# Patryk27/strolle

Measured on NVIDIA H100. Metric: Mrays/s (+ frames/s) at 1080p-per-GPU Cornell, ReSTIR DI+GI + SVGF; H100 vs CPU restatement of the reference, higher is better.
Workload: dtype f32

## Files before the change

### strolle_b200/csrc/engine.cu

```cuda
#include <algorithm>
#include <cmath>
#include <cstdio>
#include <cstring>
#include <deque>
#include <functional>
#include <limits>
#include <string>
#include <unordered_map>
#include <vector>

#include <nccl.h>

#include "../../include/strolle_b200.h"
#include "kernels.h"

#include <dlfcn.h>
namespace {
struct NcclApi {
    void* lib = nullptr;
    ncclResult_t (*GetUniqueId)(ncclUniqueId*) = nullptr;
    ncclResult_t (*CommInitRank)(ncclComm_t*, int, ncclUniqueId, int) = nullptr;
    ncclResult_t (*CommDestroy)(ncclComm_t) = nullptr;
    ncclResult_t (*GroupStart)() = nullptr;
    ncclResult_t (*GroupEnd)() = nullptr;
// ... 268 lines not shown
            nodes[pr.dst] = n;
        }
    }
    void plan_child(RefitPlan* plan, int child, uint32_t ptr, uint32_t slot, int depth) const {
        const Node& c = nodes[child];
        if (c.left >= 0) {
            if ((int)plan->levels.size() <= depth) plan->levels.resize(depth + 1);
            plan->levels[depth].push_back(make_uint2(ptr, slot));
        } else plan->runs.push_back(make_uint4(slot, ptr, c.e - c.b, 0u));
    }
    uint32_t emit(int id, int depth, const std::vector<uint8_t>& alpha, BvhOut* out, RefitPlan* plan) const {
        uint32_t at = (uint32_t)out->buf.size();
        if (depth > out->depth) out->depth = depth;
        const Node& nd = nodes[id];
        if (nd.left >= 0) {
            out->buf.resize(out->buf.size() + 4, make_float4(0, 0, 0, 0));
            uint32_t lp = emit(nd.left, depth + 1, alpha, out, plan);
            uint32_t rp = emit(nd.right, depth + 1, alpha, out, plan);
            if (plan) { plan_child(plan, nd.left, lp, at, depth + 1); plan_child(plan, nd.right, rp, at + 2, depth + 1); }
            const Box& lb = nodes[nd.left].box; const Box& rb = nodes[nd.right].box;
            out->buf[at] = make_float4(lb.lo.x, lb.lo.y, lb.lo.z, bits2f(0u));
            out->buf[at + 1] = make_float4(lb.hi.x, lb.hi.y, lb.hi.z, bits2f(rp));
            out->buf[at + 2] = make_float4(rb.lo.x, rb.lo.y, rb.lo.z, 0.0f);
            out->buf[at + 3] = make_float4(rb.hi.x, rb.hi.y, rb.hi.z, 0.0f);
        } else {
            uint32_t n = nd.e - nd.b;
            for (uint32_t i = 0; i < n; i++) {
                const Prim& p = prims[nd.b + i];
                uint32_t flags = (i + 1 < n ? 1u : 0u) | ((alpha[p.mat] ? 1u : 0u) << 1);
                out->buf.push_back(make_float4(bits2f(flags), bits2f(p.tri), bits2f(p.mat), bits2f(1u)));
            }
        }
        return at;
    }
};

struct DevMem {
    void* p = nullptr; size_t cap = 0;
    int ensure(size_t bytes) {
        if (bytes <= cap) return ST_OK;
        if (p) cudaFree(p);
        p = nullptr; cap = 0;
        size_t want = std::max<size_t>(bytes, 256);
        CK(cudaMalloc(&p, want));
        CK(cudaMemset(p, 0, want));
        CK(cudaDeviceSynchronize());
        cap = want;
        return ST_OK;
    }
    void release() { if (p) cudaFree(p); p = nullptr; cap = 0; }
};

static const char* kPassNames[P_COUNT] = {
    "prim_gbuffer", "di_sampling", "di_temporal_resampling", "di_spatial_resampling_pick", "di_spatial_resampling_trace", "di_spatial_resampling_sample",
    "di_resolving", "gi_reprojection", "gi_sampling_a", "gi_sampling_b", "gi_temporal_resampling", "gi_spatial_resampling_pick",
    "gi_spatial_resampling_trace", "gi_spatial_resampling_sample", "gi_preview_resampling", "gi_resolving", "frame_reprojection",
    "frame_denoising_reproject", "frame_denoising_estimate_variance", "frame_denoising_wavelet", "frame_composition", "ref_tracing",
    "ref_shading", "bvh_heatmap", "atmosphere", "trace_stream", "halo_exchange"};

static uint32_t dispatch_seed(uint32_t base, uint32_t frame, uint32_t k) {
    uint32_t s = base ^ (frame * 64u + k);
    s = s * 747796405u + 2891336453u;
    uint32_t w = ((s >> ((s >> 28) + 4u)) ^ s) * 277803737u;
    return (w >> 22) ^ w;
}

struct CameraSlot {
    bool alive = false;
    st_camera desc;
    st_camera prev_desc;
    uint32_t frame = 0;
    CameraDev dev;
    std::vector<std::pair<std::string, float4**>> named;
    std::vector<std::pair<std::string, size_t>> sizes;
    DevMem arena;
    DevMem svgf_pairs; float4* pair[2] = {nullptr, nullptr};
    DevMem rgba8; int rgba8_slot = 0;
    DevMem taa; float4* taa_hist[2] = {nullptr, nullptr};
    cudaEvent_t ev_ready[2] = {nullptr, nullptr}, ev_copied[2] = {nullptr, nullptr};
    cudaStream_t side[2] = {nullptr, nullptr}; cudaEvent_t ev_produced = nullptr, ev_pushed[2] = {nullptr, nullptr}; bool pushed_pending[2] = {false, false};
    struct PeerLink { bool ready = false; bool ipc = false; std::vector<char*> arena, rgba8; std::vector<uint32_t*> flags; DevMem sync; uint32_t seq = 0, fseq = 0; } peer;
};

struct Step { int pass; std::function<void(cudaStream_t)> run; int sub = -1; };

}

using namespace st;

struct st_engine {
    int device = 0;
    cudaStream_t stream = nullptr; bool own_stream = true;
    cudaStream_t copy_stream = nullptr;
    std::unordered_map<st_handle, std::vector<st_mesh_triangle>> meshes;
    std::vector<st_material> materials; std::vector<st_handle> material_handles; bool materials_dirty = false;
    struct MatTex { st_handle tex[4]; uint32_t mask; };
    std::vector<MatTex> material_textures;
    struct ImageRect { st_handle handle; uint32_t x, y, w, h; };
    std::vector<ImageRect> images; uint32_t shelf_x = 0, shelf_y = 0, shelf_h = 0; bool images_dirty = false;
    DevMem d_atlas, d_srgb, d_tri_instance, d_instance_xforms;
    bool motion_dirty = true;
    bool moved_last_tick = false;
    struct Inst {
        st_handle handle, mesh, material; Affine3 xf, xf_inv, prev_xf; bool dirty;
        st_handle baked_mesh = ~(st_handle)0, baked_material = ~(st_handle)0; bool host_stale = false; Affine3 dev_xf, dev_xf_inv;
    };
    std::vector<Inst> instances; bool instances_dirty = false;
    struct Range { st_handle handle; size_t b, e; };
    std::vector<Range> tri_ranges; SlotAllocator tri_alloc;
    std::vector<float4> h_triangles; std::vector<Prim> prims; bool triangles_dirty = false;
    BvhBuild bvh; BvhOut bvh_out; bool bvh_dirty = false;
    std::vector<GpuMaterial> h_materials;
    static const st_handle kSun = ~(st_handle)0;
    std::vector<GpuLight> h_lights; std::vector<std::pair<st_handle, uint32_t>> light_slots;
    std::vector<st_handle> lights_created, lights_updated; std::vector<std::pair<st_handle, uint32_t>> lights_remapped; std::vector<uint32_t> lights_killed;
    uint32_t next_light = 1; bool lights_dirty = true;
    float sun_azimuth = 0.0f, sun_altitude = 0.35f; bool sun_dirty = true;
    GpuWorld world;
    uint32_t frame = 1, seed_base = 0xC0FFEEu;
    DevMem d_triangles, d_bvh, d_materials, d_matpacked, d_unpacklut, d_lights, d_noise, d_tlut, d_slut, d_skylut, d_scratch, d_raycount;
    bool count_rays = false;
    bool svgf_fast = true;
    bool shading_fast = ST_SHADING_FAST_DEFAULT != 0;
    bool fused_passes = ST_FUSED_PASSES_DEFAULT != 0;
    bool async_output = false;
    bool halo_nccl = false;
    int wavelet_paired = ST_WAVELET_PAIRED_DEFAULT;
    int strip_dma = ST_STRIP_DMA_DEFAULT;
    bool strip_fused = true;
    bool last_frame_fused = false;
    int wavelet_tiled = ST_WAVELET_TILED_DEFAULT;
    int wavelet_cfg = ST_WAVELET_CFG_DEFAULT;
    DevMem d_tile_errors; uint64_t wavelet_tiled_launches = 0;
    bool fuse_reproject = ST_FUSE_REPROJECT_DEFAULT != 0;
    bool bvh_reuse = true;
    bool variance_tiled = ST_VARIANCE_TILED_DEFAULT != 0; uint64_t variance_tiled_launches = 0;
    bool normal_maps = false, any_normal_map = false, nmap_frame = false; uint64_t normal_map_launches = 0;
    int bvh_refit = 0; uint32_t refit_run = 0; uint64_t bvh_refits = 0; bool structure_changed = false;
    RefitPlan plan; bool plan_ready = false; std::vector<uint32_t> plan_levels; std::vector<uint8_t> plan_alpha; DevMem d_plan, d_bake;
    std::unordered_map<st_handle, DevMem> d_meshes;
    void* staging[2] = {nullptr, nullptr}; size_t staging_cap[2] = {0, 0}; cudaEvent_t staging_ev[2] = {nullptr, nullptr}; int staging_slot = 0;
    int light_grid = 0, lgrid_built = 0; bool lgrid_frame = false; LightGridDev lgrid{}; DevMem d_lgrid; uint64_t light_grid_builds = 0;
    bool texture_filter = false, texf_built = false, any_color_texture = false, texf_frame = false; TexFilterDev texf{};
    DevMem d_texf_pool, d_texf_table, d_texf_jobs; std::vector<uint2> h_texf_table; std::vector<MipJob> h_texf_jobs; size_t texf_pool_texels = 0;
    uint64_t texture_mip_builds = 0;
    bool temporal_aa = false, taa_frame = false; uint64_t taa_resolves = 0;
    bool luts_static_ready = false, sky_ready = false; float sky_for_altitude = 0.0f;
    std::vector<CameraSlot*> cameras;
    bool timing = false;
    float pass_ms[P_COUNT] = {}; uint32_t pass_launches[P_COUNT] = {};
    float wavelet_ms[5] = {}; uint32_t wavelet_launches[5] = {};
    struct Timed { int pass; cudaEvent_t a, b; int sub; };
    std::vector<Timed> pending; std::vector<cudaEvent_t> event_pool;
    cudaEvent_t mark_a = nullptr, mark_b = nullptr;
    ncclComm_t comm = nullptr; int rank = 0, n_ranks = 1;
    uint64_t halo_bytes_last_frame = 0;

    SceneDev scene() const {
        SceneDev s;
        s.triangles = (const float4*)d_triangles.p; s.bvh = (const float4*)d_bvh.p; s.bvh_len = (uint32_t)bvh_out.buf.size(); s.materials = (const GpuMaterial*)d_materials.p;
        s.lights = (const GpuLight*)d_lights.p; s.blue_noise = (const uchar4*)d_noise.p;
        s.transmittance_lut = (const float4*)d_tlut.p; s.scattering_lut = (const float4*)d_slut.p; s.sky_lut = (const float4*)d_skylut.p;
        s.world = world;
        s.tri_instance = (const uint32_t*)d_tri_instance.p; s.instance_xforms = (const float4*)d_instance_xforms.p;
        s.atlas = (const uchar4*)d_atlas.p; s.srgb_lut = (const float*)d_srgb.p;
        s.material_packed = (const uint32_t*)d_matpacked.p; s.unpack_lut = (const float*)d_unpacklut.p;
        s.ray_counter = count_rays ? (unsigned long long*)d_raycount.p : nullptr;
// ... 400 lines not shown
    for (auto& s : cs->sizes) total += (s.second * 16 + 255) / 256 * 256;
    cs->arena.release();
    int rc = cs->arena.ensure(total); if (rc) return rc;
    CK(cudaMemsetAsync(cs->arena.p, 0, total, e->stream));
    const size_t pair_bytes = (2 * n * 16 + 255) / 256 * 256;
    cs->svgf_pairs.release();
    if ((rc = cs->svgf_pairs.ensure(2 * pair_bytes))) return rc;
    CK(cudaMemsetAsync(cs->svgf_pairs.p, 0, 2 * pair_bytes, e->stream));
    cs->pair[0] = (float4*)cs->svgf_pairs.p; cs->pair[1] = (float4*)((char*)cs->svgf_pairs.p + pair_bytes);
    size_t off = 0;
    for (size_t i = 0; i < cs->named.size(); i++) { *cs->named[i].second = (float4*)((char*)cs->arena.p + off); off += (cs->sizes[i].second * 16 + 255) / 256 * 256; }
    d.w = (int)cs->desc.width; d.h = (int)cs->desc.height; d.y0 = 0; d.y1 = d.h;
    d.own_y0 = 0; d.own_y1 = d.h; d.mirror_up = 0; d.mirror_dn = 0; d.need_rows = nullptr; d.gi_mirror_reach = 128; d.di_mirror_reach = 128;
    cs->taa.release(); cs->taa_hist[0] = cs->taa_hist[1] = nullptr;
    return ST_OK;
}

struct StripExt { int gbuffer = 0, variance = 0, wavelet[5] = {0, 0, 0, 0, 0}; int preview_mirror[2] = {0, 0}; bool still = false;  };
static CameraDev grown(const CameraDev& c, int rows) { CameraDev g = c; g.y0 = std::max(0, c.y0 - rows); g.y1 = std::min(c.h, c.y1 + rows); return g; }
static void build_schedule(st_engine* e, CameraSlot* cs, std::vector<Step>* steps, const StripExt* ext = nullptr) {
    GpuCamera jc, jp; float4 jit;
    const bool taa = taa_cameras(e, cs, &jc, &jp, &jit);
    const CameraDev cam = [&] { CameraDev c = cs->dev; if (taa) { c.curr = jc; c.prev = jp; } return c; }();
    const StripExt no_ext; const StripExt& x = ext ? *ext : no_ext;
    const CameraDev camG = grown(cam, x.gbuffer), camV = grown(cam, x.variance);
    const int pm0 = x.preview_mirror[0], pm1 = x.preview_mirror[1];
    const SceneDev sc = e->scene();
    const uint32_t f = cs->frame;
    const int cur = (f % 2u) == 1u ? 1 : 0;
    const st_camera& d = cs->desc;
    const bool fs = e->shading_fast;
    const bool nm = e->nmap_frame;
    const bool lgon = e->lgrid_frame;
    const LightGridDev lgd = e->lgrid;
    const bool tfon = e->texf_frame;
    const TexFilterDev tfd = e->texf;
    auto seed = [&](uint32_t k) { return dispatch_seed(e->seed_base, f, k); };
    auto add = [&](int pass, std::function<void(cudaStream_t)> fn) { steps->push_back(Step{pass, std::move(fn)}); };
    const float4* di_final = (d.denoise && (d.mode == ST_MODE_IMAGE || d.mode == ST_MODE_DI_DIFFUSE)) ? cam.di_diff_curr_colors : cam.di_diff_samples;
    const float4* gi_final = (d.denoise && (d.mode == ST_MODE_IMAGE || d.mode == ST_MODE_GI_DIFFUSE)) ? cam.gi_diff_curr_colors : cam.gi_diff_samples;
    if (d.mode == ST_MODE_BVH_HEATMAP) {
        add(P_BVH_HEATMAP, [=](cudaStream_t s) { launch_bvh_heatmap(cam, sc, s); });
        add(P_COMPOSITION, [=](cudaStream_t s) { launch_composition(cam, sc, cur, 5u, di_final, gi_final, s); });
        return;
    }
    if (d.mode == ST_MODE_REFERENCE) {
        for (uint32_t depth = 0; depth <= (uint32_t)d.ref_depth; depth++) {
            uint32_t sd = seed(P_REF_SHADING_SEED + depth);
            add(P_REF_TRACING, [=](cudaStream_t s) { if (nm) e->normal_map_launches++; launch_ref_tracing(cam, sc, depth, nm, s); });
            add(P_REF_SHADING, [=](cudaStream_t s) { launch_ref_shading(cam, sc, sd, depth, lgon ? &lgd : nullptr, tfon ? &tfd : nullptr, s); });
        }
        add(P_REF_SHADING, [=](cudaStream_t s) { launch_ref_shading(cam, sc, 0u, 255u, nullptr, nullptr, s); });
        add(P_COMPOSITION, [=](cudaStream_t s) { launch_composition(cam, sc, cur, 6u, di_final, gi_final, s); });
        return;
    }
    const bool needs_di = d.mode == ST_MODE_IMAGE || d.mode == ST_MODE_DI_DIFFUSE || d.mode == ST_MODE_DI_SPECULAR;
    const bool needs_gi = d.mode == ST_MODE_IMAGE || d.mode == ST_MODE_GI_DIFFUSE || d.mode == ST_MODE_GI_SPECULAR;
    const int k4_in_k0 = (e->fused_passes && (ext == nullptr || ext->still) && !e->instances.empty()) ? 1 : 0;
    add(P_PRIM_GBUFFER, [=](cudaStream_t s) { if (nm) e->normal_map_launches++; launch_prim_gbuffer(camG, sc, cur, k4_in_k0, nm, tfon ? &tfd : nullptr, s); });
    const bool fp = e->fused_passes;
    if (!e->instances.empty()) {
        if (!k4_in_k0) add(P_FRAME_REPROJECTION, [=](cudaStream_t s) { launch_frame_reprojection(cam, sc, cur, s); });
        if (needs_di) {
            uint32_t s1 = seed(P_DI_SAMPLING), s2 = seed(P_DI_TEMPORAL), s3 = seed(P_DI_SPATIAL_PICK), s5 = seed(P_DI_SPATIAL_SAMPLE);
            if (fp) {
                add(P_DI_TEMPORAL, [=](cudaStream_t s) { (fs ? stf::launch_di_sample_temporal : st::launch_di_sample_temporal)(cam, sc, cur, s1, s2, f, lgon ? &lgd : nullptr, s); });
                add(P_DI_SPATIAL_PICK, [=](cudaStream_t s) { (fs ? stf::launch_di_spatial_fused : st::launch_di_spatial_fused)(cam, sc, cur, s3, s5, f, s); });
            } else {
                add(P_DI_SAMPLING, [=](cudaStream_t s) { (fs ? stf::launch_di_sampling : st::launch_di_sampling)(cam, sc, cur, s1, f, lgon ? &lgd : nullptr, s); });
                add(P_DI_TEMPORAL, [=](cudaStream_t s) { (fs ? stf::launch_di_temporal : st::launch_di_temporal)(cam, sc, cur, s2, s); });
                add(P_DI_SPATIAL_PICK, [=](cudaStream_t s) { (fs ? stf::launch_di_spatial_pick : st::launch_di_spatial_pick)(cam, sc, cur, s3, f, s); });
                add(P_DI_SPATIAL_TRACE, [=](cudaStream_t s) { (fs ? stf::launch_spatial_trace : st::launch_spatial_trace)(cam, sc, cam.di_diff_samples, cam.di_diff_curr_colors, cam.di_diff_stash, s); });
                add(P_DI_SPATIAL_SAMPLE, [=](cudaStream_t s) { (fs ? stf::launch_di_spatial_sample : st::launch_di_spatial_sample)(cam, sc, s5, f, s); });
            }
            add(P_DI_RESOLVING, [=](cudaStream_t s) { (fs ? stf::launch_di_resolving : st::launch_di_resolving)(cam, sc, cur, s); });
        }
        if (needs_gi) {
            uint32_t sa = seed(P_GI_SAMPLING_A), sb = seed(P_GI_SAMPLING_B), st_ = seed(P_GI_TEMPORAL), sp = seed(P_GI_SPATIAL_PICK), ss = seed(P_GI_SPATIAL_SAMPLE), sv = seed(P_GI_PREVIEW);
            uint32_t source;
            const bool tracing = f % 6u < 4u;
            const int inline_rp = (fp && tracing) ? 1 : 0;
            if (!inline_rp) add(P_GI_REPROJECTION, [=](cudaStream_t s) { (fs ? stf::launch_gi_reprojection : st::launch_gi_reprojection)(cam, sc, cur, s); });
            auto sampling = [&]() {
                if (fp) { add(P_GI_SAMPLING_B, [=](cudaStream_t s) { if (nm) e->normal_map_launches++; (fs ? stf::launch_gi_sampling_fused : st::launch_gi_sampling_fused)(cam, sc, cur, sa, sb, f, nm, lgon ? &lgd : nullptr, tfon ? &tfd : nullptr, s); }); return; }
                add(P_GI_SAMPLING_A, [=](cudaStream_t s) { if (nm) e->normal_map_launches++; (fs ? stf::launch_gi_sampling_a : st::launch_gi_sampling_a)(cam, sc, cur, sa, f, nm, tfon ? &tfd : nullptr, s); });
                add(P_GI_SAMPLING_B, [=](cudaStream_t s) { (fs ? stf::launch_gi_sampling_b : st::launch_gi_sampling_b)(cam, sc, cur, sb, f, lgon ? &lgd : nullptr, s); });
            };
            if (tracing) {
                if (f % 2u == 0u) sampling();
                add(P_GI_TEMPORAL, [=](cudaStream_t s) { (fs ? stf::launch_gi_temporal : st::launch_gi_temporal)(cam, sc, cur, st_, f, inline_rp, s); });
                if (f % 2u == 1u) {
                    if (fp) add(P_GI_SPATIAL_PICK, [=](cudaStream_t s) { (fs ? stf::launch_gi_spatial_fused : st::launch_gi_spatial_fused)(cam, sc, cur, sp, ss, f, s); });
                    else {
                        add(P_GI_SPATIAL_PICK, [=](cudaStream_t s) { (fs ? stf::launch_gi_spatial_pick : st::launch_gi_spatial_pick)(cam, sc, cur, sp, f, s); });
                        add(P_GI_SPATIAL_TRACE, [=](cudaStream_t s) { (fs ? stf::launch_spatial_trace : st::launch_spatial_trace)(cam, sc, cam.gi_d0, cam.gi_d1, cam.gi_d2, s); });
                        add(P_GI_SPATIAL_SAMPLE, [=](cudaStream_t s) { (fs ? stf::launch_gi_spatial_sample : st::launch_gi_spatial_sample)(cam, sc, ss, f, s); });
                    }
                    source = 1;
                } else source = 0;
            } else {
                sampling();
                add(P_GI_TEMPORAL, [=](cudaStream_t s) { (fs ? stf::launch_gi_temporal : st::launch_gi_temporal)(cam, sc, cur, st_, f, 0, s); });
                source = 0;
            }
            const float4* src0 = source == 0 ? cam.gi_reservoirs[1] : cam.gi_reservoirs[2];
            add(P_GI_PREVIEW, [=](cudaStream_t s) { (fs ? stf::launch_gi_preview : st::launch_gi_preview)(cam, sc, cur, sv, 0u, src0, cam.gi_reservoirs[3], pm0, s); });
            if (fp) add(P_GI_PREVIEW, [=](cudaStream_t s) { (fs ? stf::launch_gi_preview_resolve : st::launch_gi_preview_resolve)(cam, sc, cur, sv, cam.gi_reservoirs[3], src0, s); });
            else {
                add(P_GI_PREVIEW, [=](cudaStream_t s) { (fs ? stf::launch_gi_preview : st::launch_gi_preview)(cam, sc, cur, sv, 1u, cam.gi_reservoirs[3], cam.gi_reservoirs[0], pm1, s); });
                add(P_GI_RESOLVING, [=](cudaStream_t s) { (fs ? stf::launch_gi_resolving : st::launch_gi_resolving)(cam, sc, cur, src0, s); });
            }
        }
    }
    if (d.denoise) {
        if (e->fuse_reproject) {
            add(P_DENOISE_REPROJECT, [=](cudaStream_t s) { launch_denoise_reproject_pair(cam, sc, cur, s); });
        } else {
            add(P_DENOISE_REPROJECT, [=](cudaStream_t s) { launch_denoise_reproject(cam, sc, cur, cam.di_diff_prev_colors, cam.di_diff_moments[cur ^ 1], cam.di_diff_samples, cam.di_diff_curr_colors, cam.di_diff_moments[cur], s); });
            add(P_DENOISE_REPROJECT, [=](cudaStream_t s) { launch_denoise_reproject(cam, sc, cur, cam.gi_diff_prev_colors, cam.gi_diff_moments[cur ^ 1], cam.gi_diff_samples, cam.gi_diff_curr_colors, cam.gi_diff_moments[cur], s); });
        }
        const bool fast = e->svgf_fast;
        const bool var_tiled = e->variance_tiled; uint32_t* verr = (uint32_t*)e->d_tile_errors.p;
        add(P_DENOISE_VARIANCE, [=](cudaStream_t s) {
            if (var_tiled && launch_denoise_variance_tiled(camV, sc, cur, fast, verr, s)) { e->variance_tiled_launches++; return; }
            launch_denoise_variance(camV, sc, cur, fast, s);
        });
        float4* di_io[5][2] = {{cam.di_diff_stash, cam.di_diff_prev_colors}, {cam.di_diff_prev_colors, cam.di_diff_stash}, {cam.di_diff_stash, cam.di_diff_curr_colors},
                               {cam.di_diff_curr_colors, cam.di_diff_stash}, {cam.di_diff_stash, cam.di_diff_curr_colors}};
        float4* gi_io[5][2] = {{cam.gi_diff_stash, cam.gi_diff_prev_colors}, {cam.gi_diff_prev_colors, cam.gi_diff_stash}, {cam.gi_diff_stash, cam.gi_diff_curr_colors},
                               {cam.gi_diff_curr_colors, cam.gi_diff_stash}, {cam.gi_diff_stash, cam.gi_diff_curr_colors}};
        const bool whole_or_fused = ext != nullptr || (cam.y0 == 0 && cam.y1 == cam.h);
        const int first_paired_read = (fast && whole_or_fused && cs->pair[0]) ? (e->wavelet_paired == 2 ? 3 : e->wavelet_paired == 1 ? 4 : 5) : 5;
        for (uint32_t nth = 0; nth < 5; nth++) {
            float4 *a = di_io[nth][0], *b = di_io[nth][1], *c = gi_io[nth][0], *g = gi_io[nth][1];
            const bool reads_pair = (int)nth >= first_paired_read, writes_pair = (int)nth + 1 >= first_paired_read && nth < 4;
            const float4* pin = reads_pair ? cs->pair[nth & 1] : nullptr; float4* pout = writes_pair ? cs->pair[(nth + 1) & 1] : nullptr;
            const bool tiled = !reads_pair && ((e->wavelet_tiled >> nth) & 1) != 0; const int cfg = (e->wavelet_cfg >> (4 * nth)) & 15;
            uint32_t* terr = (uint32_t*)e->d_tile_errors.p;
            const CameraDev camW = grown(cam, x.wavelet[nth]);
            add(P_DENOISE_WAVELET, [=](cudaStream_t s) {
                if (tiled && launch_denoise_wavelet_tiled(camW, sc, f, 1u << nth, (float)(1 + nth), a, b, c, g, pout, fast, cfg, terr, s)) { e->wavelet_tiled_launches++; return; }
                launch_denoise_wavelet(camW, sc, cur, f, 1u << nth, (float)(1 + nth), a, b, c, g, pin, pout, fast, s);
            });
            steps->back().sub = (int)nth;
        }
    }
    uint32_t mode = (uint32_t)d.mode;
    if (taa) {
        const float4* hin = cs->taa_hist[cur ^ 1]; float4* hout = cs->taa_hist[cur];
        add(P_COMPOSITION, [=](cudaStream_t s) { e->taa_resolves++; launch_taa_resolve(cam, sc, cur, mode, di_final, gi_final, hin, hout, jit, s); });
        return;
    }
    add(P_COMPOSITION, [=](cudaStream_t s) { launch_composition(cam, sc, cur, mode, di_final, gi_final, s); });
}


struct HaloItem { std::string name; int reach; };
struct HaloExchange { int before_step; std::vector<HaloItem> items; };
static const int kSpatialReach = 128;
static const int kPreview2Reach = 64;
static const int kVarianceReach = 3;
static const int kWaveletReach[5] = {1, 2, 4, 9, 19};

static void plan_frame(const int* schedule, int n, uint32_t frame, int temporal_reach, std::vector<HaloExchange>* plan) {
    const char* cur = (frame % 2u == 1u) ? "b" : "a";
    const char* prv = (frame % 2u == 1u) ? "a" : "b";
    bool have_gbuffer = false; int nth_preview = 0, nth_wavelet = 0;
    const char* wavelet_inputs[5] = {"stash", "prev_colors", "stash", "curr_colors", "stash"};
    bool has_preview = false, has_gi_spatial = false;
    for (int i = 0; i < n; i++) { if (schedule[i] == P_GI_PREVIEW) has_preview = true; if (schedule[i] == P_GI_SPATIAL_PICK) has_gi_spatial = true; }
    std::string gi_source = has_gi_spatial ? "gi_reservoirs_2" : "gi_reservoirs_1";
    for (int i = 0; i < n; i++) {
        int p = schedule[i];
        HaloExchange ex; ex.before_step = i;
        auto add = [&](const std::string& name, int reach) { ex.items.push_back({name, reach}); };
        if (i == 0 && temporal_reach > 0) {
            add(std::string("prim_surface_map_") + prv, temporal_reach); add(std::string("prim_gbuffer_d0_") + prv, temporal_reach); add(std::string("prim_gbuffer_d1_") + prv, temporal_reach);
            add("di_reservoirs_0", temporal_reach); add("gi_reservoirs_0", temporal_reach); add("di_diff_prev_colors", temporal_reach); add("gi_diff_prev_colors", temporal_reach);
            add(std::string("di_diff_moments_") + prv, temporal_reach); add(std::string("gi_diff_moments_") + prv, temporal_reach);
        }
        if (p == P_DI_SPATIAL_PICK || p == P_GI_SPATIAL_PICK) {
            if (!have_gbuffer) { add(std::string("prim_gbuffer_d0_") + cur, kSpatialReach); add(std::string("prim_gbuffer_d1_") + cur, kSpatialReach); add("surface_nd", kSpatialReach); have_gbuffer = true; }
            add(p == P_DI_SPATIAL_PICK ? "di_reservoirs_1" : "gi_reservoirs_1", kSpatialReach);
        } else if (p == P_GI_PREVIEW) {
            if (nth_preview == 0) {
// ... 564 lines not shown
            e->refit_run = 0;
            e->plan_ready = e->bvh_refit > 0 && !too_deep;
            if (e->plan_ready) { e->plan_alpha = alpha; if ((rc = upload_plan(e))) return rc; }
        }
        e->moved_last_tick = e->motion_dirty;
    }
    if (e->motion_dirty) {
        e->motion_dirty = false;
        std::vector<uint32_t> tri_inst(e->h_triangles.size() / 9, 0u);
        std::vector<float4> xf = instance_xforms();
        for (size_t k = 0; k < e->instances.size(); k++)
            for (const auto& r : e->tri_ranges) if (r.handle == e->instances[k].handle) for (size_t t = r.b; t < r.e; t++) tri_inst[t] = (uint32_t)k;
        if ((rc = upload(e, e->d_tri_instance, tri_inst.data(), tri_inst.size() * 4))) return rc;
        if ((rc = upload(e, e->d_instance_xforms, xf.data(), xf.size() * 16))) return rc;
        CK(cudaStreamSynchronize(e->stream));
    }
    if (e->triangles_dirty) { e->triangles_dirty = false; if ((rc = upload(e, e->d_triangles, e->h_triangles.data(), e->h_triangles.size() * 16))) return rc; }
    e->world.light_count = e->next_light; e->world.sun_azimuth = e->sun_azimuth; e->world.sun_altitude = e->sun_altitude;
    if (e->sun_dirty) {
        e->sun_dirty = false;
        if ((rc = e->d_scratch.ensure(64))) return rc;
        launch_atm_sun_color((float4*)e->d_scratch.p, e->world, e->stream);
        float4 sun[2];
        CK(cudaMemcpyAsync(sun, e->d_scratch.p, 32, cudaMemcpyDeviceToHost, e->stream));
        CK(cudaStreamSynchronize(e->stream));
        light_overwrite(e, 0, st_engine::kSun, make_sun(sun[0], sun[1]));
    }
    const bool lights_uploaded = e->lights_dirty;
    if (e->lights_dirty) {
        for (uint32_t id : e->lights_killed) e->h_lights[id].d3.x = bits2f(0xcafebabeu);
        for (auto& r : e->lights_remapped) e->h_lights[r.second].d3.x = bits2f(*e->light_slot(r.first) + 1u);
        if ((rc = upload(e, e->d_lights, e->h_lights.data(), e->h_lights.size() * sizeof(GpuLight)))) return rc;
        CK(cudaStreamSynchronize(e->stream));
        bool again = !e->lights_created.empty() || !e->lights_updated.empty() || !e->lights_killed.empty() || !e->lights_remapped.empty();
        for (st_handle h : e->lights_created) { GpuLight& l = e->h_lights[*e->light_slot(h)]; l.prev_d0 = l.d0; l.prev_d1 = l.d1; l.prev_d2 = l.d2; }
        for (st_handle h : e->lights_updated) { GpuLight& l = e->h_lights[*e->light_slot(h)]; l.prev_d0 = l.d0; l.prev_d1 = l.d1; l.prev_d2 = l.d2; }
        for (uint32_t id : e->lights_killed) e->h_lights[id].d3.x = 0.0f;
        for (auto& r : e->lights_remapped) e->h_lights[r.second].d3.x = 0.0f;
        e->lights_created.clear(); e->lights_updated.clear(); e->lights_remapped.clear(); e->lights_killed.clear();
        e->lights_dirty = again;
    }
    if (e->light_grid == 0) e->lgrid_built = 0;
    else if (lights_uploaded || e->lgrid_built != e->light_grid) { if ((rc = build_light_grid(e))) return rc; }
    e->lgrid_frame = e->light_grid > 0;
    for (CameraSlot* c : e->cameras) if (c->alive) c->frame = e->frame;
    e->nmap_frame = e->normal_maps && e->any_normal_map;
    if (!e->texture_filter) {
        if (e->texf_built || e->d_texf_pool.p) { e->d_texf_pool.release(); e->d_texf_table.release(); e->d_texf_jobs.release(); e->texf = TexFilterDev{}; }
        e->texf_built = false;
    } else if (textures_changed || !e->texf_built) { if ((rc = build_texture_mips(e))) return rc; }
    e->texf_frame = e->texture_filter && e->any_color_texture;
    if (e->temporal_aa != e->taa_frame) for (CameraSlot* c : e->cameras) { c->taa.release(); c->taa_hist[0] = c->taa_hist[1] = nullptr; }
    e->taa_frame = e->temporal_aa;
    e->frame += 1;
    if (too_deep) return fail(ST_ERR_LIMIT, "BVH deeper than the 24-entry traversal stack (strolle-gpu/src/lib.rs:72-76): the scene is not drawn until it changes");
    return ST_OK;
}

int st_frame_schedule(st_engine* e, st_camera_handle h, int* pass_ids, int cap, int* count) {
    CameraSlot* cs = e ? get_camera(e, h) : nullptr;
    if (!cs || !count) return fail(ST_ERR_NOT_FOUND, "unknown camera");
    std::vector<Step> steps; build_schedule(e, cs, &steps);
    *count = (int)steps.size();
    for (int i = 0; i < cap && i < *count; i++) pass_ids[i] = steps[i].pass;
    return ST_OK;
}
static int ensure_taa_history(st_engine* e, CameraSlot* cs) {
    GpuCamera a, b; float4 j;
    if (cs->taa.p || !taa_cameras(e, cs, &a, &b, &j)) return ST_OK;
    const size_t bytes = ((size_t)cs->desc.width * cs->desc.height * 16 + 255) / 256 * 256;
    int rc = cs->taa.ensure(2 * bytes); if (rc) return rc;
    cs->taa_hist[0] = (float4*)cs->taa.p; cs->taa_hist[1] = (float4*)((char*)cs->taa.p + bytes);
    return ST_OK;
}
int st_render_range(st_engine* e, st_camera_handle h, int first, int last) {
    CameraSlot* cs = e ? get_camera(e, h) : nullptr;
    if (!cs) return fail(ST_ERR_NOT_FOUND, "unknown camera");
    if (cs->frame == 0) return fail(ST_ERR_INVALID, "st_tick must precede st_render_camera");
    CK(cudaSetDevice(e->device));
    int rc = ensure_luts(e); if (rc) return rc;
    if ((rc = ensure_taa_history(e, cs))) return rc;
    std::vector<Step> steps; build_schedule(e, cs, &steps);
    if (last < 0 || last >= (int)steps.size()) last = (int)steps.size() - 1;
    for (int i = std::max(first, 0); i <= last; i++) e->run_timed(steps[i].pass, steps[i].run, steps[i].sub);
    CK(cudaGetLastError());
    return ST_OK;
}
int st_render_camera(st_engine* e, st_camera_handle h, void* host_out, int format) {
    int rc = st_render_range(e, h, 0, -1); if (rc) return rc;
    if (host_out) return st_copy_output(e, h, host_out, format);
    return ST_OK;
}
static int copy_rows_out(st_engine* e, CameraSlot* cs, void* host_out, int format, int y0, int y1) {
    const size_t W = cs->desc.width, n = W * cs->desc.height;
    const size_t first = (size_t)y0 * W, count = (size_t)(y1 - y0) * W;
    if (format == ST_FORMAT_RGBA32F) CK(cudaMemcpyAsync((char*)host_out + first * 16, cs->dev.output + first, count * 16, cudaMemcpyDeviceToHost, e->stream));
    else if (format == ST_FORMAT_RGBA8_SRGB) {
        int rc2 = cs->rgba8.ensure(2 * n * 4); if (rc2) return rc2;
        cs->rgba8_slot ^= 1;
        SceneDev sc = e->scene(); uchar4* dst8 = (uchar4*)cs->rgba8.p + (cs->rgba8_slot ? n : 0); CameraDev cd = cs->dev; cd.y0 = y0; cd.y1 = y1;
        const int k = cs->rgba8_slot;
        if (e->async_output) {
            if (!e->copy_stream) CK(cudaStreamCreateWithFlags(&e->copy_stream, cudaStreamNonBlocking));
            if (!cs->ev_ready[k]) { CK(cudaEventCreateWithFlags(&cs->ev_ready[k], cudaEventDisableTiming)); CK(cudaEventCreateWithFlags(&cs->ev_copied[k], cudaEventDisableTiming)); }
            else CK(cudaStreamWaitEvent(e->stream, cs->ev_copied[k], 0));
        }
        e->run_timed(P_COMPOSITION, [=](cudaStream_t s) { launch_output_rgba8(cd, sc, dst8, s); });
        if (e->async_output) {
            CK(cudaEventRecord(cs->ev_ready[k], e->stream));
            CK(cudaStreamWaitEvent(e->copy_stream, cs->ev_ready[k], 0));
            CK(cudaMemcpyAsync((char*)host_out + first * 4, dst8 + first, count * 4, cudaMemcpyDeviceToHost, e->copy_stream));
            CK(cudaEventRecord(cs->ev_copied[k], e->copy_stream));
        } else CK(cudaMemcpyAsync((char*)host_out + first * 4, dst8 + first, count * 4, cudaMemcpyDeviceToHost, e->stream));
    } else return fail(ST_ERR_INVALID, "unsupported output format");
    return ST_OK;
}
int st_copy_output(st_engine* e, st_camera_handle h, void* host_out, int format) {
    CameraSlot* cs = e ? get_camera(e, h) : nullptr;
    if (!cs || !host_out) return fail(ST_ERR_NOT_FOUND, "unknown camera");
    CK(cudaSetDevice(e->device));
    int rc = copy_rows_out(e, cs, host_out, format, 0, (int)cs->desc.height); if (rc) return rc;
    if (!e->async_output) CK(cudaStreamSynchronize(e->stream));
    return ST_OK;
}
int st_synchronize(st_engine* e) {
    if (!e) return fail(ST_ERR_INVALID, "null engine");
    CK(cudaSetDevice(e->device)); CK(cudaStreamSynchronize(e->stream));
    if (e->copy_stream) CK(cudaStreamSynchronize(e->copy_stream));
    for (CameraSlot* c : e->cameras) for (int k = 0; k < 2; k++) if (c->side[k]) CK(cudaStreamSynchronize(c->side[k]));
    return ST_OK;
}

int st_read_buffer(st_engine* e, st_camera_handle h, const char* name, float* dst, size_t cap, size_t* count) {
    CameraSlot* cs = e ? get_camera(e, h) : nullptr;
    if (!cs || !name || !count) return fail(ST_ERR_NOT_FOUND, "unknown camera");
    CK(cudaSetDevice(e->device));
    if (!std::strcmp(name, "curr_camera") || !std::strcmp(name, "prev_camera")) {
        GpuCamera jc, jp; float4 jit;
        const bool taa = taa_cameras(e, cs, &jc, &jp, &jit);
        const GpuCamera& c = !std::strcmp(name, "curr_camera") ? (taa ? jc : cs->dev.curr) : (taa ? jp : cs->dev.prev);
        *count = 40; if (dst) std::memcpy(dst, &c, 4 * std::min<size_t>(cap, 40)); return ST_OK;
    }
    if (!std::strcmp(name, "taa_history_a") || !std::strcmp(name, "taa_history_b")) {
        const float4* p = cs->taa_hist[name[12] == 'a' ? 0 : 1];
        if (!p) return fail(ST_ERR_NOT_FOUND, "no temporal history: ST_OPT_TEMPORAL_AA is off or the camera has not resolved a frame since");
        *count = (size_t)cs->desc.width * cs->desc.height * 4;
        if (dst) { CK(cudaStreamSynchronize(e->stream)); CK(cudaMemcpy(dst, p, 4 * std::min(cap, *count), cudaMemcpyDeviceToHost)); }
        return ST_OK;
    }
    for (size_t i = 0; i < cs->named.size(); i++) if (cs->named[i].first == name) {
        *count = cs->sizes[i].second * 4;
        if (dst) { CK(cudaStreamSynchronize(e->stream)); CK(cudaMemcpy(dst, *cs->named[i].second, 4 * std::min(cap, *count), cudaMemcpyDeviceToHost)); }
        return ST_OK;
    }
    return fail(ST_ERR_NOT_FOUND, std::string("unknown buffer ") + name);
}
int st_buffer_device_ptr(st_engine* e, st_camera_handle h, const char* name, void** ptr, size_t* bytes) {
    CameraSlot* cs = e ? get_camera(e, h) : nullptr;
    if (!cs || !name || !ptr || !bytes) return fail(ST_ERR_NOT_FOUND, "unknown camera");
    for (size_t i = 0; i < cs->named.size(); i++) if (cs->named[i].first == name) { *ptr = *cs->named[i].second; *bytes = cs->sizes[i].second * 16; return ST_OK; }
    if ((!std::strcmp(name, "taa_history_a") || !std::strcmp(name, "taa_history_b")) && cs->taa_hist[0]) {
        *ptr = cs->taa_hist[name[12] == 'a' ? 0 : 1]; *bytes = (size_t)cs->desc.width * cs->desc.height * 16; return ST_OK;
    }
    return fail(ST_ERR_NOT_FOUND, std::string("unknown buffer ") + name);
}
int st_read_scene(st_engine* e, const char* name, float* dst, size_t cap, size_t* count) {
    if (!e || !name || !count) return fail(ST_ERR_INVALID, "null argument");
// ... 598 lines not shown
```

### strolle_b200/csrc/kernels.cu

```cuda
#include <algorithm>
#include <cstdio>
#include <cuda_fp16.h>
#include <cuda.h>
#include <map>
#include <mutex>
#include <tuple>
#include <vector>
#include "st_device.cuh"
#include "kernels.h"

#if defined(ST_FAST) && ST_FAST
#define ST_EXACT_ONLY 0
#else
#define ST_EXACT_ONLY 1
#endif

namespace ST_NS {

#define TILE_W 16
#define TILE_H 8

struct Px { u32 x, y; bool in; };
ST_DEV u32 row_tile(const CameraDev& cam) {
    if (cam.mirror_dn == 0) return blockIdx.y;
    const u32 lead = (u32)(ST_REACH_SPATIAL / TILE_H);
    return gridDim.y > lead ? (blockIdx.y + gridDim.y - lead) % gridDim.y : blockIdx.y;
}
ST_DEV Px pixel_full(const CameraDev& cam) {
    Px p; p.x = blockIdx.x * TILE_W + (threadIdx.x % TILE_W); p.y = (u32)cam.y0 + row_tile(cam) * TILE_H + (threadIdx.x / TILE_W);
    p.in = p.x < (u32)cam.w && p.y < (u32)cam.y1;
    return p;
}
ST_DEV int half_grid_w(int w) { return 8 * (((w + 7) / 8) / 2); }
ST_DEV Px pixel_half(const CameraDev& cam) {
    Px p; p.x = blockIdx.x * TILE_W + (threadIdx.x % TILE_W); p.y = (u32)cam.y0 + row_tile(cam) * TILE_H + (threadIdx.x / TILE_W);
    p.in = p.x < (u32)half_grid_w(cam.w) && p.y < (u32)cam.y1;
    return p;
}
ST_DEV size_t pix(const CameraDev& cam, u32 x, u32 y) { return (size_t)y * (size_t)cam.w + x; }
ST_DEV size_t screen_idx(const CameraDev& cam, u32 x, u32 y) { return (size_t)(y * to_u32_sat(cam.curr.screen.x) + x); }
ST_DEV bool in_tex(const CameraDev& cam, u32 x, u32 y) { return x < (u32)cam.w && y < (u32)cam.h; }
ST_DEV float4 tex_or_zero(const float4* __restrict__ t, const CameraDev& cam, u32 x, u32 y) { return in_tex(cam, x, y) ? t[pix(cam, x, y)] : f4zero(); }
ST_DEV void tex_store(float4* __restrict__ t, const CameraDev& cam, u32 x, u32 y, float4 v) { if (in_tex(cam, x, y)) t[pix(cam, x, y)] = v; }
ST_DEV Hit load_hit(const GpuCamera& c, const float4* __restrict__ d0, const float4* __restrict__ d1, const CameraDev& cam, u32 x, u32 y) {
    return hit_make(cam_ray(c, x, y), gbuf_unpack(tex_or_zero(d0, cam, x, y), tex_or_zero(d1, cam, x, y)));
}
ST_DEV Hit load_hit_lut(const SceneDev& sc, const GpuCamera& c, const float4* __restrict__ d0, const float4* __restrict__ d1, const CameraDev& cam, u32 x, u32 y) {
    return hit_make(cam_ray(c, x, y), gbuf_unpack(sc, tex_or_zero(d0, cam, x, y), tex_or_zero(d1, cam, x, y)));
}
#define ST_TRACE_STACK()                                          \
    __shared__ u32 s_stack[ST_BVH_STACK * ST_BLOCK];              \
    TraceStack stk; stk.base = s_stack + threadIdx.x;

#define KPARAMS const __grid_constant__ CameraDev cam, const __grid_constant__ SceneDev sc

#define ST_LB_N(N) __launch_bounds__(ST_BLOCK, N)
#if !defined(ST_MINB_ALL)
#define ST_MINB_GI_PREVIEW 8
#define ST_MINB_GI_TEMPORAL 8
#define ST_MINB_GI_SAMPLING_B 8
#define ST_MINB_GI_SPATIAL_PICK 8
#define ST_MINB_DI_TEMPORAL 12
#endif
#define ST_LB_PICK(per_kernel) ST_LB_CHOOSE(ST_MINB_ALL_OR_0, per_kernel)
#if defined(ST_MINB_ALL)
#define ST_MINB_ALL_OR_0 ST_MINB_ALL
#else
#define ST_MINB_ALL_OR_0 0
#endif
template <int ALL, int ONE> struct LbMin { static constexpr int value = ALL > 0 ? ALL : ONE; };
#define ST_LB_CHOOSE(all, one) __launch_bounds__(ST_BLOCK, (LbMin<all, one>::value > 0 ? LbMin<all, one>::value : 1))
#ifndef ST_MINB_PRIM_GBUFFER
#define ST_MINB_PRIM_GBUFFER 0
#endif
#define ST_LB_PRIM_GBUFFER ST_LB_PICK(ST_MINB_PRIM_GBUFFER)
#ifndef ST_MINB_DI_SAMPLING
#define ST_MINB_DI_SAMPLING 0
#endif
#define ST_LB_DI_SAMPLING ST_LB_PICK(ST_MINB_DI_SAMPLING)
#ifndef ST_MINB_DI_TEMPORAL
#define ST_MINB_DI_TEMPORAL 0
#endif
#define ST_LB_DI_TEMPORAL ST_LB_PICK(ST_MINB_DI_TEMPORAL)
#ifndef ST_MINB_DI_SPATIAL_PICK
#define ST_MINB_DI_SPATIAL_PICK 0
#endif
#define ST_LB_DI_SPATIAL_PICK ST_LB_PICK(ST_MINB_DI_SPATIAL_PICK)
#ifndef ST_MINB_SPATIAL_TRACE
#define ST_MINB_SPATIAL_TRACE 0
#endif
#define ST_LB_SPATIAL_TRACE ST_LB_PICK(ST_MINB_SPATIAL_TRACE)
#ifndef ST_MINB_DI_RESOLVING
#define ST_MINB_DI_RESOLVING 0
#endif
#define ST_LB_DI_RESOLVING ST_LB_PICK(ST_MINB_DI_RESOLVING)
#ifndef ST_MINB_GI_SAMPLING_A
#define ST_MINB_GI_SAMPLING_A 0
#endif
#define ST_LB_GI_SAMPLING_A ST_LB_PICK(ST_MINB_GI_SAMPLING_A)
#ifndef ST_MINB_GI_SAMPLING_B
#define ST_MINB_GI_SAMPLING_B 0
#endif
#define ST_LB_GI_SAMPLING_B ST_LB_PICK(ST_MINB_GI_SAMPLING_B)
#ifndef ST_MINB_GI_TEMPORAL
#define ST_MINB_GI_TEMPORAL 0
#endif
#define ST_LB_GI_TEMPORAL ST_LB_PICK(ST_MINB_GI_TEMPORAL)
#ifndef ST_MINB_GI_SPATIAL_PICK
#define ST_MINB_GI_SPATIAL_PICK 0
#endif
#define ST_LB_GI_SPATIAL_PICK ST_LB_PICK(ST_MINB_GI_SPATIAL_PICK)
#ifndef ST_MINB_GI_SPATIAL_SAMPLE
#define ST_MINB_GI_SPATIAL_SAMPLE 0
#endif
#define ST_LB_GI_SPATIAL_SAMPLE ST_LB_PICK(ST_MINB_GI_SPATIAL_SAMPLE)
#ifndef ST_MINB_GI_PREVIEW
#define ST_MINB_GI_PREVIEW 0
#endif
#define ST_LB_GI_PREVIEW ST_LB_PICK(ST_MINB_GI_PREVIEW)
#ifndef ST_MINB_GI_RESOLVING
#define ST_MINB_GI_RESOLVING 0
#endif
#define ST_LB_GI_RESOLVING ST_LB_PICK(ST_MINB_GI_RESOLVING)

#if ST_EXACT_ONLY
ST_DEV float4 frame_reprojection_px(const CameraDev& cam, int cur, Px p, float4 surface_texel, float4 vel);
template <bool NMAP, bool TEXF>
__global__ void ST_LB_PRIM_GBUFFER k_prim_gbuffer(KPARAMS, int cur, int with_reprojection, const __grid_constant__ TexFilterDev tf) {
    ST_TRACE_STACK();
    Px p = pixel_full(cam);
    if (!p.in) return;
    Ray ray = cam_ray(cam.curr, p.x, p.y);
    TriHit th = trace_closest(ray, sc, stk);
    if ((int)p.y < cam.own_y0 || (int)p.y >= cam.own_y1) uncount_ray(sc);
    float4 g0 = f4zero(), g1 = f4zero(), surf = f4zero(), vel = f4zero(), tid = f4(bitsf(0xffffffffu), 0.f, 0.f, 0.f), nd = f4zero();
    if (trihit_some(th)) {
        const GpuMaterial m = sc.materials[th.material_id];
        if (NMAP) th.normal = nmap_normal(sc, th, m.normal_map_texture);
        GBuf g;
        float2 mr;
        if (TEXF) {
            TexFoot ft; ft.tri = th.triangle_id; ft.dir = ray.d; ft.w = texf_cone_width(cam.curr, p.x, p.y, th.t, true);
            const float4 t = texf_sample(sc, tf, th.material_id, 2u, m.metallic_roughness_texture, f4(1.0f, m.roughness, m.metallic, 1.0f), th.uv, ft);
            mr = f2(t.z, t.y);
            g.base_color = texf_sample(sc, tf, th.material_id, 0u, m.base_color_texture, m.base_color, th.uv, ft);
            g.emissive = xyz(texf_sample(sc, tf, th.material_id, 1u, m.emissive_texture, m.emissive, th.uv, ft));
        } else {
            mr = mat_metallic_roughness(sc, m, th.uv);
            g.base_color = mat_base_color(sc, m, th.uv); g.emissive = mat_emissive(sc, m, th.uv);
        }
        g.normal = th.normal; g.metallic = mr.x;
        g.roughness = mr.y; g.reflectance = m.reflectance; g.depth = dist(ray.o, th.point);
        gbuf_pack_pre(g, all_zero(m.base_color_texture) ? __ldg(sc.material_packed + th.material_id) : gbuf_pack_color(g.base_color), &g0, &g1);
        float2 n = oct_encode(th.normal);
        surf = f4(n.x, n.y, g.depth, m.roughness);
        nd = f4(oct_decode(n), g.depth);
        const float4* xf = sc.instance_xforms + 6u * (size_t)__ldg(sc.tri_instance + th.triangle_id);
        float4 c0 = ldg4(xf), c1 = ldg4(xf + 1), c2 = ldg4(xf + 2), q0 = ldg4(xf + 3), q1 = ldg4(xf + 4), q2 = ldg4(xf + 5);
        float3 local = ((xyz(c0) * th.point.x + xyz(c1) * th.point.y) + xyz(c2) * th.point.z) + f3(c0.w, c1.w, c2.w);
        float3 prev_point = ((xyz(q0) * local.x + xyz(q1) * local.y) + xyz(q2) * local.z) + f3(q0.w, q1.w, q2.w);
        float2 v = cam_world_to_screen(cam.curr, th.point) - cam_world_to_screen(cam.prev, prev_point);
        if (len2(v) >= 0.001f) vel = f4(v.x, v.y, 0.f, 0.f);
        tid.x = bitsf(th.triangle_id);
        if (cam.need_rows != nullptr && vel.y != 0.0f && (int)p.y >= cam.own_y0 && (int)p.y < cam.own_y1) {
            float py = (float)p.y - vel.y;
            int lo = max(0, min(cam.h - 1, to_i32_sat(floorf(py)))), hi = max(0, min(cam.h - 1, to_i32_sat(ceilf(py))));
            if (lo < cam.own_y0) atomicMin(cam.need_rows, lo);
            if (hi >= cam.own_y1) atomicMax(cam.need_rows + 1, hi);
        }
    }
    size_t i = pix(cam, p.x, p.y);
    cam.prim_gbuffer_d0[cur][i] = g0; cam.prim_gbuffer_d1[cur][i] = g1; cam.prim_surface_map[cur][i] = surf;
    cam.velocity_map[i] = vel; cam.prim_triangle_ids[i] = tid; cam.surface_nd[i] = nd;
    if (with_reprojection && (int)p.y >= cam.own_y0 && (int)p.y < cam.own_y1) cam.reprojection_map[i] = frame_reprojection_px(cam, cur, p, surf, vel);
}

ST_DEV float4 frame_reprojection_px(const CameraDev& cam, int cur, Px p, float4 surface_texel, float4 vel) {
    const float4* sp_ = cam.prim_surface_map[cur ^ 1];
    Reproj rp; rp.px = 0.f; rp.py = 0.f; rp.confidence = 0.f; rp.validity = 0u;
    Surf surface = surf_decode(surface_texel);
    if (surface.depth == 0.0f) return reproj_encode(rp);
    float2 prev = f2((float)p.x, (float)p.y) - f2(vel.x, vel.y);
    float2 pr = f2(roundf(prev.x), roundf(prev.y));
    if (cam_contains_f(cam.prev, pr)) {
        Surf ps = surf_decode(tex_or_zero(sp_, cam, to_u32_sat(pr.x), to_u32_sat(pr.y)));
        float conf = surf_similarity(ps, surface);
        if (conf > 0.0f) { rp.px = prev.x; rp.py = prev.y; rp.confidence = conf; rp.validity = 0u; }
    }
    if (reproj_some(rp)) {
        int x0 = to_i32_sat(floorf(rp.px)), x1 = to_i32_sat(ceilf(rp.px)), y0 = to_i32_sat(floorf(rp.py)), y1 = to_i32_sat(ceilf(rp.py));
        int xs[4] = {x0, x1, x0, x1}, ys[4] = {y0, y0, y1, y1};
#pragma unroll
        for (int k = 0; k < 4; k++) {
            if (!cam_contains_i(cam.curr, xs[k], ys[k])) continue;
            if (surf_similarity(surf_decode(sp_[pix(cam, (u32)xs[k], (u32)ys[k])]), surface) >= 0.25f) rp.validity |= (1u << k);
        }
    }
    return reproj_encode(rp);
}
__global__ void __launch_bounds__(ST_BLOCK) k_frame_reprojection(KPARAMS, int cur) {
    Px p = pixel_full(cam);
    if (!p.in) return;
    size_t i = pix(cam, p.x, p.y);
    cam.reprojection_map[i] = frame_reprojection_px(cam, cur, p, cam.prim_surface_map[cur][i], cam.velocity_map[i]);
}
#endif

template <bool LGRID>
ST_DEV DiRes di_sampling_px(const CameraDev& cam, const SceneDev& sc, const TraceStack& stk, const Hit& hit, u32 seed, u32 frame, Px p, const LightGridDev& lg) {
    Rng rng = rng_make(seed, p.x, p.y);
    EphRes res = LGRID ? ephemeral_build_list(rng, sc, hit, lgrid_list(lg, hit.point)) : ephemeral_build(rng, sc, hit);
    DiRes out = di_zero();
    if (res.m > 0.0f) {
        float4 bn = blue_noise(sc, p.x, p.y, frame);
        Ray ray = light_ray_bnoise(light_load(sc, res.light_id), f2(bn.x, bn.y), hit.point);
        bool occ = trace_any(ray, sc, stk);
        if (occ) res.w = 0.0f;
        out.pdf = 0.f; out.confidence = 0.f; out.light_id = res.light_id; out.light_point = ray.o; out.occluded = occ; out.m = 1.0f; out.w = res.w;
    }
    return out;
}
template <bool LGRID>
__global__ void ST_LB_DI_SAMPLING k_di_sampling(KPARAMS, int cur, u32 seed, u32 frame, const __grid_constant__ LightGridDev lg) {
    ST_TRACE_STACK();
    Px p = pixel_full(cam);
    if (!p.in) return;
    Hit hit = load_hit_lut(sc, cam.curr, cam.prim_gbuffer_d0[cur], cam.prim_gbuffer_d1[cur], cam, p.x, p.y);
    if (!hit_some(hit)) return;
    di_store(di_sampling_px<LGRID>(cam, sc, stk, hit, seed, frame, p, lg), cam.di_reservoirs[1], screen_idx(cam, p.x, p.y));
}

ST_DEV DiRes di_temporal_px(const CameraDev& cam, const SceneDev& sc, int cur, u32 seed, Px p, const Hit& lhs_hit, DiRes lhs) {
    size_t npx = (size_t)cam.w * cam.h;
    Rng rng = rng_make(seed, p.x, p.y);
    if (lhs.m != 0.0f) lhs.pdf = di_pdf_with(lhs, light_load(sc, lhs.light_id), lhs_hit);
    DiRes rhs = di_zero();
    Hit rhs_hit = hit_zero();
    bool killed = false;
    Reproj rp = reproj_decode(cam.reprojection_map[pix(cam, p.x, p.y)]);
    if (reproj_some(rp)) {
        uint2 rpos = reproj_round(rp);
        size_t ridx = screen_idx(cam, rpos.x, rpos.y);
        if (ridx < npx) rhs = di_load(cam.di_reservoirs[0], ridx);
        rhs.m = rmin(rhs.m, 64.0f);
        if (rhs.m != 0.0f) {
            GpuLight rl = light_load(sc, rhs.light_id);
            u32 slot = fbits(rl.d3.x);
            if (slot == 0xcafebabeu) { rhs.w = 0.0f; killed = true; }
            else if (slot > 0u) rhs.light_id = slot - 1u;
            rhs_hit = load_hit_lut(sc, cam.prev, cam.prim_gbuffer_d0[cur ^ 1], cam.prim_gbuffer_d1[cur ^ 1], cam, rpos.x, rpos.y);
        }
    }
    MisIn mi;
    mi.lhs_m = lhs.m; mi.rhs_m = rhs.m; mi.rhs_jacobian = 1.0f; mi.lhs_lhs_pdf = lhs.pdf; mi.rhs_rhs_pdf = rhs.pdf;
    mi.lhs_rhs_pdf = ((lhs.m > 0.0f) & hit_some(rhs_hit)) ? di_pdf_with(lhs, light_prev(light_load(sc, lhs.light_id)), rhs_hit) : 0.0f;
    mi.rhs_lhs_pdf = ((rhs.m > 0.0f) & !killed) ? di_pdf_with(rhs, light_load(sc, rhs.light_id), lhs_hit) : 0.0f;
    MisOut mo = mis_eval(mi);
    DiRes main_ = di_zero();
    float main_pdf = 0.0f;
    if (di_update(main_, rng, lhs, mo.lhs_mis * mo.lhs_pdf * lhs.w)) main_pdf = mo.lhs_pdf;
    if (di_update(main_, rng, rhs, mo.rhs_mis * mo.rhs_pdf * rhs.w)) main_pdf = mo.rhs_pdf;
    main_.m = lhs.m + mo.m;
    main_.pdf = main_pdf;
    main_.confidence = killed ? 0.0f : 1.0f;
    main_.w = res_norm(main_.w, main_pdf, 1.0f, 1.0f);
    return main_;
}
__global__ void ST_LB_DI_TEMPORAL k_di_temporal(KPARAMS, int cur, u32 seed) {
    Px p = pixel_full(cam);
    if (!p.in) return;
    size_t lhs_idx = screen_idx(cam, p.x, p.y);
    Hit lhs_hit = load_hit_lut(sc, cam.curr, cam.prim_gbuffer_d0[cur], cam.prim_gbuffer_d1[cur], cam, p.x, p.y);
    if (!hit_some(lhs_hit)) return;
    di_store_m(cam, di_temporal_px(cam, sc, cur, seed, p, lhs_hit, di_load(cam.di_reservoirs[1], lhs_idx)), cam.di_reservoirs[1], lhs_idx, p.y, cam.di_mirror_reach);
}
template <bool LGRID>
__global__ void ST_LB_DI_SAMPLING k_di_sample_temporal(KPARAMS, int cur, u32 seed_sampling, u32 seed_temporal, u32 frame, const __grid_constant__ LightGridDev lg) {
    ST_TRACE_STACK();
    Px p = pixel_full(cam);
    if (!p.in) return;
    Hit hit = load_hit_lut(sc, cam.curr, cam.prim_gbuffer_d0[cur], cam.prim_gbuffer_d1[cur], cam, p.x, p.y);
    if (!hit_some(hit)) return;
    DiRes fresh = di_sampling_px<LGRID>(cam, sc, stk, hit, seed_sampling, frame, p, lg);
    di_store_m(cam, di_temporal_px(cam, sc, cur, seed_temporal, p, hit, fresh), cam.di_reservoirs[1], screen_idx(cam, p.x, p.y), p.y, cam.di_mirror_reach);
}

struct PairTexels { float4 a0, a1, b0, b1; int state; };

ST_DEV PairTexels di_spatial_pick_pair(const CameraDev& cam, const SceneDev& sc, int cur, u32 seed, u32 frame, Px g) {
    PairTexels o; o.a0 = o.a1 = o.b0 = o.b1 = f4zero(); o.state = 0;
    uint2 lp = checker(g.x, g.y, frame / 2u + 1u);
    if (!cam_contains_u(cam.curr, lp.x, lp.y)) return o;
    o.state = 1;
    size_t lhs_idx = screen_idx(cam, lp.x, lp.y);
    Rng rng = rng_make(seed, lp.x, lp.y);
    const float4* gd0 = cam.prim_gbuffer_d0[cur]; const float4* gd1 = cam.prim_gbuffer_d1[cur];
    Hit lhs_hit = load_hit_lut(sc, cam.curr, gd0, gd1, cam, lp.x, lp.y);
    if (!hit_some(lhs_hit)) return o;
    DiRes lhs = di_load(cam.di_reservoirs[1], lhs_idx);
    DiRes rhs = di_zero();
    size_t rhs_idx = 0;
    Hit rhs_hit = hit_zero();
    float max_radius = 128.0f;
    for (u32 nth = 0u; nth < 8u; nth++) {
        float2 off = rng_disk(rng) * max_radius;
        float2 fp = f2((float)lp.x, (float)lp.y) + off;
        uint2 rpos = cam_contain(cam.curr, to_i32_sat(fp.x), to_i32_sat(fp.y));
        if (rpos.x == lp.x && rpos.y == lp.y) continue;
        float4 nd = tex_or_zero(cam.surface_nd, cam, rpos.x, rpos.y);
        if (nd.w == 0.0f) { max_radius = rmax(max_radius * 0.5f, 5.0f); continue; }
        if (fabs_(nd.w - lhs_hit.g.depth) > 0.33f * lhs_hit.g.depth) { max_radius = rmax(max_radius * 0.5f, 5.0f); continue; }
        if (dot(xyz(nd), lhs_hit.g.normal) < 0.33f) { max_radius = rmax(max_radius * 0.5f, 5.0f); continue; }
        rhs_idx = screen_idx(cam, rpos.x, rpos.y);
        rhs = di_load(cam.di_reservoirs[1], rhs_idx);
        if (rhs.m != 0.0f) { rhs_hit = load_hit_lut(sc, cam.curr, gd0, gd1, cam, rpos.x, rpos.y); break; }
    }
    if (rhs.m == 0.0f) return o;
    float lhs_rhs_pdf = di_pdf_with(lhs, light_load(sc, lhs.light_id), rhs_hit);
    float rhs_lhs_pdf = di_pdf_with(rhs, light_load(sc, rhs.light_id), lhs_hit);
    Ray ra = (lhs_rhs_pdf > 0.0f) ? di_ray(lhs, rhs_hit.point) : ray_zero();
    Ray rb = (rhs_lhs_pdf > 0.0f) ? di_ray(rhs, lhs_hit.point) : ray_zero();
    float2 na = oct_encode(ra.d), nb = oct_encode(rb.d);
    o.a0 = f4(ra.o, ra.len); o.a1 = f4(na.x, na.y, bitsf((u32)rhs_idx + 1u), 0.0f);
    o.b0 = f4(rb.o, rb.len); o.b1 = f4(nb.x, nb.y, lhs_rhs_pdf, rhs_lhs_pdf);
    o.state = 2;
    return o;
}
ST_DEV void store_pair_texels(const CameraDev& cam, const PairTexels& o, float4* buf_d0, float4* buf_d1, Px g) {
    if (o.state == 0) return;
    u32 ax = g.x * 2u, bx = g.x * 2u + 1u;
    if (o.state == 2) { tex_store(buf_d0, cam, ax, g.y, o.a0); tex_store(buf_d0, cam, bx, g.y, o.b0); }
    tex_store(buf_d1, cam, ax, g.y, o.a1); tex_store(buf_d1, cam, bx, g.y, o.b1);
}
__global__ void ST_LB_DI_SPATIAL_PICK k_di_spatial_pick(KPARAMS, int cur, u32 seed, u32 frame) {
    Px g = pixel_half(cam);
    if (!g.in) return;
    store_pair_texels(cam, di_spatial_pick_pair(cam, sc, cur, seed, frame, g), cam.di_diff_samples, cam.di_diff_curr_colors, g);
}

ST_DEV float4 spatial_trace_texel(const SceneDev& sc, const TraceStack& stk, float4 d0, float4 d1) {
    if (all_zero(d1)) return f4zero();
    Ray ray = ray_make(xyz(d0), oct_decode(f2(d1.x, d1.y)), d0.w);
    bool occ = trace_any(ray, sc, stk);
    return f4(occ ? 0.0f : 1.0f, d1.z, d1.w, 0.0f);
}
__global__ void ST_LB_SPATIAL_TRACE k_spatial_trace(KPARAMS, const float4* __restrict__ buf_d0, const float4* __restrict__ buf_d1, float4* __restrict__ buf_d2) {
    ST_TRACE_STACK();
    Px p = pixel_full(cam);
    if (!p.in) return;
    size_t i = pix(cam, p.x, p.y);
    buf_d2[i] = spatial_trace_texel(sc, stk, buf_d0[i], buf_d1[i]);
}
ST_DEV void trace_pair_texels(const CameraDev& cam, const SceneDev& sc, const TraceStack& stk, const PairTexels& o, Px g, float4* d2a, float4* d2b) {
    u32 ax = g.x * 2u, bx = g.x * 2u + 1u;
    *d2a = (o.state == 2 && in_tex(cam, ax, g.y)) ? spatial_trace_texel(sc, stk, o.a0, o.a1) : f4zero();
    *d2b = (o.state == 2 && in_tex(cam, bx, g.y)) ? spatial_trace_texel(sc, stk, o.b0, o.b1) : f4zero();
}

ST_DEV void di_spatial_sample_pair(const CameraDev& cam, u32 seed, u32 frame, Px g, float4 d0, float4 d1) {
    uint2 lp = checker(g.x, g.y, frame / 2u + 1u);
    if (!cam_contains_u(cam.curr, lp.x, lp.y)) return;
    size_t npx = (size_t)cam.w * cam.h;
    size_t lhs_idx = screen_idx(cam, lp.x, lp.y);
    Rng rng = rng_make(seed, lp.x, lp.y);
    const float4* in = cam.di_reservoirs[1]; float4* out = cam.di_reservoirs[2];
    float lhs_rhs_vis = d0.x; u32 rhs_idx = fbits(d0.y);
    float rhs_lhs_vis = d1.x, lhs_rhs_pdf = d1.y, rhs_lhs_pdf = d1.z;
    DiRes lhs = di_load(in, lhs_idx);
    if (rhs_idx > 0u && (size_t)rhs_idx - 1 < npx) {
        DiRes rhs = di_load(in, (size_t)rhs_idx - 1);
        MisIn mi;
        mi.lhs_m = lhs.m; mi.rhs_m = rhs.m; mi.rhs_jacobian = 1.0f; mi.lhs_lhs_pdf = lhs.pdf;
        mi.lhs_rhs_pdf = lhs_rhs_pdf * lhs_rhs_vis; mi.rhs_lhs_pdf = rhs_lhs_pdf * rhs_lhs_vis; mi.rhs_rhs_pdf = rhs.pdf;
        MisOut mo = mis_eval(mi);
        DiRes main_ = di_zero();
        float main_pdf = 0.0f;
        if (di_update(main_, rng, lhs, mo.lhs_mis * mo.lhs_pdf * lhs.w)) main_pdf = mo.lhs_pdf;
        if (di_update(main_, rng, rhs, mo.rhs_mis * mo.rhs_pdf * rhs.w)) { main_pdf = mo.rhs_pdf; main_.occluded = lhs_rhs_vis == 0.0f; }
        main_.m = lhs.m + mo.m;
        main_.pdf = main_pdf;
        main_.w = res_norm(main_.w, main_pdf, 1.0f, 1.0f);
        di_store(main_, out, lhs_idx);
    } else di_store(lhs, out, lhs_idx);
    uint2 op = checker(g.x, g.y, frame / 2u);
    if (cam_contains_u(cam.curr, op.x, op.y)) { size_t oi = screen_idx(cam, op.x, op.y); di_store(di_load(in, oi), out, oi); }
}
__global__ void __launch_bounds__(ST_BLOCK) k_di_spatial_sample(KPARAMS, u32 seed, u32 frame) {
    Px g = pixel_half(cam);
    if (!g.in) return;
    di_spatial_sample_pair(cam, seed, frame, g, tex_or_zero(cam.di_diff_stash, cam, g.x * 2u, g.y), tex_or_zero(cam.di_diff_stash, cam, g.x * 2u + 1u, g.y));
}
__global__ void ST_LB_DI_SPATIAL_PICK k_di_spatial_fused(KPARAMS, int cur, u32 seed_pick, u32 seed_sample, u32 frame) {
    ST_TRACE_STACK();
    Px g = pixel_half(cam);
    if (!g.in) return;
    PairTexels o = di_spatial_pick_pair(cam, sc, cur, seed_pick, frame, g);
    if (o.state == 0) return;
    float4 d2a, d2b; trace_pair_texels(cam, sc, stk, o, g, &d2a, &d2b);
    di_spatial_sample_pair(cam, seed_sample, frame, g, d2a, d2b);
}

__global__ void ST_LB_DI_RESOLVING k_di_resolving(KPARAMS, int cur) {
    ST_TRACE_STACK();
    Px p = pixel_full(cam);
    if (!p.in) return;
    size_t idx = screen_idx(cam, p.x, p.y);
    Hit hit = load_hit_lut(sc, cam.curr, cam.prim_gbuffer_d0[cur], cam.prim_gbuffer_d1[cur], cam, p.x, p.y);
    DiRes res = di_load(cam.di_reservoirs[2], idx);
    float confidence;
    LightRad rad;
    if (hit_some(hit)) {
        bool occ = trace_any(di_ray(res, hit.point), sc, stk);
        confidence = (res.occluded == occ) ? res.confidence : 0.0f;
        res.confidence = 1.0f;
        res.occluded = occ;
        if (occ) rad = lightrad_zero();
        else { rad = light_radiance(light_load(sc, res.light_id), hit); rad.radiance = rad.radiance * res.w; }
    } else {
        confidence = 1.0f;
        rad.radiance = atmosphere_sample(sc, world_sun_dir(sc.world), hit.dir);
        rad.diff = f3s(1.0f); rad.spec = f3s(0.0f);
    }
    float diff_brdf = (1.0f - hit.g.metallic) / kPi;
    size_t i = pix(cam, p.x, p.y);
    cam.di_diff_samples[i] = f4(rad.radiance * diff_brdf, confidence);
    cam.di_spec_samples[i] = f4(rad.radiance * rad.spec, confidence);
    di_store(res, cam.di_reservoirs[0], idx);
}

ST_DEV GiRes gi_reprojection_px(const CameraDev& cam, const Hit& hit, const Reproj& rp) {
    size_t npx = (size_t)cam.w * cam.h;
    GiRes res = gi_zero();
    if (reproj_some(rp)) {
        uint2 rpos = reproj_round(rp);
        size_t ridx = screen_idx(cam, rpos.x, rpos.y);
        if (ridx < npx) res = gi_load(cam.gi_reservoirs[0], ridx);
    }
    res.confidence = 1.0f;
    res.v1 = hit.point;
    return res;
}
__global__ void __launch_bounds__(ST_BLOCK) k_gi_reprojection(KPARAMS, int cur) {
    Px p = pixel_full(cam);
    if (!p.in) return;
    Hit hit = load_hit_lut(sc, cam.curr, cam.prim_gbuffer_d0[cur], cam.prim_gbuffer_d1[cur], cam, p.x, p.y);
    if (!hit_some(hit)) return;
    gi_store_m(cam, gi_reprojection_px(cam, hit, reproj_decode(cam.reprojection_map[pix(cam, p.x, p.y)])), cam.gi_reservoirs[2], screen_idx(cam, p.x, p.y), p.y,
               (int)p.x >= 2 * half_grid_w(cam.w) ? cam.gi_mirror_reach : 0);
}

template <bool NMAP, bool TEXF>
ST_DEV bool gi_sampling_a_pair(const CameraDev& cam, const SceneDev& sc, const TraceStack& stk, int cur, u32 seed, u32 frame, Px g, float4* t0, float4* t1, float4* t2,
                               const TexFilterDev& tf) {
    bool tracing = gi_tracing_frame(frame);
    uint2 sp = tracing ? checker(g.x, g.y, frame / 2u) : checker(g.x, g.y, frame);
    if (!cam_contains_u(cam.curr, sp.x, sp.y)) return false;
    size_t idx = screen_idx(cam, sp.x, sp.y);
    Ray gi_r; float gi_pdf_;
    if (tracing) {
        Rng rng = rng_make(seed, sp.x, sp.y);
        Hit hit = load_hit_lut(sc, cam.curr, cam.prim_gbuffer_d0[cur], cam.prim_gbuffer_d1[cur], cam, sp.x, sp.y);
        if (!hit_some(hit)) return false;
        BrdfS s = brdf_layered_sample(hit.g, rng, -hit.dir);
        gi_r = ray_make(hit.point, s.dir);
        gi_pdf_ = s.pdf;
    } else {
        GiRes res = gi_load(cam.gi_reservoirs[2], idx);
        if (res.m == 0.0f) return false;
        gi_r = ray_make(res.v1, gi_dir(res, res.v1));
        gi_pdf_ = 1.0f;
    }
    TriHit gh = trace_closest(gi_r, sc, stk);
    GBuf gg = gbuf_zero();
    u32 gi_color_bits = 0u;
    if (trihit_some(gh)) {
        GpuMaterial m = sc.materials[gh.material_id];
        m.roughness = rmax(m.roughness, 0.75f * 0.75f);
        if (TEXF) {
            TexFoot ft; ft.tri = gh.triangle_id; ft.dir = gi_r.d; ft.w = texf_cone_width(cam.curr, sp.x, sp.y, gh.t, false);
            gg.base_color = texf_sample(sc, tf, gh.material_id, 0u, m.base_color_texture, m.base_color, gh.uv, ft);
            gg.emissive = xyz(texf_sample(sc, tf, gh.material_id, 1u, m.emissive_texture, m.emissive, gh.uv, ft));
            gg.normal = NMAP ? nmap_normal(sc, gh, m.normal_map_texture) : gh.normal; gg.metallic = m.metallic;
        } else {
            gg.base_color = mat_base_color(sc, m, gh.uv); gg.normal = NMAP ? nmap_normal(sc, gh, m.normal_map_texture) : gh.normal; gg.metallic = m.metallic; gg.emissive = mat_emissive(sc, m, gh.uv);
        }
        gi_color_bits = all_zero(m.base_color_texture) ? __ldg(sc.material_packed + gh.material_id) : gbuf_pack_color(gg.base_color);
        gg.roughness = m.roughness; gg.reflectance = m.reflectance; gg.depth = dist(gi_r.o, gh.point);
    }
    gbuf_pack_pre(gg, gi_color_bits, t1, t2);
    *t0 = f4(gi_r.d, gi_pdf_);
    return true;
}
template <bool NMAP, bool TEXF>
__global__ void ST_LB_GI_SAMPLING_A k_gi_sampling_a(KPARAMS, int cur, u32 seed, u32 frame, const __grid_constant__ TexFilterDev tf) {
    ST_TRACE_STACK();
    Px g = pixel_half(cam);
    if (!g.in) return;
    float4 t0, t1, t2;
    if (!gi_sampling_a_pair<NMAP, TEXF>(cam, sc, stk, cur, seed, frame, g, &t0, &t1, &t2, tf)) return;
    size_t gi = pix(cam, g.x, g.y);
    cam.gi_d0[gi] = t0; cam.gi_d1[gi] = t1; cam.gi_d2[gi] = t2;
}

template <bool LGRID>
ST_DEV void gi_sampling_b_pair(const CameraDev& cam, const SceneDev& sc, const TraceStack& stk, int cur, u32 seed, u32 frame, Px g, float4 d0, float4 d1, float4 d2, const LightGridDev& lg) {
    bool tracing = gi_tracing_frame(frame);
    uint2 sp = tracing ? checker(g.x, g.y, frame / 2u) : checker(g.x, g.y, frame);
    if (!cam_contains_u(cam.curr, sp.x, sp.y)) return;
    size_t idx = screen_idx(cam, sp.x, sp.y);
    Hit prim = load_hit_lut(sc, cam.curr, cam.prim_gbuffer_d0[cur], cam.prim_gbuffer_d1[cur], cam, sp.x, sp.y);
    if (!hit_some(prim)) return;
    Rng rng; Hit gh; float gi_pdf_;
    if (tracing) {
        rng = rng_make(seed, sp.x, sp.y);
        gh = hit_make(ray_make(prim.point, xyz(d0)), gbuf_unpack(sc, d1, d2));
        gi_pdf_ = d0.w;
    } else {
        GiRes res = gi_load(cam.gi_reservoirs[2], idx);
        if (res.m == 0.0f) return;
        rng.s = res.rng;
        gh = hit_make(ray_make(res.v1, xyz(d0)), gbuf_unpack(sc, d1, d2));
        gi_pdf_ = 1.0f;
    }
    u32 rng_state = rng.s;
    const u32 SKY = 0xffffffffu;
    float3 sun_dir = world_sun_dir(sc.world);
    u32 light_id; float light_pdf; float3 light_rad; float3 light_dir = f3s(0.f);
    if (!hit_some(gh)) { light_id = SKY; light_pdf = 1.0f; light_rad = atmosphere_sample(sc, sun_dir, gh.dir); }
    else {
        float atm_pdf = (sc.world.sun_altitude <= -1.0f) ? 0.0f : 0.25f;
        if (sc.world.light_count == 0u || rng_f(rng) < atm_pdf) {
            light_id = SKY; light_pdf = atm_pdf;
            light_dir = rng_hemisphere(rng, gh.g.normal);
            light_rad = atmosphere_sample(sc, sun_dir, light_dir) * dot(gh.g.normal, light_dir);
        } else {
            EphRes er = LGRID ? ephemeral_build_list(rng, sc, gh, lgrid_list(lg, gh.point)) : ephemeral_build(rng, sc, gh);
            if (er.w > 0.0f) { light_id = er.light_id; light_pdf = (1.0f / er.w) * (1.0f - atm_pdf); light_rad = er.rad.radiance * (f3s(1.0f) + er.rad.spec); }
            else { light_id = 0u; light_pdf = 1.0f; light_rad = f3s(0.f); }
        }
    }
    float3 radiance;
    if (light_pdf > 0.0f) {
        float vis;
        if (hit_some(gh)) {
            Ray r = (light_id == SKY) ? ray_make(gh.point, light_dir) : light_ray_wnoise(light_load(sc, light_id), rng, gh.point);
            vis = trace_any(r, sc, stk) ? 0.0f : 1.0f;
        } else vis = 1.0f;
        radiance = light_rad * vis / light_pdf;
    } else radiance = f3s(0.f);
    if (hit_some(gh)) { radiance = radiance * (xyz(gh.g.base_color) / kPi); radiance = radiance + gh.g.emissive; }
    GiRes res = gi_zero();
    if (gi_pdf_ > 0.0f) {
        res.rng = rng_state; res.radiance = radiance; res.v1 = prim.point;
        if (hit_some(gh)) { res.v2 = gh.point; res.v2n = gh.g.normal; }
        else { res.v2 = prim.point + gh.dir * 1000.0f; res.v2n = -gh.dir; }
        res.m = 1.0f; res.w = 1.0f / gi_pdf_;
        res.pdf = 0.0f;
        res.pdf = gi_pdf(res, prim);
    }
    gi_store(res, cam.gi_reservoirs[1], idx);
}
template <bool LGRID>
__global__ void ST_LB_GI_SAMPLING_B k_gi_sampling_b(KPARAMS, int cur, u32 seed, u32 frame, const __grid_constant__ LightGridDev lg) {
    ST_TRACE_STACK();
    Px g = pixel_half(cam);
    if (!g.in) return;
    size_t gi = pix(cam, g.x, g.y);
    gi_sampling_b_pair<LGRID>(cam, sc, stk, cur, seed, frame, g, cam.gi_d0[gi], cam.gi_d1[gi], cam.gi_d2[gi], lg);
}
template <bool NMAP, bool LGRID, bool TEXF>
__global__ void ST_LB_GI_SAMPLING_B k_gi_sampling_fused(KPARAMS, int cur, u32 seed_a, u32 seed_b, u32 frame, const __grid_constant__ LightGridDev lg,
                                                        const __grid_constant__ TexFilterDev tf) {
    ST_TRACE_STACK();
    Px g = pixel_half(cam);
    if (!g.in) return;
    float4 t0, t1, t2;
    if (!gi_sampling_a_pair<NMAP, TEXF>(cam, sc, stk, cur, seed_a, frame, g, &t0, &t1, &t2, tf)) return;
    gi_sampling_b_pair<LGRID>(cam, sc, stk, cur, seed_b, frame, g, t0, t1, t2, lg);
}

__global__ void ST_LB_GI_TEMPORAL k_gi_temporal(KPARAMS, int cur, u32 seed, u32 frame, int inline_reprojection) {
    Px p = pixel_full(cam);
    if (!p.in) return;
    bool tracing = gi_tracing_frame(frame);
    size_t lhs_idx = screen_idx(cam, p.x, p.y);
    Rng rng = rng_make(seed, p.x, p.y);
    Hit lhs_hit = load_hit_lut(sc, cam.curr, cam.prim_gbuffer_d0[cur], cam.prim_gbuffer_d1[cur], cam, p.x, p.y);
    float4* curr = cam.gi_reservoirs[1];
    if (!hit_some(lhs_hit)) { gi_store_m(cam, gi_zero(), curr, lhs_idx, p.y, cam.gi_mirror_reach); return; }
    bool got = tracing ? (frame % 2u == 0u && checker_at(p.x, p.y, frame / 2u)) : checker_at(p.x, p.y, frame);
    GiRes lhs = got ? gi_load(curr, lhs_idx) : gi_zero();
    GiRes rhs = gi_zero();
    Hit rhs_hit = hit_zero();
    Reproj rp = reproj_decode(cam.reprojection_map[pix(cam, p.x, p.y)]);
    if (inline_reprojection) {
        GiRes r11 = gi_reprojection_px(cam, lhs_hit, rp);
        if ((int)p.x >= 2 * half_grid_w(cam.w)) gi_store_m(cam, r11, cam.gi_reservoirs[2], lhs_idx, p.y, cam.gi_mirror_reach);
        if (reproj_some(rp)) { rhs = r11; rhs.v2n = oct_decode(oct_encode(r11.v2n)); }
    } else if (reproj_some(rp)) rhs = gi_load(cam.gi_reservoirs[2], lhs_idx);
    if (reproj_some(rp)) {
        rhs.confidence = 1.0f;
        rhs.m = rmin(rhs.m, 128.0f);
        if (!tracing && lhs.m != 0.0f && rhs.m != 0.0f && gi_exists(rhs)) {
            if (dist(lhs.radiance, rhs.radiance) > 0.33f) rhs.confidence = 0.0f;
            rhs.radiance = lhs.radiance; rhs.v2 = lhs.v2; rhs.v2n = lhs.v2n;
        }
        if (rhs.m != 0.0f) {
            uint2 rpos = reproj_round(rp);
            rhs_hit = load_hit_lut(sc, cam.prev, cam.prim_gbuffer_d0[cur ^ 1], cam.prim_gbuffer_d1[cur ^ 1], cam, rpos.x, rpos.y);
        }
    }
    GiRes main_ = gi_zero();
    float main_pdf = 0.0f;
    if (tracing) {
        MisIn mi;
        mi.lhs_m = lhs.m; mi.rhs_m = rhs.m; mi.rhs_jacobian = 1.0f; mi.lhs_lhs_pdf = lhs.pdf; mi.rhs_rhs_pdf = rhs.pdf;
        mi.lhs_rhs_pdf = ((lhs.m > 0.0f) & hit_some(rhs_hit)) ? gi_pdf(lhs, rhs_hit) : 0.0f;
        mi.rhs_lhs_pdf = (rhs.m > 0.0f) ? gi_pdf(rhs, lhs_hit) : 0.0f;
        MisOut mo = mis_eval(mi);
        if (gi_update(main_, rng, lhs, mo.lhs_mis * mo.lhs_pdf * lhs.w)) main_pdf = mo.lhs_pdf;
        if (gi_update(main_, rng, rhs, mo.rhs_mis * mo.rhs_pdf * rhs.w)) main_pdf = mo.rhs_pdf;
        main_.m = lhs.m + mo.m;
        main_.confidence = 1.0f;
        main_.w = res_norm(main_.w, main_pdf, 1.0f, 1.0f);
    } else {
        if (gi_merge(main_, rng, rhs, rhs.pdf)) main_pdf = rhs.pdf;
        main_.confidence = rhs.confidence;
        main_.w = res_norm(main_.w, main_pdf, 1.0f, main_.m);
    }
    main_.pdf = main_pdf;
    main_.v1 = lhs_hit.point;
    main_.w = rmin(main_.w, 5.0f);
    gi_store_m(cam, main_, curr, lhs_idx, p.y, cam.gi_mirror_reach);
}

ST_DEV PairTexels gi_spatial_pick_pair(const CameraDev& cam, const SceneDev& sc, int cur, u32 seed, u32 frame, Px g) {
    PairTexels o; o.a0 = o.a1 = o.b0 = o.b1 = f4zero(); o.state = 0;
    uint2 lp = checker(g.x, g.y, frame / 2u + 1u);
    if (!cam_contains_u(cam.curr, lp.x, lp.y)) return o;
    o.state = 1;
    size_t lhs_idx = screen_idx(cam, lp.x, lp.y);
    Rng rng = rng_make(seed, lp.x, lp.y);
    const float4* gd0 = cam.prim_gbuffer_d0[cur]; const float4* gd1 = cam.prim_gbuffer_d1[cur];
    const float4* reservoirs = cam.gi_reservoirs[1];
    Hit lhs_hit = load_hit_lut(sc, cam.curr, gd0, gd1, cam, lp.x, lp.y);
    GiRes lhs = gi_load(reservoirs, lhs_idx);
    if (!hit_some(lhs_hit) || lhs.m == 0.0f) return o;
    GiRes rhs = gi_zero();
    size_t rhs_idx = 0;
    Hit rhs_hit = hit_zero();
    float rhs_jac = 0.0f;
    float max_radius = 128.0f;
    for (u32 nth = 0u; nth < 8u; nth++) {
        float2 off = rng_disk(rng) * max_radius;
        float2 fp = f2((float)lp.x, (float)lp.y) + off;
        uint2 rpos = cam_contain(cam.curr, to_i32_sat(fp.x), to_i32_sat(fp.y));
        if (rpos.x == lp.x && rpos.y == lp.y) continue;
        float4 nd = tex_or_zero(cam.surface_nd, cam, rpos.x, rpos.y);
        if (nd.w == 0.0f) { max_radius = rmax(max_radius * 0.5f, 5.0f); continue; }
        if (fabs_(nd.w - lhs_hit.g.depth) > 0.33f * lhs_hit.g.depth) { max_radius = rmax(max_radius * 0.5f, 5.0f); continue; }
        if (dot(xyz(nd), lhs_hit.g.normal) < 0.33f) { max_radius = rmax(max_radius * 0.5f, 5.0f); continue; }
        rhs_idx = screen_idx(cam, rpos.x, rpos.y);
        rhs = gi_load(reservoirs, rhs_idx);
        if (rhs.m == 0.0f) continue;
        rhs_jac = gi_jacobian(rhs, lhs_hit.point);
        if (rhs_jac < 1.0f / 10.0f || rhs_jac > 10.0f) { rhs.m = 0.0f; continue; }
        rhs_jac = rclamp(rhs_jac, 1.0f / 3.0f, 3.0f);
        rhs_hit = load_hit_lut(sc, cam.curr, gd0, gd1, cam, rpos.x, rpos.y);
        break;
    }
    if (rhs.m == 0.0f || !hit_some(rhs_hit)) return o;
    float lhs_rhs_pdf = gi_pdf(lhs, rhs_hit);
    float rhs_lhs_pdf = gi_pdf(rhs, lhs_hit);
    Ray ra = (lhs_rhs_pdf > 0.0f) ? gi_ray(lhs, rhs_hit.point) : ray_zero();
    Ray rb = (rhs_lhs_pdf > 0.0f) ? gi_ray(rhs, lhs_hit.point) : ray_zero();
    float2 na = oct_encode(ra.d), nb = oct_encode(rb.d);
    o.a0 = f4(ra.o, ra.len); o.a1 = f4(na.x, na.y, bitsf((u32)rhs_idx + 1u), rhs_jac);
    o.b0 = f4(rb.o, rb.len); o.b1 = f4(nb.x, nb.y, lhs_rhs_pdf, rhs_lhs_pdf);
    o.state = 2;
    return o;
}
__global__ void ST_LB_GI_SPATIAL_PICK k_gi_spatial_pick(KPARAMS, int cur, u32 seed, u32 frame) {
    Px g = pixel_half(cam);
    if (!g.in) return;
    store_pair_texels(cam, gi_spatial_pick_pair(cam, sc, cur, seed, frame, g), cam.gi_d0, cam.gi_d1, g);
}

ST_DEV void gi_spatial_sample_pair(const CameraDev& cam, u32 seed, u32 frame, Px g, float4 d0, float4 d1) {
    uint2 sp = checker(g.x, g.y, frame / 2u + 1u);
    if (!cam_contains_u(cam.curr, sp.x, sp.y)) return;
    size_t npx = (size_t)cam.w * cam.h;
    size_t idx = screen_idx(cam, sp.x, sp.y);
    Rng rng = rng_make(seed, sp.x, sp.y);
    const float4* in = cam.gi_reservoirs[1]; float4* out = cam.gi_reservoirs[2];
    float lhs_rhs_vis = d0.x; u32 rhs_idx = fbits(d0.y); float rhs_jac = d0.z;
    float rhs_lhs_vis = d1.x, lhs_rhs_pdf = d1.y, rhs_lhs_pdf = d1.z;
    GiRes lhs = gi_load(in, idx);
    if (rhs_idx > 0u && (size_t)rhs_idx - 1 < npx) {
        GiRes rhs = gi_load(in, (size_t)rhs_idx - 1);
        MisIn mi;
        mi.lhs_m = lhs.m; mi.rhs_m = rhs.m; mi.rhs_jacobian = rhs_jac; mi.lhs_lhs_pdf = lhs.pdf;
        mi.lhs_rhs_pdf = lhs_rhs_pdf * lhs_rhs_vis; mi.rhs_lhs_pdf = rhs_lhs_pdf * rhs_lhs_vis; mi.rhs_rhs_pdf = rhs.pdf;
        MisOut mo = mis_eval(mi);
        GiRes main_ = gi_zero();
        float main_pdf = 0.0f;
        if (gi_update(main_, rng, lhs, mo.lhs_mis * mo.lhs_pdf * lhs.w)) main_pdf = mo.lhs_pdf;
        if (gi_update(main_, rng, rhs, mo.rhs_mis * mo.rhs_pdf * rhs.w * rhs_jac)) main_pdf = mo.rhs_pdf;
        main_.m = lhs.m + mo.m;
        main_.confidence = 1.0f;
        main_.pdf = main_pdf;
        main_.v1 = lhs.v1;
        main_.w = res_norm(main_.w, main_pdf, 1.0f, 1.0f);
        main_.w = rmin(main_.w, 5.0f);
        gi_store_m(cam, main_, out, idx, sp.y, cam.gi_mirror_reach);
    } else gi_store_m(cam, lhs, out, idx, sp.y, cam.gi_mirror_reach);
    uint2 op = checker(g.x, g.y, frame / 2u);
    if (cam_contains_u(cam.curr, op.x, op.y)) { size_t oi = screen_idx(cam, op.x, op.y); gi_store_m(cam, gi_load(in, oi), out, oi, op.y, cam.gi_mirror_reach); }
}
__global__ void ST_LB_GI_SPATIAL_SAMPLE k_gi_spatial_sample(KPARAMS, u32 seed, u32 frame) {
    Px g = pixel_half(cam);
    if (!g.in) return;
    gi_spatial_sample_pair(cam, seed, frame, g, tex_or_zero(cam.gi_d2, cam, g.x * 2u, g.y), tex_or_zero(cam.gi_d2, cam, g.x * 2u + 1u, g.y));
}
__global__ void ST_LB_GI_SPATIAL_PICK k_gi_spatial_fused(KPARAMS, int cur, u32 seed_pick, u32 seed_sample, u32 frame) {
    ST_TRACE_STACK();
    Px g = pixel_half(cam);
    if (!g.in) return;
    PairTexels o = gi_spatial_pick_pair(cam, sc, cur, seed_pick, frame, g);
    if (o.state == 0) return;
    float4 d2a, d2b; trace_pair_texels(cam, sc, stk, o, g, &d2a, &d2b);
    gi_spatial_sample_pair(cam, seed_sample, frame, g, d2a, d2b);
}

ST_DEV bool gi_preview_px(const CameraDev& cam, const SceneDev& sc, const Hit& chit, u32 seed, u32 nth, const float4* __restrict__ in, Px p, GiRes* result) {
    size_t cidx = screen_idx(cam, p.x, p.y);
    Rng rng = rng_make(seed, p.x, p.y);
    if (!hit_some(chit)) { *result = gi_zero(); return true; }
    GiRes main_ = gi_zero();
    float main_pdf = 0.0f;
    GiRes center = gi_load(in, cidx);
    if (gi_merge(main_, rng, center, center.pdf)) main_pdf = center.pdf;
    u32 max_samples = to_u32_sat(lerpc(8.0f, 0.0f, main_.m / 8.0f));
    float max_radius = (nth == 0u) ? 128.0f : 64.0f;
    const float4* __restrict__ surf = cam.surface_nd;
    for (u32 k = 0u; k < max_samples; k++) {
        float2 off = rng_disk(rng) * max_radius;
        float2 fp = f2((float)p.x, (float)p.y) + off;
        uint2 sp = cam_contain(cam.curr, to_i32_sat(fp.x), to_i32_sat(fp.y));
        if (sp.x == p.x && sp.y == p.y) return false;
        if (!cam_contains_u(cam.curr, sp.x, sp.y)) continue;
        float4 nd = surf[pix(cam, sp.x, sp.y)];
        if (nd.w == 0.0f) continue;
        if (fabs_(nd.w - chit.g.depth) > 0.25f * chit.g.depth) continue;
        if (dot(xyz(nd), chit.g.normal) < 0.5f) continue;
        GiRes s = gi_load(in, screen_idx(cam, sp.x, sp.y));
        if (s.m == 0.0f) continue;
        float s_pdf = gi_pdf(s, chit);
        float s_jac = gi_jacobian(s, chit.point);
        if (s_jac < 1.0f / 10.0f || s_jac > 10.0f) continue;
        s_jac = rclamp(s_jac, 1.0f / 3.0f, 3.0f);
        if (gi_merge(main_, rng, s, s_pdf * s_jac)) main_pdf = s_pdf;
    }
    main_.confidence = center.confidence;
    main_.pdf = main_pdf;
    main_.v1 = center.v1;
    main_.w = res_norm(main_.w, main_pdf, 1.0f, main_.m);
    main_.w = rmin(main_.w, 5.0f);
    *result = main_;
    return true;
}
__global__ void ST_LB_GI_PREVIEW k_gi_preview(KPARAMS, int cur, u32 seed, u32 nth, const float4* __restrict__ in, float4* __restrict__ out, int reach) {
    Px p = pixel_full(cam);
    if (!p.in) return;
    Hit chit = load_hit_lut(sc, cam.curr, cam.prim_gbuffer_d0[cur], cam.prim_gbuffer_d1[cur], cam, p.x, p.y);
    GiRes r;
    if (gi_preview_px(cam, sc, chit, seed, nth, in, p, &r)) gi_store_m(cam, r, out, screen_idx(cam, p.x, p.y), p.y, reach);
}

ST_DEV void gi_resolving_px(const CameraDev& cam, const Hit& hit, const GiRes& res, const float4* __restrict__ in, Px p) {
    size_t idx = screen_idx(cam, p.x, p.y);
    float confidence; float3 radiance;
    if (hit_some(hit)) { confidence = res.confidence; radiance = res.w * gi_cosine(res, hit) * res.radiance; }
    else { confidence = 1.0f; radiance = f3s(0.f); }
    float diff_brdf = (1.0f - hit.g.metallic) / kPi;
    float3 spec = gi_spec(res, hit);
    size_t i = pix(cam, p.x, p.y);
    cam.gi_diff_samples[i] = f4(radiance * diff_brdf, confidence);
    cam.gi_spec_samples[i] = f4(radiance * spec, confidence);
    gi_store(gi_load(in, idx), cam.gi_reservoirs[0], idx);
}
__global__ void ST_LB_GI_RESOLVING k_gi_resolving(KPARAMS, int cur, const float4* __restrict__ in) {
    Px p = pixel_full(cam);
    if (!p.in) return;
    Hit hit = load_hit_lut(sc, cam.curr, cam.prim_gbuffer_d0[cur], cam.prim_gbuffer_d1[cur], cam, p.x, p.y);
    gi_resolving_px(cam, hit, gi_load(cam.gi_reservoirs[0], screen_idx(cam, p.x, p.y)), in, p);
}
__global__ void ST_LB_GI_PREVIEW k_gi_preview_resolve(KPARAMS, int cur, u32 seed, const float4* __restrict__ in, const float4* __restrict__ source) {
    Px p = pixel_full(cam);
    if (!p.in) return;
    Hit chit = load_hit_lut(sc, cam.curr, cam.prim_gbuffer_d0[cur], cam.prim_gbuffer_d1[cur], cam, p.x, p.y);
    GiRes r;
    if (!gi_preview_px(cam, sc, chit, seed, 1u, in, p, &r)) r = gi_load(cam.gi_reservoirs[0], screen_idx(cam, p.x, p.y));
    gi_resolving_px(cam, chit, r, source, p);
}

#if ST_EXACT_ONLY
__global__ void __launch_bounds__(ST_BLOCK) k_denoise_reproject(KPARAMS, int cur, const float4* __restrict__ prev_colors, const float4* __restrict__ prev_moments,
                                                                const float4* __restrict__ samples, float4* __restrict__ colors, float4* __restrict__ moments) {
    Px p = pixel_full(cam);
    if (!p.in) return;
    size_t i = pix(cam, p.x, p.y);
    float4 sample = samples[i];
    if (cam.prim_surface_map[cur][i].z == 0.0f) { store4m(cam, colors + i, sample, p.y, ST_REACH_SVGF); return; }
    float sl = luma(xyz(sample));
    Reproj rp = reproj_decode(cam.reprojection_map[i]);
    float3 color, moment;
    if (reproj_some(rp) && sample.w > 0.0f) {
        float4 pc = history_fetch(rp, prev_colors, cam.w, cam.h);
        float4 pm = history_fetch(rp, prev_moments, cam.w, cam.h);
        float hist = rmin(pm.x + 1.0f, 16.0f);
        float alpha = 1.0f / hist;
        color = lerpc(xyz(pc), xyz(sample), alpha);
        moment = f3(hist, lerpc(pm.y, sl, alpha), lerpc(pm.z, sl * sl, alpha));
    } else { color = xyz(sample); moment = f3(1.0f, sl, sl * sl); }
    store4m(cam, colors + i, f4(color, 0.0f), p.y, ST_REACH_SVGF);
    store4m(cam, moments + i, f4(moment, 0.0f), p.y, ST_REACH_SVGF);
}

struct ReprojectSignal { const float4* prev_colors; const float4* prev_moments; const float4* samples; float4* colors; float4* moments; };
ST_DEV void denoise_reproject_signal(const CameraDev& cam, size_t i, u32 y, float4 sample, const Reproj& rp, bool has_rp, const ReprojectSignal& g) {
    float sl = luma(xyz(sample));
    float3 color, moment;
    if (has_rp && sample.w > 0.0f) {
        float4 pc = history_fetch(rp, g.prev_colors, cam.w, cam.h);
        float4 pm = history_fetch(rp, g.prev_moments, cam.w, cam.h);
        float hist = rmin(pm.x + 1.0f, 16.0f);
        float alpha = 1.0f / hist;
        color = lerpc(xyz(pc), xyz(sample), alpha);
        moment = f3(hist, lerpc(pm.y, sl, alpha), lerpc(pm.z, sl * sl, alpha));
    } else { color = xyz(sample); moment = f3(1.0f, sl, sl * sl); }
    store4m(cam, g.colors + i, f4(color, 0.0f), y, ST_REACH_SVGF);
    store4m(cam, g.moments + i, f4(moment, 0.0f), y, ST_REACH_SVGF);
}
__global__ void __launch_bounds__(ST_BLOCK) k_denoise_reproject_pair(KPARAMS, int cur, const __grid_constant__ ReprojectSignal di, const __grid_constant__ ReprojectSignal gi) {
    Px p = pixel_full(cam);
    if (!p.in) return;
    size_t i = pix(cam, p.x, p.y);
    float4 sd = di.samples[i], sg = gi.samples[i];
    if (cam.prim_surface_map[cur][i].z == 0.0f) { store4m(cam, di.colors + i, sd, p.y, ST_REACH_SVGF); store4m(cam, gi.colors + i, sg, p.y, ST_REACH_SVGF); return; }
    Reproj rp = reproj_decode(cam.reprojection_map[i]);
    bool has_rp = reproj_some(rp);
    denoise_reproject_signal(cam, i, p.y, sd, rp, has_rp, di);
    denoise_reproject_signal(cam, i, p.y, sg, rp, has_rp, gi);
}

ST_DEV float sfu_ex2(float x) { float r; asm("ex2.approx.ftz.f32 %0, %1;" : "=f"(r) : "f"(x)); return r; }
ST_DEV float sfu_sqrt(float x) { float r; asm("sqrt.approx.ftz.f32 %0, %1;" : "=f"(r) : "f"(x)); return r; }
ST_DEV float sfu_rcp(float x) { float r; asm("rcp.approx.ftz.f32 %0, %1;" : "=f"(r) : "f"(x)); return r; }
template <bool FAST> ST_DEV float sv_sqrt(float x) { return FAST ? sfu_sqrt(x) : sqrtf(x); }
template <bool FAST> ST_DEV float sv_luma(float3 c) { return FAST ? __fmaf_rn(c.z, 0.0722f, __fmaf_rn(c.y, 0.7152f, c.x * 0.2126f)) : luma(c); }
template <bool FAST> ST_DEV float svgf_depth_weight(float c_depth, float s_depth, float depth_sigma) {
    float leeway = c_depth * depth_sigma;
    float diff = fabs_(s_depth - c_depth);
    if (diff >= leeway) return 0.0f;
    return FAST ? __fmaf_rn(-diff, sfu_rcp(leeway), 1.0f) : 1.0f - diff / leeway;
}
template <bool FAST> ST_DEV float svgf_normal_weight(float3 c_normal, float3 s_normal) {
    float d = FAST ? __fmaf_rn(s_normal.z, c_normal.z, __fmaf_rn(s_normal.y, c_normal.y, s_normal.x * c_normal.x)) : dot(s_normal, c_normal);
    return pow_det(rmax(d, 0.0f), 64.0f);
}
template <bool FAST> ST_DEV float svgf_luma_weight(float sqrt_center_luma, float sample_luma, float luma_sigma) {
    float lw = fabs_(sqrt_center_luma - sv_sqrt<FAST>(sample_luma)) * luma_sigma;
    return FAST ? sfu_ex2(lw * -1.44269504088896341f) : exp_det(-lw);
}

template <bool FAST>
__global__ void __launch_bounds__(ST_BLOCK) k_denoise_variance(KPARAMS, int cur) {
    Px p = pixel_full(cam);
    if (!p.in) return;
    size_t i = pix(cam, p.x, p.y);
    const float4* __restrict__ snd = cam.surface_nd;
    const float4* __restrict__ di_colors = cam.di_diff_curr_colors; const float4* __restrict__ gi_colors = cam.gi_diff_curr_colors;
    float4 cnd = snd[i];
    float4 cdi = di_colors[i], cgi = gi_colors[i];
    if (cnd.w == 0.0f) { cam.di_diff_stash[i] = cdi; cam.gi_diff_stash[i] = cgi; return; }
    float4 mdi = cam.di_diff_moments[cur][i], mgi = cam.gi_diff_moments[cur][i];
    float di_var, gi_var;
    if (mdi.x >= 4.0f) { di_var = mdi.z - sq(mdi.y); gi_var = mgi.z - sq(mgi.y); }
    else {
        float3 cn = xyz(cnd);
        float scdl = sv_sqrt<FAST>(sv_luma<FAST>(xyz(cdi))), scgl = sv_sqrt<FAST>(sv_luma<FAST>(xyz(cgi)));
        float3 sdi = f3s(0.f), sgi = f3s(0.f);
        int ox = -2, oy = -2;
        for (;;) {
            int sx = (int)p.x + ox, sy = (int)p.y + oy;
            if (cam_contains_i(cam.curr, sx, sy)) {
                size_t si = pix(cam, (u32)sx, (u32)sy);
                float4 nds = snd[si];
                if (nds.w != 0.0f) {
                    float common = svgf_depth_weight<FAST>(cnd.w, nds.w, 0.2f);
                    float nw = svgf_normal_weight<FAST>(cn, xyz(nds));
                    float sl = sv_luma<FAST>(xyz(di_colors[si]));
                    float w = svgf_luma_weight<FAST>(scdl, sl, 1.0f) * common * nw;
                    sdi = sdi + f3(sl, sl * sl, 1.0f) * f3s(w);
                    float gl = sv_luma<FAST>(xyz(gi_colors[si]));
                    float wg = svgf_luma_weight<FAST>(scgl, gl, 1.0f) * common * nw;
                    sgi = sgi + f3(gl, gl * gl, 1.0f) * f3s(wg);
                }
            }
            ox += 1;
            if (ox == 3) { ox = -3; oy += 1; if (oy == 3) break; }
        }
        { float m1 = sdi.x / sdi.z, m2 = sdi.y / sdi.z; di_var = fabs_(m2 - m1 * m1) * 4.0f; }
        { float m1 = sgi.x / sgi.z, m2 = sgi.y / sgi.z; gi_var = fabs_(m2 - m1 * m1) * 4.0f; }
    }
    di_var = rmax(di_var, 0.0f); gi_var = rmax(gi_var, 0.0f);
    cam.di_diff_stash[i] = f4(xyz(cdi), di_var);
    cam.gi_diff_stash[i] = f4(xyz(cgi), gi_var);
}

#ifndef ST_WAVELET_MIN_BLOCKS
#define ST_WAVELET_MIN_BLOCKS 10
#endif
template <bool FAST, bool PAIR_IN>
__global__ void __launch_bounds__(ST_BLOCK, ST_WAVELET_MIN_BLOCKS) k_denoise_wavelet(KPARAMS, int cur, u32 frame, u32 stride, float strength,
                                                              const float4* __restrict__ di_in, float4* __restrict__ di_out,
                                                              const float4* __restrict__ gi_in, float4* __restrict__ gi_out,
                                                              const float4* __restrict__ pair_in, float4* __restrict__ pair_out) {
    Px p = pixel_full(cam);
    if (!p.in) return;
    size_t i = pix(cam, p.x, p.y);
    const float4* __restrict__ snd = cam.surface_nd;
    float4 cnd = snd[i];
    float4 cdi, cgi;
    if (PAIR_IN) { F8 c = ld8(pair_in + 2 * i); cdi = c.a; cgi = c.b; } else cdi = di_in[i];
    float3 cdc = xyz(cdi); float cdv = cdi.w;
    if (cnd.w == 0.0f) { if (pair_out) pair_out[2 * i] = f4(cdc, cdv); else di_out[i] = f4(cdc, cdv); return; }
    float4 bn = blue_noise(sc, p.x, p.y, frame);
    if (!PAIR_IN) cgi = gi_in[i];
    float3 cgc = xyz(cgi); float cgv = cgi.w;
    float3 cn = xyz(cnd);
    float scdl = sv_sqrt<FAST>(sv_luma<FAST>(cdc)), scgl = sv_sqrt<FAST>(sv_luma<FAST>(cgc));
    float ls_di = lerpc(2.5f, 0.5f, sv_sqrt<FAST>(cdv));
    float ls_gi = lerpc(1.0f, 0.0f, sv_sqrt<FAST>(cgv));
    float depth_sigma = 0.33f / strength;
    float2 jf = (f2(bn.z, bn.w) - f2(0.5f, 0.5f)) * ((float)stride - 1.0f) * 0.5f;
    int jx = to_i32_sat(jf.x), jy = to_i32_sat(jf.y);
    float sdw = 1.0f; float3 sdc = cdc; float sdv = cdv;
    float sgw = 1.0f; float3 sgc = cgc; float sgv = cgv;
#pragma unroll
    for (int oy = -1; oy <= 1; oy++) {
#pragma unroll
        for (int ox = -1; ox <= 1; ox++) {
            if (ox == 0 && oy == 0) continue;
            int sx = (int)p.x + jx + ox * (int)stride, sy = (int)p.y + jy + oy * (int)stride;
            if (!cam_contains_i(cam.curr, sx, sy)) continue;
            size_t si = pix(cam, (u32)sx, (u32)sy);
            float4 nds = snd[si];
            if (nds.w == 0.0f) continue;
            float dw = svgf_depth_weight<FAST>(cnd.w, nds.w, depth_sigma);
            float nw = svgf_normal_weight<FAST>(cn, xyz(nds));
            if (dw == 0.0f || nw == 0.0f) continue;
            float dnw = dw * nw;
            float4 sdi, sgi;
            if (PAIR_IN) { F8 t = ld8(pair_in + 2 * si); sdi = t.a; sgi = t.b; } else { sdi = di_in[si]; sgi = gi_in[si]; }
            if (FAST) {
                float wd = svgf_luma_weight<true>(scdl, sv_luma<true>(xyz(sdi)), ls_di) * dnw;
                if (wd > 0.0f) { sdw += wd; sdc = f3(__fmaf_rn(wd, sdi.x, sdc.x), __fmaf_rn(wd, sdi.y, sdc.y), __fmaf_rn(wd, sdi.z, sdc.z)); sdv = __fmaf_rn(wd * wd, sdi.w, sdv); }
                float wg = svgf_luma_weight<true>(scgl, sv_luma<true>(xyz(sgi)), ls_gi) * dnw;
                if (wg > 0.0f) { sgw += wg; sgc = f3(__fmaf_rn(wg, sgi.x, sgc.x), __fmaf_rn(wg, sgi.y, sgc.y), __fmaf_rn(wg, sgi.z, sgc.z)); sgv = __fmaf_rn(wg * wg, sgi.w, sgv); }
            } else {
                float wd = svgf_luma_weight<false>(scdl, luma(xyz(sdi)), ls_di) * dw * nw;
                if (wd > 0.0f) { sdw += wd; sdc = sdc + wd * xyz(sdi); sdv += sq(wd) * sdi.w; }
                float wg = svgf_luma_weight<false>(scgl, luma(xyz(sgi)), ls_gi) * dw * nw;
                if (wg > 0.0f) { sgw += wg; sgc = sgc + wg * xyz(sgi); sgv += sq(wg) * sgi.w; }
            }
        }
    }
    float4 odi, ogi;
    if (FAST) {
        float rd = sfu_rcp(sdw), rg = sfu_rcp(sgw);
        odi = f4(sdc * rd, sdv * (rd * rd));
        ogi = f4(sgc * rg, sgv * (rg * rg));
    } else {
        odi = f4(sdc / sdw, sdv / (sdw * sdw));
        ogi = f4(sgc / sgw, sgv / (sgw * sgw));
    }
    if (pair_out) st8(pair_out + 2 * i, odi, ogi);
    else { di_out[i] = odi; gi_out[i] = ogi; }
}

ST_DEV u32 smem_addr(const void* p) { return (u32)__cvta_generic_to_shared(p); }
ST_DEV void mbar_init(u32 bar, u32 count) { asm volatile("mbarrier.init.shared::cta.b64 [%0], %1;" ::"r"(bar), "r"(count) : "memory"); }
ST_DEV void mbar_fence_init() { asm volatile("fence.mbarrier_init.release.cluster;" ::: "memory"); }
ST_DEV void mbar_expect_tx(u32 bar, u32 bytes) { asm volatile("mbarrier.arrive.expect_tx.shared::cta.b64 _, [%0], %1;" ::"r"(bar), "r"(bytes) : "memory"); }
ST_DEV bool mbar_try_wait(u32 bar, u32 parity) {
    u32 ok;
    asm volatile("{\n\t.reg .pred p;\n\tmbarrier.try_wait.parity.shared::cta.b64 p, [%1], %2;\n\tselp.u32 %0, 1, 0, p;\n\t}" : "=r"(ok) : "r"(bar), "r"(parity) : "memory");
    return ok != 0u;
}
ST_DEV void tma_load_2d(u32 dst, const CUtensorMap* tm, int c0, int c1, u32 bar) {
    asm volatile("cp.async.bulk.tensor.2d.shared::cluster.global.mbarrier::complete_tx::bytes [%0], [%1, {%2, %3}], [%4];"
                 ::"r"(dst), "l"(reinterpret_cast<unsigned long long>(tm)), "r"(c0), "r"(c1), "r"(bar) : "memory");
}

template <bool FAST> struct WaveletCentre {
    float3 n; float depth, leeway, rcp_leeway, scdl, scgl, ls_di, ls_gi;
    float sdw; float3 sdc; float sdv; float sgw; float3 sgc; float sgv;
    ST_DEV void init(float4 cnd, float4 cdi, float4 cgi, float depth_sigma) {
        n = xyz(cnd); depth = cnd.w; leeway = cnd.w * depth_sigma; rcp_leeway = FAST ? sfu_rcp(leeway) : 0.0f;
        float3 cdc = xyz(cdi), cgc = xyz(cgi);
        scdl = sv_sqrt<FAST>(sv_luma<FAST>(cdc)); scgl = sv_sqrt<FAST>(sv_luma<FAST>(cgc));
        ls_di = lerpc(2.5f, 0.5f, sv_sqrt<FAST>(cdi.w)); ls_gi = lerpc(1.0f, 0.0f, sv_sqrt<FAST>(cgi.w));
        sdw = 1.0f; sdc = cdc; sdv = cdi.w; sgw = 1.0f; sgc = cgc; sgv = cgi.w;
    }
    ST_DEV bool geometry(float4 nds, float* dw, float* nw) const {
        float diff = fabs_(nds.w - depth);
        if (diff >= leeway) return false;
        *dw = FAST ? __fmaf_rn(-diff, rcp_leeway, 1.0f) : 1.0f - diff / leeway;
        *nw = svgf_normal_weight<FAST>(n, xyz(nds));
        return !(*dw == 0.0f || *nw == 0.0f);
    }
    ST_DEV void add(float dw, float nw, float4 sdi, float4 sgi) {
        if (FAST) {
            float dnw = dw * nw;
            float wd = svgf_luma_weight<true>(scdl, sv_luma<true>(xyz(sdi)), ls_di) * dnw;
            if (wd > 0.0f) { sdw += wd; sdc = f3(__fmaf_rn(wd, sdi.x, sdc.x), __fmaf_rn(wd, sdi.y, sdc.y), __fmaf_rn(wd, sdi.z, sdc.z)); sdv = __fmaf_rn(wd * wd, sdi.w, sdv); }
            float wg = svgf_luma_weight<true>(scgl, sv_luma<true>(xyz(sgi)), ls_gi) * dnw;
            if (wg > 0.0f) { sgw += wg; sgc = f3(__fmaf_rn(wg, sgi.x, sgc.x), __fmaf_rn(wg, sgi.y, sgc.y), __fmaf_rn(wg, sgi.z, sgc.z)); sgv = __fmaf_rn(wg * wg, sgi.w, sgv); }
        } else {
            float wd = svgf_luma_weight<false>(scdl, luma(xyz(sdi)), ls_di) * dw * nw;
            if (wd > 0.0f) { sdw += wd; sdc = sdc + wd * xyz(sdi); sdv += sq(wd) * sdi.w; }
            float wg = svgf_luma_weight<false>(scgl, luma(xyz(sgi)), ls_gi) * dw * nw;
            if (wg > 0.0f) { sgw += wg; sgc = sgc + wg * xyz(sgi); sgv += sq(wg) * sgi.w; }
        }
    }
    ST_DEV void store(float4* __restrict__ di_out, float4* __restrict__ gi_out, float4* __restrict__ pair_out, size_t i) const {
        float4 odi, ogi;
        if (FAST) {
            float rd = sfu_rcp(sdw), rg = sfu_rcp(sgw);
            odi = f4(sdc * rd, sdv * (rd * rd));
            ogi = f4(sgc * rg, sgv * (rg * rg));
        } else {
            odi = f4(sdc / sdw, sdv / (sdw * sdw));
            ogi = f4(sgc / sgw, sgv / (sgw * sgw));
        }
        if (pair_out) st8(pair_out + 2 * i, odi, ogi);
        else { di_out[i] = odi; gi_out[i] = ogi; }
    }
};

template <int S, int J, int TW, int TH> struct WaveletTile {
    static constexpr int HL = S + J, BW = TW + 2 * HL, BH = TH + 2 * HL;
    static constexpr u32 BOX_BYTES = (u32)(BW * BH * 16);
    static constexpr u32 PLANE = (BOX_BYTES + 127u) & ~127u;
    static constexpr u32 SMEM = 3u * PLANE + 128u;
};

#ifndef ST_WAVELET_TILED_MINB
#define ST_WAVELET_TILED_MINB 1
#endif
template <bool FAST, int S, int J, int TW, int TH>
__global__ void __launch_bounds__(TW * TH, (TW * TH <= 256 && S <= 8) ? ST_WAVELET_TILED_MINB : 1) k_denoise_wavelet_tiled(KPARAMS, u32 frame, float strength,
                                                                   const __grid_constant__ CUtensorMap tm_nd, const __grid_constant__ CUtensorMap tm_di,
                                                                   const __grid_constant__ CUtensorMap tm_gi,
                                                                   float4* __restrict__ di_out, float4* __restrict__ gi_out, float4* __restrict__ pair_out,
                                                                   u32* __restrict__ errors) {
    typedef WaveletTile<S, J, TW, TH> T;
    extern __shared__ unsigned char s_raw[];
    __shared__ __align__(8) unsigned long long s_bar;
    const int tx = (int)threadIdx.x % TW, ty = (int)threadIdx.x / TW;
    const int x0 = (int)blockIdx.x * TW, y0 = cam.y0 + (int)blockIdx.y * TH;
    const u32 bar = smem_addr(&s_bar);
    const u32 raw = smem_addr(s_raw);
    const u32 base = (raw + 127u) & ~127u;
    if (threadIdx.x == 0) { mbar_init(bar, 1u); mbar_fence_init(); }
    __syncthreads();
    if (threadIdx.x == 0) {
        mbar_expect_tx(bar, 3u * T::BOX_BYTES);
        tma_load_2d(base, &tm_nd, (x0 - T::HL) * 2, y0 - T::HL, bar);
        tma_load_2d(base + T::PLANE, &tm_di, (x0 - T::HL) * 2, y0 - T::HL, bar);
        tma_load_2d(base + 2u * T::PLANE, &tm_gi, (x0 - T::HL) * 2, y0 - T::HL, bar);
    }
    const u32 px = (u32)(x0 + tx), py = (u32)(y0 + ty);
    const bool in = px < (u32)cam.w && py < (u32)cam.y1;
    int jo = 0;
    if (J > 0 && in) {
        float4 bn = blue_noise(sc, px, py, frame);
        float2 jf = (f2(bn.z, bn.w) - f2(0.5f, 0.5f)) * ((float)S - 1.0f) * 0.5f;
        jo = to_i32_sat(jf.y) * T::BW + to_i32_sat(jf.x);
    }
    {
        bool done = false;
        for (u32 spin = 0; spin < (1u << 20) && !done; spin++) done = mbar_try_wait(bar, 0u);
        if (!done) { if (threadIdx.x == 0) atomicAdd(errors, 1u); return; }
    }
    if (!in) return;
    const float4* __restrict__ t_nd = reinterpret_cast<const float4*>(s_raw + (base - raw));
    const float4* __restrict__ t_di = reinterpret_cast<const float4*>(s_raw + (base - raw) + T::PLANE);
    const float4* __restrict__ t_gi = reinterpret_cast<const float4*>(s_raw + (base - raw) + 2u * T::PLANE);
    const int c = (ty + T::HL) * T::BW + (tx + T::HL);
    const size_t i = pix(cam, px, py);
    float4 cnd = t_nd[c];
    float4 cdi = t_di[c];
    if (cnd.w == 0.0f) { if (pair_out) pair_out[2 * i] = f4(xyz(cdi), cdi.w); else di_out[i] = f4(xyz(cdi), cdi.w); return; }
    WaveletCentre<FAST> ctr;
    ctr.init(cnd, cdi, t_gi[c], 0.33f / strength);
    const int cj = c + jo;
#pragma unroll
    for (int oy = -1; oy <= 1; oy++) {
#pragma unroll
        for (int ox = -1; ox <= 1; ox++) {
            if (ox == 0 && oy == 0) continue;
            const int k = cj + oy * S * T::BW + ox * S;
            float4 nds = t_nd[k];
            if (nds.w == 0.0f) continue;
            float dw, nw;
            if (!ctr.geometry(nds, &dw, &nw)) continue;
            ctr.add(dw, nw, t_di[k], t_gi[k]);
        }
    }
    ctr.store(di_out, gi_out, pair_out, i);
}

ST_DEV float3 compose_px(const CameraDev& cam, const SceneDev& sc, int cur, u32 mode, const float4* __restrict__ di_diff, const float4* __restrict__ gi_diff, size_t i) {
    float3 color;
    if (mode == 0u) {
        GBuf g = gbuf_unpack(sc, cam.prim_gbuffer_d0[cur][i], cam.prim_gbuffer_d1[cur][i]);
        float3 dd = xyz(di_diff[i]), ds = xyz(cam.di_spec_samples[i]), gd = xyz(gi_diff[i]), gs = xyz(cam.gi_spec_samples[i]);
        if (g.depth != 0.0f) color = g.emissive + (dd + gd) * xyz(g.base_color) + ds + gs;
        else color = dd;
    } else if (mode == 1u) color = xyz(di_diff[i]);
    else if (mode == 2u) color = xyz(cam.di_spec_samples[i]);
    else if (mode == 3u) color = xyz(gi_diff[i]);
    else if (mode == 4u) color = xyz(cam.gi_spec_samples[i]);
    else if (mode == 5u) color = xyz(cam.ref_colors[i]);
    else if (mode == 6u) { float4 c = cam.ref_colors[i]; color = xyz(c) / c.w; }
    else color = f3s(0.f);
    return color;
}
__global__ void __launch_bounds__(ST_BLOCK) k_composition(KPARAMS, int cur, u32 mode, const float4* __restrict__ di_diff, const float4* __restrict__ gi_diff) {
    Px p = pixel_full(cam);
    if (!p.in) return;
    size_t i = pix(cam, p.x, p.y);
    cam.output[i] = f4(compose_px(cam, sc, cur, mode, di_diff, gi_diff, i), 1.0f);
}

#define TAA_TW 32
#define TAA_TH 8
static const float kTaaClipEps = 1e-8f;
ST_DEV float taa_max(float a, float b) { return a > b ? a : b; }
ST_DEV float taa_min(float a, float b) { return a < b ? a : b; }
ST_DEV float3 taa_tonemap(float3 c) { const float d = 1.0f + taa_max(taa_max(c.x, c.y), c.z); return f3(c.x / d, c.y / d, c.z / d); }
ST_DEV float3 taa_untonemap(float3 t) { const float d = 1.0f - taa_max(taa_max(t.x, t.y), t.z); return f3(t.x / d, t.y / d, t.z / d); }
ST_DEV float3 taa_ycocg(float3 c) { return f3((0.25f * c.x + 0.5f * c.y) + 0.25f * c.z, 0.5f * c.x - 0.5f * c.z, (-0.25f * c.x + 0.5f * c.y) - 0.25f * c.z); }
ST_DEV float3 taa_rgb(float3 v) { const float t = v.x - v.z; return f3(t + v.y, v.x + v.z, t - v.y); }
ST_DEV void taa_cr_weights(float f, float w[4]) {
    w[0] = f * (-0.5f + f * (1.0f - 0.5f * f));
    w[1] = 1.0f + (f * f) * (-2.5f + 1.5f * f);
    w[2] = f * (0.5f + f * (2.0f - 1.5f * f));
    w[3] = (f * f) * (-0.5f + 0.5f * f);
}
__global__ void __launch_bounds__(TAA_TW * TAA_TH) k_taa_resolve(KPARAMS, int cur, u32 mode, const float4* __restrict__ di_diff, const float4* __restrict__ gi_diff,
                                                                 const float4* __restrict__ hist_in, float4* __restrict__ hist_out, float4 jit) {
    const int HW = TAA_TW + 2, HH = TAA_TH + 2;
    __shared__ float4 s_t[HW * HH];
    const int bx = (int)blockIdx.x * TAA_TW - 1, by = (int)blockIdx.y * TAA_TH - 1;
    for (int k = threadIdx.x; k < HW * HH; k += TAA_TW * TAA_TH) {
        const int x = min(max(bx + k % HW, 0), cam.w - 1), y = min(max(by + k / HW, 0), cam.h - 1);
        s_t[k] = f4(taa_tonemap(compose_px(cam, sc, cur, mode, di_diff, gi_diff, pix(cam, (u32)x, (u32)y))), 0.0f);
    }
    __syncthreads();
    const int tx = threadIdx.x % TAA_TW, ty = threadIdx.x / TAA_TW;
    const u32 px = blockIdx.x * TAA_TW + tx, py = blockIdx.y * TAA_TH + ty;
    if (px >= (u32)cam.w || py >= (u32)cam.h) return;
    const size_t i = pix(cam, px, py);
    const float3 t = xyz(s_t[(ty + 1) * HW + tx + 1]);
    float3 lo = taa_ycocg(xyz(s_t[ty * HW + tx])), hi = lo;
#pragma unroll
    for (int k = 1; k < 9; k++) {
        const float3 v = taa_ycocg(xyz(s_t[(ty + k / 3) * HW + tx + k % 3]));
        lo = f3(taa_min(lo.x, v.x), taa_min(lo.y, v.y), taa_min(lo.z, v.z)); hi = f3(taa_max(hi.x, v.x), taa_max(hi.y, v.y), taa_max(hi.z, v.z));
    }
    const float W = cam.curr.screen.x, H = cam.curr.screen.y;
    float2 q; bool ok = true;
    if (cam.prim_gbuffer_d0[cur][i].x != 0.0f) {
        const float4 v = cam.velocity_map[i];
        q = f2((((float)px + 0.5f) - v.x) - (jit.x - jit.z), (((float)py + 0.5f) - v.y) - (jit.y - jit.w));
    } else {
        const float sx = ((float)px + 0.5f) - jit.x, sy = ((float)py + 0.5f) - jit.y;
        const float nx = sx * 2.0f / W - 1.0f, ny = -(sy * 2.0f / H - 1.0f);
        const float3 far_plane = project_point(cam_n2w(cam.curr), f3(nx, ny, kF32Eps)), near_plane = project_point(cam_n2w(cam.curr), f3(nx, ny, 1.0f));
        const float4 clip = mat_mul(cam_pv(cam.prev), f4(norm(far_plane - near_plane), 0.0f));
        const float2 s = cam_clip_to_screen(cam.prev, clip);
        q = f2(s.x + jit.z, s.y + jit.w);
        ok = clip.w > 0.0f;
    }
    ok = ok && q.x >= 0.0f && q.y >= 0.0f && q.x < W && q.y < H;
    float n = 0.0f;
    if (ok) n = hist_in[pix(cam, (u32)floorf(q.x), (u32)floorf(q.y))].w;
    float3 h = t;
    if (n > 0.0f) {
        const float ux = q.x - 0.5f, uy = q.y - 0.5f, fx0 = floorf(ux), fy0 = floorf(uy);
        float wx[4], wy[4];
        taa_cr_weights(ux - fx0, wx); taa_cr_weights(uy - fy0, wy);
        const int ix = (int)fx0 - 1, iy = (int)fy0 - 1;
        h = f3s(0.0f);
#pragma unroll
        for (int j = 0; j < 4; j++) {
            const u32 yy = (u32)min(max(iy + j, 0), cam.h - 1);
            float3 row = f3s(0.0f);
#pragma unroll
            for (int k = 0; k < 4; k++) row = row + wx[k] * xyz(hist_in[pix(cam, (u32)min(max(ix + k, 0), cam.w - 1), yy)]);
            h = h + wy[j] * row;
        }
        const float3 c = 0.5f * (hi + lo), e = 0.5f * (hi - lo) + f3s(kTaaClipEps);
        const float3 d = taa_ycocg(h) - c;
        const float m = taa_max(taa_max(fabs_(d.x / e.x), fabs_(d.y / e.y)), fabs_(d.z / e.z));
        if (m > 1.0f) h = taa_rgb(c + d / m);
    } else n = 0.0f;
    const float a = 1.0f / (n + 1.0f), alpha = a > 0.1f ? a : 0.1f;
    const float3 r = (1.0f - alpha) * h + alpha * t;
    const float n1 = n + 1.0f;
    hist_out[i] = f4(r, n1 < 16.0f ? n1 : 16.0f);
    cam.output[i] = f4(taa_untonemap(r), 1.0f);
}


__global__ void __launch_bounds__(ST_BLOCK) k_output_rgba8(KPARAMS, uchar4* __restrict__ out) {
    Px p = pixel_full(cam);
    if (!p.in) return;
    size_t i = pix(cam, p.x, p.y);
    float4 c = cam.output[i];
    float v[3] = {c.x, c.y, c.z};
    u32 q[3];
#pragma unroll
    for (int k = 0; k < 3; k++) {
        float x = sat(v[k]);
        float e = (x <= 0.0031308f) ? 12.92f * x : 1.055f * pow_det(x, 1.0f / 2.4f) - 0.055f;
        q[k] = to_u32_sat(sat(e) * 255.0f + 0.5f);
    }
    out[i] = make_uchar4((unsigned char)q[0], (unsigned char)q[1], (unsigned char)q[2], 255);
}

template <bool NMAP>
__global__ void __launch_bounds__(ST_BLOCK) k_ref_tracing(KPARAMS, u32 depth) {
    ST_TRACE_STACK();
    Px p = pixel_full(cam);
    if (!p.in) return;
    size_t idx = screen_idx(cam, p.x, p.y);
    Ray ray;
    if (depth == 0u) ray = cam_ray(cam.curr, p.x, p.y);
    else {
        float4 d0 = cam.ref_rays[3 * idx], d1 = cam.ref_rays[3 * idx + 1];
        if (all_zero(d1)) return;
        ray = ray_make(xyz(d0), xyz(d1));
    }
    TriHit h = trace_closest(ray, sc, stk);
    if (NMAP && trihit_some(h)) h.normal = nmap_normal(sc, h, ldg4(&sc.materials[h.material_id].normal_map_texture));
    float4 h0, h1; trihit_pack(h, &h0, &h1);
    cam.ref_hits[2 * idx] = h0; cam.ref_hits[2 * idx + 1] = h1;
}

template <bool LGRID, bool TEXF>
__global__ void __launch_bounds__(ST_BLOCK) k_ref_shading(KPARAMS, u32 seed, u32 depth, const __grid_constant__ LightGridDev lg,
                                                          const __grid_constant__ TexFilterDev tf) {
    ST_TRACE_STACK();
    Px p = pixel_full(cam);
    if (!p.in) return;
    size_t idx = screen_idx(cam, p.x, p.y);
    Rng rng = rng_make(seed, p.x, p.y);
    float4* rays = cam.ref_rays;
    if (depth == 255u) {
        size_t i = pix(cam, p.x, p.y);
        float4 prev = cam_is_eq(cam.curr, cam.prev) ? cam.ref_colors[i] : f4zero();
        cam.ref_colors[i] = prev + f4(xyz(rays[3 * idx + 2]), 1.0f);
        return;
    }
    Ray ray; float3 color, thr;
    if (depth == 0u) { ray = cam_ray(cam.curr, p.x, p.y); color = f3s(0.f); thr = f3s(1.0f); }
    else {
        float4 d0 = rays[3 * idx], d1 = rays[3 * idx + 1], d2 = rays[3 * idx + 2];
        if (all_zero(d1)) return;
        ray = ray_make(xyz(d0), xyz(d1)); color = xyz(d2); thr = f3(d0.w, d1.w, d2.w);
    }
    TriHit th = trihit_unpack(cam.ref_hits[2 * idx], cam.ref_hits[2 * idx + 1]);
    if (!trihit_some(th)) {
        color = color + thr * atmosphere_sample(sc, world_sun_dir(sc.world), ray.d);
        rays[3 * idx] = f4zero(); rays[3 * idx + 1] = f4zero(); rays[3 * idx + 2] = f4(color, 0.0f);
        return;
    }
    GpuMaterial m = sc.materials[th.material_id];
    if (depth > 0u) m.roughness = rmax(m.roughness, 0.75f * 0.75f);
    Hit hit;
    hit.point = th.point + th.normal * 0.01f; hit.origin = ray.o; hit.dir = ray.d;
    if (TEXF) {
        const TriHit again = trace_closest(ray, sc, stk);
        uncount_ray(sc);
        TexFoot ft; ft.tri = again.triangle_id; ft.dir = ray.d; ft.w = texf_cone_width(cam.curr, p.x, p.y, again.t, depth == 0u);
        hit.g.base_color = texf_sample(sc, tf, th.material_id, 0u, m.base_color_texture, m.base_color, th.uv, ft);
        hit.g.emissive = xyz(texf_sample(sc, tf, th.material_id, 1u, m.emissive_texture, m.emissive, th.uv, ft));
    } else { hit.g.base_color = mat_base_color(sc, m, th.uv); hit.g.emissive = mat_emissive(sc, m, th.uv); }
    hit.g.normal = th.normal; hit.g.metallic = m.metallic;
    hit.g.roughness = m.roughness; hit.g.reflectance = m.reflectance; hit.g.depth = 0.0f;
    color = color + thr * hit.g.emissive;
    const LgList list = LGRID ? lgrid_list(lg, hit.point) : LgList{nullptr, sc.world.light_count};
    if (list.n > 0u) {
        u32 lid = lgrid_pick(list, rng_u32(rng) % list.n);
        float lpdf = 1.0f / (float)list.n;
        GpuLight light = light_load(sc, lid);
        bool occ = trace_any(light_ray_wnoise(light, rng, hit.point), sc, stk);
        if (!occ) color = color + thr * lightrad_sum(light_radiance(light, hit)) / lpdf;
// ... 220 lines not shown
            float dt = nt - t; t = nt;
            float3 np = pos + t * rd;
            float3 rs, ext; float ms; atm_scattering(np, &rs, &ms, &ext);
            float3 st_ = exp3(-dt * ext);
            float3 snp = rs + f3s(ms);
            float3 sf = (snp - snp * st_) / ext;
            lf = lf + tr * sf;
            float3 sun_t = atm_lut(tl, 256, 64, np, sun_dir);
            float3 ri = rs * rp;
            float mi = ms * mp;
            float3 ins = (ri + f3s(mi)) * sun_t;
            float3 si = (ins - ins * st_) / ext;
            lum = lum + si * tr;
            tr = tr * st_;
        }
        if (gdist > 0.0f) {
            float3 hp = pos + gdist * rd;
            if (dot(pos, sun_dir) > 0.0f) {
                hp = norm(hp) * ST_ATM_GROUND;
                lum = lum + tr * f3s(0.25f) * atm_lut(tl, 256, 64, hp, sun_dir);
            }
        }
        fms = fms + lf * inv_samples;
        lum_total = lum_total + lum * inv_samples;
    }
    float3 o = lum_total / (f3s(1.0f) - fms);
    out[y * 32 + x] = f4(round_f16(o.x), round_f16(o.y), round_f16(o.z), 1.0f);
}
__global__ void k_atm_sky(const float4* __restrict__ tl, const float4* __restrict__ sl, float sun_altitude, float4* __restrict__ out) {
    int x = threadIdx.x, y = blockIdx.x;
    float2 uv = f2((float)x, (float)y) / f2(256.0f, 256.0f);
    float azimuth = (uv.x - 0.5f) * 2.0f * kPi;
    float v;
    if (uv.y < 0.5f) { float c = 1.0f - 2.0f * uv.y; v = -c * c; }
    else { float c = uv.y * 2.0f - 1.0f; v = c * c; }
    float3 vp = atm_view_pos();
    float height = len(vp);
    float horizon;
    { float t = sq(height) - sq(ST_ATM_GROUND); t = sqrtf(t) / height; horizon = acos_det(rclamp(t, -1.0f, 1.0f)) - 0.5f * kPi; }
    float altitude = v * 0.5f * kPi - horizon;
    float sa, ca, sz, cz; sincos_det(altitude, &sa, &ca); sincos_det(azimuth, &sz, &cz);
    float3 rd = f3(ca * sz, sa, -ca * cz);
    float sal = fmodf(sun_altitude, 2.0f * kPi);
    float ss, cs_; sincos_det(sal, &ss, &cs_);
    float3 sun_dir = (sal < 0.5f * kPi) ? f3(0.0f, ss, -cs_) : f3(0.0f, ss, cs_);
    float adist = ray_sphere(ray_make(vp, rd), ST_ATM_TOP);
    float gdist = ray_sphere(ray_make(vp, rd), ST_ATM_GROUND);
    float t_max = (gdist < 0.0f) ? adist : gdist;
    float ct = dot(rd, sun_dir);
    float mp = atm_mie_phase(ct), rp = atm_rayleigh_phase(-ct);
    float3 lum = f3s(0.f), tr = f3s(1.0f);
    float t = 0.0f;
    for (float i = 0.0f; i < 32.0f; i += 1.0f) {
        float nt = ((i + 0.3f) / 32.0f) * t_max;
        float dt = nt - t; t = nt;
        float3 np = vp + t * rd;
        float3 rs, ext; float ms; atm_scattering(np, &rs, &ms, &ext);
        float3 st_ = exp3(-dt * ext);
        float3 sun_t = atm_lut(tl, 256, 64, np, sun_dir);
        float3 psi = atm_lut(sl, 32, 32, np, sun_dir);
        float3 ri = rs * (rp * sun_t + psi);
        float3 mi = ms * (mp * sun_t + psi);
        float3 ins = ri + mi;
        float3 si = (ins - ins * st_) / ext;
        lum = lum + si * tr;
        tr = tr * st_;
    }
    out[y * 256 + x] = f4(round_f16(lum.x), round_f16(lum.y), round_f16(lum.z), 1.0f);
}

#endif

__global__ void k_math_shading(int op, const float* __restrict__ a, const float* __restrict__ b, float* __restrict__ out, long n) {
    long i = (long)blockIdx.x * blockDim.x + threadIdx.x;
    if (i >= n) return;
    float r = 0.f, x = a[i], y = b[i];
    switch (op) {
        case 0: r = sin_det(x); break; case 1: r = cos_det(x); break; case 2: r = exp_det(x); break;
        case 3: r = pow_det(x, y); break; case 4: r = sqrtf(x); break; case 5: r = x / y; break;
    }
    out[i] = r;
}

static dim3 grid_full(const CameraDev& cam) { return dim3((cam.w + TILE_W - 1) / TILE_W, (cam.y1 - cam.y0 + TILE_H - 1) / TILE_H); }
static dim3 grid_half(const CameraDev& cam) { int hw = 8 * (((cam.w + 7) / 8) / 2); return dim3((hw + TILE_W - 1) / TILE_W, (cam.y1 - cam.y0 + TILE_H - 1) / TILE_H); }
#define HALF_LAUNCH(kernel, c, st, ...) do { dim3 g_ = grid_half(c); if (g_.x > 0 && g_.y > 0) kernel<<<g_, ST_BLOCK, 0, st>>>(__VA_ARGS__); } while (0)

void launch_di_sampling(const CameraDev& c, const SceneDev& s, int cur, u32 seed, u32 frame, const LightGridDev* lg, cudaStream_t st) {
    if (lg) k_di_sampling<true><<<grid_full(c), ST_BLOCK, 0, st>>>(c, s, cur, seed, frame, *lg); else k_di_sampling<false><<<grid_full(c), ST_BLOCK, 0, st>>>(c, s, cur, seed, frame, LightGridDev{});
}
void launch_di_temporal(const CameraDev& c, const SceneDev& s, int cur, u32 seed, cudaStream_t st) { k_di_temporal<<<grid_full(c), ST_BLOCK, 0, st>>>(c, s, cur, seed); }
void launch_di_spatial_pick(const CameraDev& c, const SceneDev& s, int cur, u32 seed, u32 frame, cudaStream_t st) { HALF_LAUNCH(k_di_spatial_pick, c, st, c, s, cur, seed, frame); }
void launch_spatial_trace(const CameraDev& c, const SceneDev& s, const float4* d0, const float4* d1, float4* d2, cudaStream_t st) { k_spatial_trace<<<grid_full(c), ST_BLOCK, 0, st>>>(c, s, d0, d1, d2); }
void launch_di_spatial_sample(const CameraDev& c, const SceneDev& s, u32 seed, u32 frame, cudaStream_t st) { HALF_LAUNCH(k_di_spatial_sample, c, st, c, s, seed, frame); }
void launch_di_resolving(const CameraDev& c, const SceneDev& s, int cur, cudaStream_t st) { k_di_resolving<<<grid_full(c), ST_BLOCK, 0, st>>>(c, s, cur); }
void launch_gi_reprojection(const CameraDev& c, const SceneDev& s, int cur, cudaStream_t st) { k_gi_reprojection<<<grid_full(c), ST_BLOCK, 0, st>>>(c, s, cur); }
void launch_gi_sampling_a(const CameraDev& c, const SceneDev& s, int cur, u32 seed, u32 frame, bool nmap, const TexFilterDev* tf, cudaStream_t st) {
    if (tf) {
        if (nmap) HALF_LAUNCH((k_gi_sampling_a<true, true>), c, st, c, s, cur, seed, frame, *tf); else HALF_LAUNCH((k_gi_sampling_a<false, true>), c, st, c, s, cur, seed, frame, *tf);
    } else {
        const TexFilterDev none{};
        if (nmap) HALF_LAUNCH((k_gi_sampling_a<true, false>), c, st, c, s, cur, seed, frame, none); else HALF_LAUNCH((k_gi_sampling_a<false, false>), c, st, c, s, cur, seed, frame, none);
    }
}
void launch_gi_sampling_b(const CameraDev& c, const SceneDev& s, int cur, u32 seed, u32 frame, const LightGridDev* lg, cudaStream_t st) {
    if (lg) HALF_LAUNCH(k_gi_sampling_b<true>, c, st, c, s, cur, seed, frame, *lg); else HALF_LAUNCH(k_gi_sampling_b<false>, c, st, c, s, cur, seed, frame, LightGridDev{});
}
void launch_gi_temporal(const CameraDev& c, const SceneDev& s, int cur, u32 seed, u32 frame, int inline_reprojection, cudaStream_t st) { k_gi_temporal<<<grid_full(c), ST_BLOCK, 0, st>>>(c, s, cur, seed, frame, inline_reprojection); }
void launch_gi_spatial_pick(const CameraDev& c, const SceneDev& s, int cur, u32 seed, u32 frame, cudaStream_t st) { HALF_LAUNCH(k_gi_spatial_pick, c, st, c, s, cur, seed, frame); }
void launch_gi_spatial_sample(const CameraDev& c, const SceneDev& s, u32 seed, u32 frame, cudaStream_t st) { HALF_LAUNCH(k_gi_spatial_sample, c, st, c, s, seed, frame); }
void launch_gi_preview(const CameraDev& c, const SceneDev& s, int cur, u32 seed, u32 nth, const float4* in, float4* out, int mirror_reach, cudaStream_t st) { k_gi_preview<<<grid_full(c), ST_BLOCK, 0, st>>>(c, s, cur, seed, nth, in, out, mirror_reach); }
void launch_gi_resolving(const CameraDev& c, const SceneDev& s, int cur, const float4* in, cudaStream_t st) { k_gi_resolving<<<grid_full(c), ST_BLOCK, 0, st>>>(c, s, cur, in); }
void launch_di_sample_temporal(const CameraDev& c, const SceneDev& s, int cur, u32 seed_sampling, u32 seed_temporal, u32 frame, const LightGridDev* lg, cudaStream_t st) {
    if (lg) k_di_sample_temporal<true><<<grid_full(c), ST_BLOCK, 0, st>>>(c, s, cur, seed_sampling, seed_temporal, frame, *lg);
    else k_di_sample_temporal<false><<<grid_full(c), ST_BLOCK, 0, st>>>(c, s, cur, seed_sampling, seed_temporal, frame, LightGridDev{});
}
void launch_di_spatial_fused(const CameraDev& c, const SceneDev& s, int cur, u32 seed_pick, u32 seed_sample, u32 frame, cudaStream_t st) { HALF_LAUNCH(k_di_spatial_fused, c, st, c, s, cur, seed_pick, seed_sample, frame); }
void launch_gi_sampling_fused(const CameraDev& c, const SceneDev& s, int cur, u32 seed_a, u32 seed_b, u32 frame, bool nmap, const LightGridDev* lg, const TexFilterDev* tf,
                              cudaStream_t st) {
    const LightGridDev none{};
    const LightGridDev& g = lg ? *lg : none;
    const TexFilterDev tnone{};
    const TexFilterDev& t = tf ? *tf : tnone;
#define ST_GSF(N_, L_, T_) HALF_LAUNCH((k_gi_sampling_fused<N_, L_, T_>), c, st, c, s, cur, seed_a, seed_b, frame, g, t)
    if (tf) {
        if (lg) { if (nmap) ST_GSF(true, true, true); else ST_GSF(false, true, true); }
        else { if (nmap) ST_GSF(true, false, true); else ST_GSF(false, false, true); }
    } else {
        if (lg) { if (nmap) ST_GSF(true, true, false); else ST_GSF(false, true, false); }
        else { if (nmap) ST_GSF(true, false, false); else ST_GSF(false, false, false); }
    }
#undef ST_GSF
}
void launch_gi_spatial_fused(const CameraDev& c, const SceneDev& s, int cur, u32 seed_pick, u32 seed_sample, u32 frame, cudaStream_t st) { HALF_LAUNCH(k_gi_spatial_fused, c, st, c, s, cur, seed_pick, seed_sample, frame); }
void launch_gi_preview_resolve(const CameraDev& c, const SceneDev& s, int cur, u32 seed, const float4* in, const float4* source, cudaStream_t st) { k_gi_preview_resolve<<<grid_full(c), ST_BLOCK, 0, st>>>(c, s, cur, seed, in, source); }
void launch_math_shading(int op, const float* a, const float* b, float* out, long n, cudaStream_t st) { k_math_shading<<<(unsigned)((n + 255) / 256), 256, 0, st>>>(op, a, b, out, n); }
#if ST_EXACT_ONLY
void launch_prim_gbuffer(const CameraDev& c, const SceneDev& s, int cur, int with_reprojection, bool nmap, const TexFilterDev* tf, cudaStream_t st) {
    const TexFilterDev none{};
    const TexFilterDev& t = tf ? *tf : none;
#define ST_PG(N_, T_) k_prim_gbuffer<N_, T_><<<grid_full(c), ST_BLOCK, 0, st>>>(c, s, cur, with_reprojection, t)
    if (tf) { if (nmap) ST_PG(true, true); else ST_PG(false, true); }
    else { if (nmap) ST_PG(true, false); else ST_PG(false, false); }
#undef ST_PG
}
void launch_frame_reprojection(const CameraDev& c, const SceneDev& s, int cur, cudaStream_t st) { k_frame_reprojection<<<grid_full(c), ST_BLOCK, 0, st>>>(c, s, cur); }
void launch_denoise_reproject(const CameraDev& c, const SceneDev& s, int cur, const float4* pc, const float4* pm, const float4* smp, float4* col, float4* mom, cudaStream_t st) { k_denoise_reproject<<<grid_full(c), ST_BLOCK, 0, st>>>(c, s, cur, pc, pm, smp, col, mom); }
void launch_denoise_reproject_pair(const CameraDev& c, const SceneDev& s, int cur, cudaStream_t st) {
    ReprojectSignal di{c.di_diff_prev_colors, c.di_diff_moments[cur ^ 1], c.di_diff_samples, c.di_diff_curr_colors, c.di_diff_moments[cur]};
    ReprojectSignal gi{c.gi_diff_prev_colors, c.gi_diff_moments[cur ^ 1], c.gi_diff_samples, c.gi_diff_curr_colors, c.gi_diff_moments[cur]};
    k_denoise_reproject_pair<<<grid_full(c), ST_BLOCK, 0, st>>>(c, s, cur, di, gi);
}
void launch_denoise_variance(const CameraDev& c, const SceneDev& s, int cur, bool fast, cudaStream_t st) {
    if (fast) k_denoise_variance<true><<<grid_full(c), ST_BLOCK, 0, st>>>(c, s, cur); else k_denoise_variance<false><<<grid_full(c), ST_BLOCK, 0, st>>>(c, s, cur);
}
void launch_denoise_wavelet(const CameraDev& c, const SceneDev& s, int cur, u32 frame, u32 stride, float strength, const float4* di_in, float4* di_out, const float4* gi_in, float4* gi_out,
                            const float4* pair_in, float4* pair_out, bool fast, cudaStream_t st) {
#define ST_WG(F_, P_) k_denoise_wavelet<F_, P_><<<grid_full(c), ST_BLOCK, 0, st>>>(c, s, cur, frame, stride, strength, di_in, di_out, gi_in, gi_out, pair_in, pair_out)
    if (pair_in) { if (fast) ST_WG(true, true); else ST_WG(false, true); }
    else { if (fast) ST_WG(true, false); else ST_WG(false, false); }
#undef ST_WG
}
template <int TW, int TH> struct VarianceTile {
    static constexpr int HX = 3, HY = 2, BW = TW + 2 * HX, BH = TH + 2 * HY;
    static constexpr u32 BOX_BYTES = (u32)(BW * BH * 16);
    static constexpr u32 PLANE = (BOX_BYTES + 127u) & ~127u;
    static constexpr u32 SMEM = 3u * PLANE + 128u;
};
template <bool FAST, int TW, int TH>
__global__ void __launch_bounds__(TW * TH) k_denoise_variance_tiled(KPARAMS, int cur, const __grid_constant__ CUtensorMap tm_nd, const __grid_constant__ CUtensorMap tm_di,
                                                                    const __grid_constant__ CUtensorMap tm_gi, u32* __restrict__ errors) {
    typedef VarianceTile<TW, TH> T;
    extern __shared__ unsigned char s_raw[];
    __shared__ __align__(8) unsigned long long s_bar;
    const int tx = (int)threadIdx.x % TW, ty = (int)threadIdx.x / TW;
    const int x0 = (int)blockIdx.x * TW, y0 = cam.y0 + (int)blockIdx.y * TH;
    const u32 bar = smem_addr(&s_bar);
    const u32 raw = smem_addr(s_raw);
    const u32 base = (raw + 127u) & ~127u;
    if (threadIdx.x == 0) { mbar_init(bar, 1u); mbar_fence_init(); }
    __syncthreads();
    if (threadIdx.x == 0) {
        mbar_expect_tx(bar, 3u * T::BOX_BYTES);
        tma_load_2d(base, &tm_nd, (x0 - T::HX) * 2, y0 - T::HY, bar);
        tma_load_2d(base + T::PLANE, &tm_di, (x0 - T::HX) * 2, y0 - T::HY, bar);
        tma_load_2d(base + 2u * T::PLANE, &tm_gi, (x0 - T::HX) * 2, y0 - T::HY, bar);
    }
    const u32 px = (u32)(x0 + tx), py = (u32)(y0 + ty);
    const bool in = px < (u32)cam.w && py < (u32)cam.y1;
    const size_t i = in ? pix(cam, px, py) : 0;
    float4 mdi = f4zero(), mgi = f4zero();
    if (in) { mdi = cam.di_diff_moments[cur][i]; mgi = cam.gi_diff_moments[cur][i]; }
    {
        bool done = false;
        for (u32 spin = 0; spin < (1u << 20) && !done; spin++) done = mbar_try_wait(bar, 0u);
        if (!done) { if (threadIdx.x == 0) atomicAdd(errors, 1u); return; }
    }
    if (!in) return;
    const float4* __restrict__ t_nd = reinterpret_cast<const float4*>(s_raw + (base - raw));
    const float4* __restrict__ t_di = reinterpret_cast<const float4*>(s_raw + (base - raw) + T::PLANE);
    const float4* __restrict__ t_gi = reinterpret_cast<const float4*>(s_raw + (base - raw) + 2u * T::PLANE);
    const int c = (ty + T::HY) * T::BW + (tx + T::HX);
    float4 cnd = t_nd[c];
    float4 cdi = t_di[c], cgi = t_gi[c];
    if (cnd.w == 0.0f) { cam.di_diff_stash[i] = cdi; cam.gi_diff_stash[i] = cgi; return; }
    float di_var, gi_var;
    if (mdi.x >= 4.0f) { di_var = mdi.z - sq(mdi.y); gi_var = mgi.z - sq(mgi.y); }
    else {
        float3 cn = xyz(cnd);
        float scdl = sv_sqrt<FAST>(sv_luma<FAST>(xyz(cdi))), scgl = sv_sqrt<FAST>(sv_luma<FAST>(xyz(cgi)));
        float3 sdi = f3s(0.f), sgi = f3s(0.f);
#pragma unroll
        for (int oy = -2; oy <= 2; oy++) {
#pragma unroll
            for (int ox = -3; ox <= 2; ox++) {
                if (oy == -2 && ox == -3) continue;
                const int k = c + oy * T::BW + ox;
                float4 nds = t_nd[k];
                if (nds.w != 0.0f) {
                    float common = svgf_depth_weight<FAST>(cnd.w, nds.w, 0.2f);
                    float nw = svgf_normal_weight<FAST>(cn, xyz(nds));
                    float sl = sv_luma<FAST>(xyz(t_di[k]));
                    float w = svgf_luma_weight<FAST>(scdl, sl, 1.0f) * common * nw;
                    sdi = sdi + f3(sl, sl * sl, 1.0f) * f3s(w);
                    float gl = sv_luma<FAST>(xyz(t_gi[k]));
                    float wg = svgf_luma_weight<FAST>(scgl, gl, 1.0f) * common * nw;
                    sgi = sgi + f3(gl, gl * gl, 1.0f) * f3s(wg);
                }
            }
        }
        { float m1 = sdi.x / sdi.z, m2 = sdi.y / sdi.z; di_var = fabs_(m2 - m1 * m1) * 4.0f; }
        { float m1 = sgi.x / sgi.z, m2 = sgi.y / sgi.z; gi_var = fabs_(m2 - m1 * m1) * 4.0f; }
    }
    di_var = rmax(di_var, 0.0f); gi_var = rmax(gi_var, 0.0f);
    cam.di_diff_stash[i] = f4(xyz(cdi), di_var);
    cam.gi_diff_stash[i] = f4(xyz(cgi), gi_var);
}

typedef CUresult (*TensorMapEncodeFn)(CUtensorMap*, CUtensorMapDataType, cuuint32_t, void*, const cuuint64_t*, const cuuint64_t*, const cuuint32_t*,
                                      const cuuint32_t*, CUtensorMapInterleave, CUtensorMapSwizzle, CUtensorMapL2promotion, CUtensorMapFloatOOBfill);
static TensorMapEncodeFn tensor_map_encoder() {
    static TensorMapEncodeFn fn = [] {
        void* p = nullptr; cudaDriverEntryPointQueryResult q = cudaDriverEntryPointSymbolNotFound;
        if (cudaGetDriverEntryPoint("cuTensorMapEncodeTiled", &p, cudaEnableDefault, &q) != cudaSuccess || q != cudaDriverEntryPointSuccess) p = nullptr;
        return (TensorMapEncodeFn)p;
    }();
    return fn;
}
static bool wavelet_tensor_map(const float4* plane, int w, int h, int bw, int bh, CUtensorMap* out) {
    typedef std::tuple<const void*, int, int, int, int> Key;
    static std::map<Key, CUtensorMap> cache; static std::mutex mu;
    std::lock_guard<std::mutex> lock(mu);
    Key key(plane, w, h, bw, bh);
    auto it = cache.find(key);
    if (it != cache.end()) { *out = it->second; return true; }
    TensorMapEncodeFn enc = tensor_map_encoder();
    if (!enc) {
        static bool warned = false;
        if (!warned) { warned = true; std::fprintf(stderr, "strolle_b200: cuTensorMapEncodeTiled is not available from this driver; the tile-staged SVGF kernels are off\n"); }
        return false;
    }
    cuuint64_t dims[2] = {(cuuint64_t)w * 2u, (cuuint64_t)h};
    cuuint64_t strides[1] = {(cuuint64_t)w * 16u};
    cuuint32_t box[2] = {(cuuint32_t)bw * 2u, (cuuint32_t)bh};
    cuuint32_t estr[2] = {1u, 1u};
    CUtensorMap tm;
    if (enc(&tm, CU_TENSOR_MAP_DATA_TYPE_UINT64, 2, const_cast<float4*>(plane), dims, strides, box, estr, CU_TENSOR_MAP_INTERLEAVE_NONE,
            CU_TENSOR_MAP_SWIZZLE_NONE, CU_TENSOR_MAP_L2_PROMOTION_L2_256B, CU_TENSOR_MAP_FLOAT_OOB_FILL_NONE) != CUDA_SUCCESS) return false;
    if (cache.size() > 4096) cache.clear();
    cache[key] = tm; *out = tm;
    return true;
}
template <bool FAST, int S, int J, int TW, int TH>
static bool wavelet_tiled_go(const CameraDev& c, const SceneDev& s, u32 frame, float strength, const float4* di_in, float4* di_out, const float4* gi_in, float4* gi_out,
                             float4* pair_out, u32* errors, cudaStream_t st) {
    typedef WaveletTile<S, J, TW, TH> T;
    if (T::BW * 2 > 256 || T::BH > 256) return false;
    CUtensorMap tn, td, tg;
    if (!wavelet_tensor_map(c.surface_nd, c.w, c.h, T::BW, T::BH, &tn) || !wavelet_tensor_map(di_in, c.w, c.h, T::BW, T::BH, &td) ||
        !wavelet_tensor_map(gi_in, c.w, c.h, T::BW, T::BH, &tg)) return false;
    auto kern = k_denoise_wavelet_tiled<FAST, S, J, TW, TH>;
    static bool attr_set[64] = {};
    int dev = 0; cudaGetDevice(&dev); dev &= 63;
    if (!attr_set[dev]) { if (cudaFuncSetAttribute(kern, cudaFuncAttributeMaxDynamicSharedMemorySize, (int)T::SMEM) != cudaSuccess) { cudaGetLastError(); return false; } attr_set[dev] = true; }
    dim3 grid((c.w + TW - 1) / TW, (c.y1 - c.y0 + TH - 1) / TH);
    kern<<<grid, TW * TH, T::SMEM, st>>>(c, s, frame, strength, tn, td, tg, di_out, gi_out, pair_out, errors);
    return true;
}
template <bool FAST, int S, int J>
static bool wavelet_tiled_cfg(int cfg, const CameraDev& c, const SceneDev& s, u32 frame, float strength, const float4* di_in, float4* di_out, const float4* gi_in, float4* gi_out,
                              float4* pair_out, u32* errors, cudaStream_t st) {
    switch (cfg) {
    case 0: return wavelet_tiled_go<FAST, S, J, 32, 8>(c, s, frame, strength, di_in, di_out, gi_in, gi_out, pair_out, errors, st);
    case 1: return wavelet_tiled_go<FAST, S, J, 32, 16>(c, s, frame, strength, di_in, di_out, gi_in, gi_out, pair_out, errors, st);
    case 2: return wavelet_tiled_go<FAST, S, J, 64, 4>(c, s, frame, strength, di_in, di_out, gi_in, gi_out, pair_out, errors, st);
    case 3: return wavelet_tiled_go<FAST, S, J, 64, 8>(c, s, frame, strength, di_in, di_out, gi_in, gi_out, pair_out, errors, st);
    default: return false;
    }
}
bool launch_denoise_wavelet_tiled(const CameraDev& c, const SceneDev& s, u32 frame, u32 stride, float strength, const float4* di_in, float4* di_out, const float4* gi_in,
                                  float4* gi_out, float4* pair_out, bool fast, int cfg, u32* errors, cudaStream_t st) {
    if (c.curr.screen.x != (float)c.w || c.curr.screen.y != (float)c.h) return false;
#define ST_WT(S_, J_) (fast ? wavelet_tiled_cfg<true, S_, J_>(cfg, c, s, frame, strength, di_in, di_out, gi_in, gi_out, pair_out, errors, st) \
                            : wavelet_tiled_cfg<false, S_, J_>(cfg, c, s, frame, strength, di_in, di_out, gi_in, gi_out, pair_out, errors, st))
    switch (stride) {
    case 1: return ST_WT(1, 0);
    case 2: return ST_WT(2, 0);
    case 4: return ST_WT(4, 0);
    case 8: return ST_WT(8, 1);
    case 16: return ST_WT(16, 3);
    default: return false;
    }
#undef ST_WT
}
template <bool FAST>
static bool variance_tiled_go(const CameraDev& c, const SceneDev& s, int cur, u32* errors, cudaStream_t st) {
    typedef VarianceTile<32, 8> T;
    CUtensorMap tn, td, tg;
    if (!wavelet_tensor_map(c.surface_nd, c.w, c.h, T::BW, T::BH, &tn) || !wavelet_tensor_map(c.di_diff_curr_colors, c.w, c.h, T::BW, T::BH, &td) ||
        !wavelet_tensor_map(c.gi_diff_curr_colors, c.w, c.h, T::BW, T::BH, &tg)) return false;
    auto kern = k_denoise_variance_tiled<FAST, 32, 8>;
    static bool attr_set[64] = {};
    int dev = 0; cudaGetDevice(&dev); dev &= 63;
    if (!attr_set[dev]) { if (cudaFuncSetAttribute(kern, cudaFuncAttributeMaxDynamicSharedMemorySize, (int)T::SMEM) != cudaSuccess) { cudaGetLastError(); return false; } attr_set[dev] = true; }
    dim3 grid((c.w + 31) / 32, (c.y1 - c.y0 + 7) / 8);
    kern<<<grid, 256, T::SMEM, st>>>(c, s, cur, tn, td, tg, errors);
    return true;
}
bool launch_denoise_variance_tiled(const CameraDev& c, const SceneDev& s, int cur, bool fast, u32* errors, cudaStream_t st) {
    if (c.curr.screen.x != (float)c.w || c.curr.screen.y != (float)c.h) return false;
    return fast ? variance_tiled_go<true>(c, s, cur, errors, st) : variance_tiled_go<false>(c, s, cur, errors, st);
}
void launch_composition(const CameraDev& c, const SceneDev& s, int cur, u32 mode, const float4* di_diff, const float4* gi_diff, cudaStream_t st) { k_composition<<<grid_full(c), ST_BLOCK, 0, st>>>(c, s, cur, mode, di_diff, gi_diff); }
void launch_taa_resolve(const CameraDev& c, const SceneDev& s, int cur, u32 mode, const float4* di_diff, const float4* gi_diff, const float4* hist_in, float4* hist_out,
                        float4 jit, cudaStream_t st) {
    const dim3 grid((c.w + TAA_TW - 1) / TAA_TW, (c.h + TAA_TH - 1) / TAA_TH);
    k_taa_resolve<<<grid, TAA_TW * TAA_TH, 0, st>>>(c, s, cur, mode, di_diff, gi_diff, hist_in, hist_out, jit);
}
void launch_output_rgba8(const CameraDev& c, const SceneDev& s, uchar4* out, cudaStream_t st) { k_output_rgba8<<<grid_full(c), ST_BLOCK, 0, st>>>(c, s, out); }
void launch_ref_tracing(const CameraDev& c, const SceneDev& s, u32 depth, bool nmap, cudaStream_t st) {
    if (nmap) k_ref_tracing<true><<<grid_full(c), ST_BLOCK, 0, st>>>(c, s, depth); else k_ref_tracing<false><<<grid_full(c), ST_BLOCK, 0, st>>>(c, s, depth);
}
void launch_ref_shading(const CameraDev& c, const SceneDev& s, u32 seed, u32 depth, const LightGridDev* lg, const TexFilterDev* tf, cudaStream_t st) {
    const LightGridDev none{};
    const LightGridDev& g = lg ? *lg : none;
    const TexFilterDev tnone{};
    const TexFilterDev& t = tf ? *tf : tnone;
#define ST_RS(L_, T_) k_ref_shading<L_, T_><<<grid_full(c), ST_BLOCK, 0, st>>>(c, s, seed, depth, g, t)
    if (tf) { if (lg) ST_RS(true, true); else ST_RS(false, true); }
    else { if (lg) ST_RS(true, false); else ST_RS(false, false); }
#undef ST_RS
}
cudaError_t launch_texture_mips(const MipJob* jobs, const u32* first, const u32* blocks, int levels, const uchar4* atlas, uchar4* pool, const float* srgb,
                                cudaStream_t st) {
    for (int k = 0; k < levels; k++) {
        if (!blocks[k]) continue;
        for (u32 j = first[k]; j < first[k + 1]; j += 65535u) {
            const u32 n = min(first[k + 1] - j, 65535u);
            k_texture_mips<<<dim3(blocks[k], n), 256, 0, st>>>(jobs + j, atlas, pool, srgb);
            const cudaError_t err = cudaGetLastError();
            if (err != cudaSuccess) return err;
        }
    }
    return cudaSuccess;
}
void launch_bvh_heatmap(const CameraDev& c, const SceneDev& s, cudaStream_t st) { k_bvh_heatmap<<<grid_full(c), ST_BLOCK, 0, st>>>(c, s); }
void launch_trace_stream_closest(const SceneDev& s, const float4* rays, long n, float4* out, cudaStream_t st) { k_trace_stream_closest<<<(unsigned)((n + ST_BLOCK - 1) / ST_BLOCK), ST_BLOCK, 0, st>>>(s, rays, n, out); }
void launch_trace_stream_any(const SceneDev& s, const float4* rays, long n, u32* out, cudaStream_t st) { k_trace_stream_any<<<(unsigned)((n + ST_BLOCK - 1) / ST_BLOCK), ST_BLOCK, 0, st>>>(s, rays, n, out); }
void launch_math(int op, const float* a, const float* b, float* out, long n, cudaStream_t st) {
    if (op == 7) k_math_log2<<<(unsigned)((n + 255) / 256), 256, 0, st>>>(a, out, n); else k_math<<<(unsigned)((n + 255) / 256), 256, 0, st>>>(op, a, b, out, n);
}
void launch_light_grid_build(const LightGridDev& lg, const GpuLight* lights, cudaStream_t st) {
    const u32 ncell = lg.dims[0] * lg.dims[1] * lg.dims[2];
    k_light_grid_build<<<(ncell + 1u + 3u) / 4u, 128, 0, st>>>(lg, lights, ncell, const_cast<u32*>(lg.counts), const_cast<u32*>(lg.lists));
}
void launch_material_derive(const GpuMaterial* mats, u32 n, u32* packed, cudaStream_t st) { if (n) k_material_derive<<<(n + 127) / 128, 128, 0, st>>>(mats, n, packed); }
void launch_srgb_lut(float* lut, cudaStream_t st) { k_srgb_lut<<<1, 256, 0, st>>>(lut); }
void launch_unpack_lut(float* lut, cudaStream_t st) { k_unpack_lut<<<1, 256, 0, st>>>(lut); }
ST_DEV void st_release_sys(u32* p, u32 v) { asm volatile("st.release.sys.global.u32 [%0], %1;" ::"l"(p), "r"(v) : "memory"); }
ST_DEV u32 ld_acquire_sys(const u32* p) { u32 v; asm volatile("ld.acquire.sys.global.u32 %0, [%1];" : "=r"(v) : "l"(p) : "memory"); return v; }
__global__ void __launch_bounds__(32) k_strip_signal(const __grid_constant__ StripSync s, int slot, u32 seq, u32 dst_mask, int* reset_need, int h) {
    __threadfence_system();
    int r = (int)threadIdx.x;
    if (r < s.n_ranks && r != s.rank && ((dst_mask >> r) & 1u) && s.peer_flags[r] != nullptr) st_release_sys(s.peer_flags[r] + slot * ST_PEER_MAX_RANKS + s.rank, seq);
    if (reset_need != nullptr && r == 0) { reset_need[0] = h; reset_need[1] = -1; }
}
__global__ void __launch_bounds__(32) k_strip_wait(const __grid_constant__ StripSync s, int slot, u32 seq, u32 src_mask) {
    int r = (int)threadIdx.x;
    if (r < s.n_ranks && r != s.rank && ((src_mask >> r) & 1u)) {
        const u32* f = s.my_flags + slot * ST_PEER_MAX_RANKS + r;
        long long t0 = clock64();
        while ((int)(ld_acquire_sys(f) - seq) < 0) {
            if (clock64() - t0 > 20000000000ll) {
                atomicAdd(s.errors, 1u); atomicCAS(s.errors + 1, 0u, 0x80000000u | ((u32)slot << 16) | ((u32)r << 8) | (seq & 0xffu)); break;
            }
            __nanosleep(64);
        }
    }
    __threadfence_system();
}
__global__ void __launch_bounds__(256) k_strip_pull(const __grid_constant__ StripPull p) {
    const int lo = max(0, min(p.need_rows[0], p.own_y0)), hi = min(p.h - 1, max(p.need_rows[1], p.own_y1 - 1));
    const StripPullItem it = p.items[blockIdx.y];
    const int have_lo = max(0, p.own_y0 - it.local_rows), have_hi = min(p.h, p.own_y1 + it.local_rows);
    const int up0 = lo, up1 = min(p.own_y0, have_lo), dn0 = max(p.own_y1, have_hi), dn1 = hi + 1;
    const int nup = max(0, up1 - up0), ndn = max(0, dn1 - dn0);
    const unsigned long long per_row = (unsigned long long)p.w * (unsigned long long)it.vec4_per_px;
    const unsigned long long total = (unsigned long long)(nup + ndn) * per_row;
    for (unsigned long long i = (unsigned long long)blockIdx.x * blockDim.x + threadIdx.x; i < total; i += (unsigned long long)gridDim.x * blockDim.x) {
        int ri = (int)(i / per_row);
        unsigned long long col = i - (unsigned long long)ri * per_row;
        int row = ri < nup ? up0 + ri : dn0 + (ri - nup);
        int owner = 0;
        while (owner + 1 < p.n_ranks && row >= p.bounds[owner + 1]) owner++;
        size_t off = it.offset + ((size_t)row * per_row + col) * 16;
        *reinterpret_cast<uint4*>(p.arena[p.rank] + off) = *reinterpret_cast<const uint4*>(p.arena[owner] + off);
    }
    if (blockIdx.x == 0 && blockIdx.y == 0 && threadIdx.x == 0) { int reach = max(0, p.own_y0 - lo) + max(0, hi + 1 - p.own_y1); if (reach > 0) atomicAdd(p.pulled_rows, (unsigned long long)reach); }
}
__global__ void __launch_bounds__(32) k_strip_signal_wait(const __grid_constant__ StripSync s, int sig_slot, u32 seq, u32 dst_mask, int wait_slot, u32 wait_seq, u32 src_mask) {
    __threadfence_system();
    int r = (int)threadIdx.x;
// ... 85 lines not shown
```

### strolle_b200/csrc/kernels.h

```cpp
#pragma once
#include <cuda_runtime.h>
#include "st_types.h"

namespace st {
typedef uint32_t u32;

void launch_prim_gbuffer(const CameraDev& c, const SceneDev& s, int cur, int with_reprojection, bool nmap, const TexFilterDev* tf, cudaStream_t st);
void launch_frame_reprojection(const CameraDev& c, const SceneDev& s, int cur, cudaStream_t st);
void launch_di_sampling(const CameraDev& c, const SceneDev& s, int cur, u32 seed, u32 frame, const LightGridDev* lg, cudaStream_t st);
void launch_di_temporal(const CameraDev& c, const SceneDev& s, int cur, u32 seed, cudaStream_t st);
void launch_di_spatial_pick(const CameraDev& c, const SceneDev& s, int cur, u32 seed, u32 frame, cudaStream_t st);
void launch_spatial_trace(const CameraDev& c, const SceneDev& s, const float4* d0, const float4* d1, float4* d2, cudaStream_t st);
void launch_di_spatial_sample(const CameraDev& c, const SceneDev& s, u32 seed, u32 frame, cudaStream_t st);
void launch_di_resolving(const CameraDev& c, const SceneDev& s, int cur, cudaStream_t st);
void launch_gi_reprojection(const CameraDev& c, const SceneDev& s, int cur, cudaStream_t st);
void launch_gi_sampling_a(const CameraDev& c, const SceneDev& s, int cur, u32 seed, u32 frame, bool nmap, const TexFilterDev* tf, cudaStream_t st);
void launch_gi_sampling_b(const CameraDev& c, const SceneDev& s, int cur, u32 seed, u32 frame, const LightGridDev* lg, cudaStream_t st);
void launch_gi_temporal(const CameraDev& c, const SceneDev& s, int cur, u32 seed, u32 frame, int inline_reprojection, cudaStream_t st);
void launch_gi_spatial_pick(const CameraDev& c, const SceneDev& s, int cur, u32 seed, u32 frame, cudaStream_t st);
void launch_gi_spatial_sample(const CameraDev& c, const SceneDev& s, u32 seed, u32 frame, cudaStream_t st);
void launch_gi_preview(const CameraDev& c, const SceneDev& s, int cur, u32 seed, u32 nth, const float4* in, float4* out, int mirror_reach, cudaStream_t st);
void launch_gi_resolving(const CameraDev& c, const SceneDev& s, int cur, const float4* in, cudaStream_t st);
void launch_di_sample_temporal(const CameraDev& c, const SceneDev& s, int cur, u32 seed_sampling, u32 seed_temporal, u32 frame, const LightGridDev* lg, cudaStream_t st);
void launch_di_spatial_fused(const CameraDev& c, const SceneDev& s, int cur, u32 seed_pick, u32 seed_sample, u32 frame, cudaStream_t st);
void launch_gi_sampling_fused(const CameraDev& c, const SceneDev& s, int cur, u32 seed_a, u32 seed_b, u32 frame, bool nmap, const LightGridDev* lg, const TexFilterDev* tf, cudaStream_t st);
void launch_gi_spatial_fused(const CameraDev& c, const SceneDev& s, int cur, u32 seed_pick, u32 seed_sample, u32 frame, cudaStream_t st);
void launch_gi_preview_resolve(const CameraDev& c, const SceneDev& s, int cur, u32 seed, const float4* in, const float4* source, cudaStream_t st);
void launch_denoise_reproject(const CameraDev& c, const SceneDev& s, int cur, const float4* pc, const float4* pm, const float4* smp, float4* col, float4* mom, cudaStream_t st);
void launch_denoise_reproject_pair(const CameraDev& c, const SceneDev& s, int cur, cudaStream_t st);
void launch_denoise_variance(const CameraDev& c, const SceneDev& s, int cur, bool fast, cudaStream_t st);
void launch_denoise_wavelet(const CameraDev& c, const SceneDev& s, int cur, u32 frame, u32 stride, float strength, const float4* di_in, float4* di_out, const float4* gi_in, float4* gi_out, const float4* pair_in, float4* pair_out, bool fast, cudaStream_t st);
bool launch_denoise_wavelet_tiled(const CameraDev& c, const SceneDev& s, u32 frame, u32 stride, float strength, const float4* di_in, float4* di_out, const float4* gi_in, float4* gi_out, float4* pair_out, bool fast, int cfg, u32* errors, cudaStream_t st);
bool launch_denoise_variance_tiled(const CameraDev& c, const SceneDev& s, int cur, bool fast, u32* errors, cudaStream_t st);
void launch_composition(const CameraDev& c, const SceneDev& s, int cur, u32 mode, const float4* di_diff, const float4* gi_diff, cudaStream_t st);
void launch_taa_resolve(const CameraDev& c, const SceneDev& s, int cur, u32 mode, const float4* di_diff, const float4* gi_diff, const float4* hist_in, float4* hist_out,
                        float4 jit, cudaStream_t st);
void launch_output_rgba8(const CameraDev& c, const SceneDev& s, uchar4* out, cudaStream_t st);
void launch_ref_tracing(const CameraDev& c, const SceneDev& s, u32 depth, bool nmap, cudaStream_t st);
void launch_ref_shading(const CameraDev& c, const SceneDev& s, u32 seed, u32 depth, const LightGridDev* lg, const TexFilterDev* tf, cudaStream_t st);
void launch_bvh_heatmap(const CameraDev& c, const SceneDev& s, cudaStream_t st);
void launch_trace_stream_closest(const SceneDev& s, const float4* rays, long n, float4* out, cudaStream_t st);
void launch_trace_stream_any(const SceneDev& s, const float4* rays, long n, u32* out, cudaStream_t st);
void launch_math(int op, const float* a, const float* b, float* out, long n, cudaStream_t st);
void launch_light_grid_build(const LightGridDev& lg, const GpuLight* lights, cudaStream_t st);
cudaError_t launch_texture_mips(const MipJob* jobs, const u32* first, const u32* blocks, int levels, const uchar4* atlas, uchar4* pool, const float* srgb, cudaStream_t st);
void launch_material_derive(const GpuMaterial* mats, u32 n, u32* packed, cudaStream_t st);
void launch_srgb_lut(float* lut, cudaStream_t st);
void launch_unpack_lut(float* lut, cudaStream_t st);
void launch_atm_transmittance(float4* out, cudaStream_t st);
void launch_atm_scattering(const float4* tl, float4* out, cudaStream_t st);
void launch_atm_sky(const float4* tl, const float4* sl, float sun_altitude, float4* out, cudaStream_t st);

#define ST_PEER_MAX_SEGMENTS 40
#define ST_PEER_MAX_RANKS 16
struct PeerSegment { const uint4* src; uint4* dst; unsigned long long n; };
struct PeerExchange {
    PeerSegment seg[ST_PEER_MAX_SEGMENTS]; int nseg;
    u32* peer_flags[ST_PEER_MAX_RANKS];
    const u32* my_flags;
    u32* counter; u32* errors;
    int n_ranks, rank; u32 seq; int signal;
};
void launch_peer_exchange(const PeerExchange& x, cudaStream_t st);

enum StripSlot { SLOT_FRAME_DONE = 0, SLOT_PULL_DONE = 1, SLOT_DI1 = 2, SLOT_GI1 = 3, SLOT_GI2 = 4, SLOT_GI3 = 5, SLOT_SVGF = 6, SLOT_GBUF = 7, SLOT_COUNT = 8 };
struct StripSync {
    const u32* my_flags;
    u32* peer_flags[ST_PEER_MAX_RANKS];
    u32* errors;
    int n_ranks, rank;
};
struct StripPullItem { size_t offset; int vec4_per_px; int local_rows; };
struct StripPull {
    char* arena[ST_PEER_MAX_RANKS]; int bounds[ST_PEER_MAX_RANKS + 1];
    int n_ranks, rank, w, h, own_y0, own_y1;
    const int* need_rows; unsigned long long* pulled_rows;
    StripPullItem items[12]; int nitems;
};
int preload_kernels();
void launch_strip_signal(const StripSync& s, int slot, u32 seq, u32 dst_mask, int* reset_need, int h, cudaStream_t st);
void launch_strip_wait(const StripSync& s, int slot, u32 seq, u32 src_mask, cudaStream_t st);
void launch_strip_signal_wait(const StripSync& s, int sig_slot, u32 seq, u32 dst_mask, int wait_slot, u32 wait_seq, u32 src_mask, cudaStream_t st);
void launch_strip_pull(const StripPull& p, cudaStream_t st);
void launch_atm_sun_color(float4* out2, const GpuWorld& world, cudaStream_t st);

struct BakeRecord { float xf[12]; float nt[9]; float sign; u32 b, e, first, pad; unsigned long long tris; };
void launch_bake_instances(const BakeRecord* recs, u32 nrec, u32 total, float4* triangles, cudaStream_t st);
void launch_refit(const uint4* runs, u32 nruns, const uint2* nodes, const u32* level_begin, int levels, const float4* triangles, float4* bvh, cudaStream_t st);

}

namespace stf {
using st::CameraDev; using st::SceneDev; using st::LightGridDev; using st::TexFilterDev; using st::u32;
int preload_kernels();
void launch_di_sampling(const CameraDev& c, const SceneDev& s, int cur, u32 seed, u32 frame, const LightGridDev* lg, cudaStream_t st);
void launch_di_temporal(const CameraDev& c, const SceneDev& s, int cur, u32 seed, cudaStream_t st);
void launch_di_spatial_pick(const CameraDev& c, const SceneDev& s, int cur, u32 seed, u32 frame, cudaStream_t st);
void launch_spatial_trace(const CameraDev& c, const SceneDev& s, const float4* d0, const float4* d1, float4* d2, cudaStream_t st);
void launch_di_spatial_sample(const CameraDev& c, const SceneDev& s, u32 seed, u32 frame, cudaStream_t st);
void launch_di_resolving(const CameraDev& c, const SceneDev& s, int cur, cudaStream_t st);
void launch_gi_reprojection(const CameraDev& c, const SceneDev& s, int cur, cudaStream_t st);
void launch_gi_sampling_a(const CameraDev& c, const SceneDev& s, int cur, u32 seed, u32 frame, bool nmap, const TexFilterDev* tf, cudaStream_t st);
void launch_gi_sampling_b(const CameraDev& c, const SceneDev& s, int cur, u32 seed, u32 frame, const LightGridDev* lg, cudaStream_t st);
void launch_gi_temporal(const CameraDev& c, const SceneDev& s, int cur, u32 seed, u32 frame, int inline_reprojection, cudaStream_t st);
void launch_gi_spatial_pick(const CameraDev& c, const SceneDev& s, int cur, u32 seed, u32 frame, cudaStream_t st);
void launch_gi_spatial_sample(const CameraDev& c, const SceneDev& s, u32 seed, u32 frame, cudaStream_t st);
void launch_gi_preview(const CameraDev& c, const SceneDev& s, int cur, u32 seed, u32 nth, const float4* in, float4* out, int mirror_reach, cudaStream_t st);
void launch_gi_resolving(const CameraDev& c, const SceneDev& s, int cur, const float4* in, cudaStream_t st);
void launch_di_sample_temporal(const CameraDev& c, const SceneDev& s, int cur, u32 seed_sampling, u32 seed_temporal, u32 frame, const LightGridDev* lg, cudaStream_t st);
void launch_di_spatial_fused(const CameraDev& c, const SceneDev& s, int cur, u32 seed_pick, u32 seed_sample, u32 frame, cudaStream_t st);
void launch_gi_sampling_fused(const CameraDev& c, const SceneDev& s, int cur, u32 seed_a, u32 seed_b, u32 frame, bool nmap, const LightGridDev* lg, const TexFilterDev* tf, cudaStream_t st);
void launch_gi_spatial_fused(const CameraDev& c, const SceneDev& s, int cur, u32 seed_pick, u32 seed_sample, u32 frame, cudaStream_t st);
void launch_gi_preview_resolve(const CameraDev& c, const SceneDev& s, int cur, u32 seed, const float4* in, const float4* source, cudaStream_t st);
void launch_math_shading(int op, const float* a, const float* b, float* out, long n, cudaStream_t st);
}
```

Baseline: 3729.

## Enable programmatic dependent launch and fold GI reprojection into fused sampling

Most frame kernels now start with griddepcontrol wait/launch_dependents and are launched through a PDL helper. This lets the next kernel's launch overlap the tail of the previous one and hides launch latency. On non-tracing frames with fused passes, the separate GI reprojection step is removed: the fused sampling kernel computes the reprojected reservoir inline, and the temporal kernel stores it using a new mode. The schedule gains joint steps that replace a span of steps. This adds complexity, and because each kernel waits at its very start, the available overlap is limited to launch and prologue.

```diff
diff --git a/strolle_b200/csrc/engine.cu b/strolle_b200/csrc/engine.cu
--- a/strolle_b200/csrc/engine.cu
+++ b/strolle_b200/csrc/engine.cu
@@ -374,7 +374,7 @@
     struct PeerLink { bool ready = false; bool ipc = false; std::vector<char*> arena, rgba8; std::vector<uint32_t*> flags; DevMem sync; uint32_t seq = 0, fseq = 0; } peer;
 };
 
-struct Step { int pass; std::function<void(cudaStream_t)> run; int sub = -1; };
+struct Step { int pass; std::function<void(cudaStream_t)> run; int sub = -1; int span = 1; std::vector<Step> joint; };
 
 }
 
@@ -941,7 +941,7 @@
             const int inline_rp = (fp && tracing) ? 1 : 0;
             if (!inline_rp) add(P_GI_REPROJECTION, [=](cudaStream_t s) { (fs ? stf::launch_gi_reprojection : st::launch_gi_reprojection)(cam, sc, cur, s); });
             auto sampling = [&]() {
-                if (fp) { add(P_GI_SAMPLING_B, [=](cudaStream_t s) { if (nm) e->normal_map_launches++; (fs ? stf::launch_gi_sampling_fused : st::launch_gi_sampling_fused)(cam, sc, cur, sa, sb, f, nm, lgon ? &lgd : nullptr, tfon ? &tfd : nullptr, s); }); return; }
+                if (fp) { add(P_GI_SAMPLING_B, [=](cudaStream_t s) { if (nm) e->normal_map_launches++; (fs ? stf::launch_gi_sampling_fused : st::launch_gi_sampling_fused)(cam, sc, cur, sa, sb, f, nm, lgon ? &lgd : nullptr, tfon ? &tfd : nullptr, 0, s); }); return; }
                 add(P_GI_SAMPLING_A, [=](cudaStream_t s) { if (nm) e->normal_map_launches++; (fs ? stf::launch_gi_sampling_a : st::launch_gi_sampling_a)(cam, sc, cur, sa, f, nm, tfon ? &tfd : nullptr, s); });
                 add(P_GI_SAMPLING_B, [=](cudaStream_t s) { (fs ? stf::launch_gi_sampling_b : st::launch_gi_sampling_b)(cam, sc, cur, sb, f, lgon ? &lgd : nullptr, s); });
             };
@@ -958,8 +958,15 @@
                     source = 1;
                 } else source = 0;
             } else {
+                const size_t k11 = steps->size() - 1;
                 sampling();
                 add(P_GI_TEMPORAL, [=](cudaStream_t s) { (fs ? stf::launch_gi_temporal : st::launch_gi_temporal)(cam, sc, cur, st_, f, 0, s); });
+                if (fp) {
+                    Step& first = (*steps)[k11];
+                    first.span = 3;
+                    first.joint.push_back(Step{P_GI_SAMPLING_B, [=](cudaStream_t s) { if (nm) e->normal_map_launches++; (fs ? stf::launch_gi_sampling_fused : st::launch_gi_sampling_fused)(cam, sc, cur, sa, sb, f, nm, lgon ? &lgd : nullptr, tfon ? &tfd : nullptr, 1, s); }});
+                    first.joint.push_back(Step{P_GI_TEMPORAL, [=](cudaStream_t s) { (fs ? stf::launch_gi_temporal : st::launch_gi_temporal)(cam, sc, cur, st_, f, 2, s); }});
+                }
                 source = 0;
             }
             const float4* src0 = source == 0 ? cam.gi_reservoirs[1] : cam.gi_reservoirs[2];
@@ -1690,7 +1697,11 @@
     if ((rc = ensure_taa_history(e, cs))) return rc;
     std::vector<Step> steps; build_schedule(e, cs, &steps);
     if (last < 0 || last >= (int)steps.size()) last = (int)steps.size() - 1;
-    for (int i = std::max(first, 0); i <= last; i++) e->run_timed(steps[i].pass, steps[i].run, steps[i].sub);
+    for (int i = std::max(first, 0); i <= last; i++) {
+        const Step& st = steps[i];
+        if (st.span > 1 && i + st.span - 1 <= last) { for (const Step& j : st.joint) e->run_timed(j.pass, j.run, j.sub); i += st.span - 1; }
+        else e->run_timed(st.pass, st.run, st.sub);
+    }
     CK(cudaGetLastError());
     return ST_OK;
 }
diff --git a/strolle_b200/csrc/kernels.cu b/strolle_b200/csrc/kernels.cu
--- a/strolle_b200/csrc/kernels.cu
+++ b/strolle_b200/csrc/kernels.cu
@@ -53,6 +53,7 @@
     TraceStack stk; stk.base = s_stack + threadIdx.x;
 
 #define KPARAMS const __grid_constant__ CameraDev cam, const __grid_constant__ SceneDev sc
+#define ST_GRID_DEP() do { asm volatile("griddepcontrol.wait;" ::: "memory"); asm volatile("griddepcontrol.launch_dependents;" ::: "memory"); } while (0)
 
 #define ST_LB_N(N) __launch_bounds__(ST_BLOCK, N)
 #if !defined(ST_MINB_ALL)
@@ -127,6 +128,7 @@
 ST_DEV float4 frame_reprojection_px(const CameraDev& cam, int cur, Px p, float4 surface_texel, float4 vel);
 template <bool NMAP, bool TEXF>
 __global__ void ST_LB_PRIM_GBUFFER k_prim_gbuffer(KPARAMS, int cur, int with_reprojection, const __grid_constant__ TexFilterDev tf) {
+    ST_GRID_DEP();
     ST_TRACE_STACK();
     Px p = pixel_full(cam);
     if (!p.in) return;
@@ -199,6 +201,7 @@
     return reproj_encode(rp);
 }
 __global__ void __launch_bounds__(ST_BLOCK) k_frame_reprojection(KPARAMS, int cur) {
+    ST_GRID_DEP();
     Px p = pixel_full(cam);
     if (!p.in) return;
     size_t i = pix(cam, p.x, p.y);
@@ -222,6 +225,7 @@
 }
 template <bool LGRID>
 __global__ void ST_LB_DI_SAMPLING k_di_sampling(KPARAMS, int cur, u32 seed, u32 frame, const __grid_constant__ LightGridDev lg) {
+    ST_GRID_DEP();
     ST_TRACE_STACK();
     Px p = pixel_full(cam);
     if (!p.in) return;
@@ -267,6 +271,7 @@
     return main_;
 }
 __global__ void ST_LB_DI_TEMPORAL k_di_temporal(KPARAMS, int cur, u32 seed) {
+    ST_GRID_DEP();
     Px p = pixel_full(cam);
     if (!p.in) return;
     size_t lhs_idx = screen_idx(cam, p.x, p.y);
@@ -276,6 +281,7 @@
 }
 template <bool LGRID>
 __global__ void ST_LB_DI_SAMPLING k_di_sample_temporal(KPARAMS, int cur, u32 seed_sampling, u32 seed_temporal, u32 frame, const __grid_constant__ LightGridDev lg) {
+    ST_GRID_DEP();
     ST_TRACE_STACK();
     Px p = pixel_full(cam);
     if (!p.in) return;
@@ -333,6 +339,7 @@
     tex_store(buf_d1, cam, ax, g.y, o.a1); tex_store(buf_d1, cam, bx, g.y, o.b1);
 }
 __global__ void ST_LB_DI_SPATIAL_PICK k_di_spatial_pick(KPARAMS, int cur, u32 seed, u32 frame) {
+    ST_GRID_DEP();
     Px g = pixel_half(cam);
     if (!g.in) return;
     store_pair_texels(cam, di_spatial_pick_pair(cam, sc, cur, seed, frame, g), cam.di_diff_samples, cam.di_diff_curr_colors, g);
@@ -345,6 +352,7 @@
     return f4(occ ? 0.0f : 1.0f, d1.z, d1.w, 0.0f);
 }
 __global__ void ST_LB_SPATIAL_TRACE k_spatial_trace(KPARAMS, const float4* __restrict__ buf_d0, const float4* __restrict__ buf_d1, float4* __restrict__ buf_d2) {
+    ST_GRID_DEP();
     ST_TRACE_STACK();
     Px p = pixel_full(cam);
     if (!p.in) return;
@@ -386,11 +394,13 @@
     if (cam_contains_u(cam.curr, op.x, op.y)) { size_t oi = screen_idx(cam, op.x, op.y); di_store(di_load(in, oi), out, oi); }
 }
 __global__ void __launch_bounds__(ST_BLOCK) k_di_spatial_sample(KPARAMS, u32 seed, u32 frame) {
+    ST_GRID_DEP();
     Px g = pixel_half(cam);
     if (!g.in) return;
     di_spatial_sample_pair(cam, seed, frame, g, tex_or_zero(cam.di_diff_stash, cam, g.x * 2u, g.y), tex_or_zero(cam.di_diff_stash, cam, g.x * 2u + 1u, g.y));
 }
 __global__ void ST_LB_DI_SPATIAL_PICK k_di_spatial_fused(KPARAMS, int cur, u32 seed_pick, u32 seed_sample, u32 frame) {
+    ST_GRID_DEP();
     ST_TRACE_STACK();
     Px g = pixel_half(cam);
     if (!g.in) return;
@@ -401,6 +411,7 @@
 }
 
 __global__ void ST_LB_DI_RESOLVING k_di_resolving(KPARAMS, int cur) {
+    ST_GRID_DEP();
     ST_TRACE_STACK();
     Px p = pixel_full(cam);
     if (!p.in) return;
@@ -441,6 +452,7 @@
     return res;
 }
 __global__ void __launch_bounds__(ST_BLOCK) k_gi_reprojection(KPARAMS, int cur) {
+    ST_GRID_DEP();
     Px p = pixel_full(cam);
     if (!p.in) return;
     Hit hit = load_hit_lut(sc, cam.curr, cam.prim_gbuffer_d0[cur], cam.prim_gbuffer_d1[cur], cam, p.x, p.y);
@@ -451,7 +463,7 @@
 
 template <bool NMAP, bool TEXF>
 ST_DEV bool gi_sampling_a_pair(const CameraDev& cam, const SceneDev& sc, const TraceStack& stk, int cur, u32 seed, u32 frame, Px g, float4* t0, float4* t1, float4* t2,
-                               const TexFilterDev& tf) {
+                               const TexFilterDev& tf, const GiRes* k11 = nullptr) {
     bool tracing = gi_tracing_frame(frame);
     uint2 sp = tracing ? checker(g.x, g.y, frame / 2u) : checker(g.x, g.y, frame);
     if (!cam_contains_u(cam.curr, sp.x, sp.y)) return false;
@@ -465,7 +477,7 @@
         gi_r = ray_make(hit.point, s.dir);
         gi_pdf_ = s.pdf;
     } else {
-        GiRes res = gi_load(cam.gi_reservoirs[2], idx);
+        GiRes res = k11 ? *k11 : gi_load(cam.gi_reservoirs[2], idx);
         if (res.m == 0.0f) return false;
         gi_r = ray_make(res.v1, gi_dir(res, res.v1));
         gi_pdf_ = 1.0f;
@@ -493,6 +505,7 @@
 }
 template <bool NMAP, bool TEXF>
 __global__ void ST_LB_GI_SAMPLING_A k_gi_sampling_a(KPARAMS, int cur, u32 seed, u32 frame, const __grid_constant__ TexFilterDev tf) {
+    ST_GRID_DEP();
     ST_TRACE_STACK();
     Px g = pixel_half(cam);
     if (!g.in) return;
@@ -503,7 +516,8 @@
 }
 
 template <bool LGRID>
-ST_DEV void gi_sampling_b_pair(const CameraDev& cam, const SceneDev& sc, const TraceStack& stk, int cur, u32 seed, u32 frame, Px g, float4 d0, float4 d1, float4 d2, const LightGridDev& lg) {
+ST_DEV void gi_sampling_b_pair(const CameraDev& cam, const SceneDev& sc, const TraceStack& stk, int cur, u32 seed, u32 frame, Px g, float4 d0, float4 d1, float4 d2, const LightGridDev& lg,
+                               const GiRes* k11 = nullptr) {
     bool tracing = gi_tracing_frame(frame);
     uint2 sp = tracing ? checker(g.x, g.y, frame / 2u) : checker(g.x, g.y, frame);
     if (!cam_contains_u(cam.curr, sp.x, sp.y)) return;
@@ -516,7 +530,7 @@
         gh = hit_make(ray_make(prim.point, xyz(d0)), gbuf_unpack(sc, d1, d2));
         gi_pdf_ = d0.w;
     } else {
-        GiRes res = gi_load(cam.gi_reservoirs[2], idx);
+        GiRes res = k11 ? *k11 : gi_load(cam.gi_reservoirs[2], idx);
         if (res.m == 0.0f) return;
         rng.s = res.rng;
         gh = hit_make(ray_make(res.v1, xyz(d0)), gbuf_unpack(sc, d1, d2));
@@ -562,24 +576,38 @@
 }
 template <bool LGRID>
 __global__ void ST_LB_GI_SAMPLING_B k_gi_sampling_b(KPARAMS, int cur, u32 seed, u32 frame, const __grid_constant__ LightGridDev lg) {
+    ST_GRID_DEP();
     ST_TRACE_STACK();
     Px g = pixel_half(cam);
     if (!g.in) return;
     size_t gi = pix(cam, g.x, g.y);
     gi_sampling_b_pair<LGRID>(cam, sc, stk, cur, seed, frame, g, cam.gi_d0[gi], cam.gi_d1[gi], cam.gi_d2[gi], lg);
 }
+ST_DEV GiRes gi_as_stored(GiRes r) { r.v2n = oct_decode(oct_encode(r.v2n)); return r; }
 template <bool NMAP, bool LGRID, bool TEXF>
 __global__ void ST_LB_GI_SAMPLING_B k_gi_sampling_fused(KPARAMS, int cur, u32 seed_a, u32 seed_b, u32 frame, const __grid_constant__ LightGridDev lg,
-                                                        const __grid_constant__ TexFilterDev tf) {
+                                                        const __grid_constant__ TexFilterDev tf, int k11_here) {
+    ST_GRID_DEP();
     ST_TRACE_STACK();
     Px g = pixel_half(cam);
     if (!g.in) return;
+    GiRes r11;
+    const GiRes* k11 = nullptr;
+    if (k11_here && !gi_tracing_frame(frame)) {
+        const uint2 sp = checker(g.x, g.y, frame);
+        if (!cam_contains_u(cam.curr, sp.x, sp.y)) return;
+        Hit hit = load_hit_lut(sc, cam.curr, cam.prim_gbuffer_d0[cur], cam.prim_gbuffer_d1[cur], cam, sp.x, sp.y);
+        if (!hit_some(hit)) return;
+        r11 = gi_as_stored(gi_reprojection_px(cam, hit, reproj_decode(cam.reprojection_map[pix(cam, sp.x, sp.y)])));
+        k11 = &r11;
+    }
     float4 t0, t1, t2;
-    if (!gi_sampling_a_pair<NMAP, TEXF>(cam, sc, stk, cur, seed_a, frame, g, &t0, &t1, &t2, tf)) return;
-    gi_sampling_b_pair<LGRID>(cam, sc, stk, cur, seed_b, frame, g, t0, t1, t2, lg);
+    if (!gi_sampling_a_pair<NMAP, TEXF>(cam, sc, stk, cur, seed_a, frame, g, &t0, &t1, &t2, tf, k11)) return;
+    gi_sampling_b_pair<LGRID>(cam, sc, stk, cur, seed_b, frame, g, t0, t1, t2, lg, k11);
 }
 
 __global__ void ST_LB_GI_TEMPORAL k_gi_temporal(KPARAMS, int cur, u32 seed, u32 frame, int inline_reprojection) {
+    ST_GRID_DEP();
     Px p = pixel_full(cam);
     if (!p.in) return;
     bool tracing = gi_tracing_frame(frame);
@@ -595,8 +623,9 @@
     Reproj rp = reproj_decode(cam.reprojection_map[pix(cam, p.x, p.y)]);
     if (inline_reprojection) {
         GiRes r11 = gi_reprojection_px(cam, lhs_hit, rp);
-        if ((int)p.x >= 2 * half_grid_w(cam.w)) gi_store_m(cam, r11, cam.gi_reservoirs[2], lhs_idx, p.y, cam.gi_mirror_reach);
-        if (reproj_some(rp)) { rhs = r11; rhs.v2n = oct_decode(oct_encode(r11.v2n)); }
+        const bool tail = (int)p.x >= 2 * half_grid_w(cam.w);
+        if (tail || inline_reprojection == 2) gi_store_m(cam, r11, cam.gi_reservoirs[2], lhs_idx, p.y, tail ? cam.gi_mirror_reach : 0);
+        if (reproj_some(rp)) rhs = gi_as_stored(r11);
     } else if (reproj_some(rp)) rhs = gi_load(cam.gi_reservoirs[2], lhs_idx);
     if (reproj_some(rp)) {
         rhs.confidence = 1.0f;
@@ -681,6 +710,7 @@
     return o;
 }
 __global__ void ST_LB_GI_SPATIAL_PICK k_gi_spatial_pick(KPARAMS, int cur, u32 seed, u32 frame) {
+    ST_GRID_DEP();
     Px g = pixel_half(cam);
     if (!g.in) return;
     store_pair_texels(cam, gi_spatial_pick_pair(cam, sc, cur, seed, frame, g), cam.gi_d0, cam.gi_d1, g);
@@ -718,11 +748,13 @@
     if (cam_contains_u(cam.curr, op.x, op.y)) { size_t oi = screen_idx(cam, op.x, op.y); gi_store_m(cam, gi_load(in, oi), out, oi, op.y, cam.gi_mirror_reach); }
 }
 __global__ void ST_LB_GI_SPATIAL_SAMPLE k_gi_spatial_sample(KPARAMS, u32 seed, u32 frame) {
+    ST_GRID_DEP();
     Px g = pixel_half(cam);
     if (!g.in) return;
     gi_spatial_sample_pair(cam, seed, frame, g, tex_or_zero(cam.gi_d2, cam, g.x * 2u, g.y), tex_or_zero(cam.gi_d2, cam, g.x * 2u + 1u, g.y));
 }
 __global__ void ST_LB_GI_SPATIAL_PICK k_gi_spatial_fused(KPARAMS, int cur, u32 seed_pick, u32 seed_sample, u32 frame) {
+    ST_GRID_DEP();
     ST_TRACE_STACK();
     Px g = pixel_half(cam);
     if (!g.in) return;
@@ -770,6 +802,7 @@
     return true;
 }
 __global__ void ST_LB_GI_PREVIEW k_gi_preview(KPARAMS, int cur, u32 seed, u32 nth, const float4* __restrict__ in, float4* __restrict__ out, int reach) {
+    ST_GRID_DEP();
     Px p = pixel_full(cam);
     if (!p.in) return;
     Hit chit = load_hit_lut(sc, cam.curr, cam.prim_gbuffer_d0[cur], cam.prim_gbuffer_d1[cur], cam, p.x, p.y);
@@ -790,12 +823,14 @@
     gi_store(gi_load(in, idx), cam.gi_reservoirs[0], idx);
 }
 __global__ void ST_LB_GI_RESOLVING k_gi_resolving(KPARAMS, int cur, const float4* __restrict__ in) {
+    ST_GRID_DEP();
     Px p = pixel_full(cam);
     if (!p.in) return;
     Hit hit = load_hit_lut(sc, cam.curr, cam.prim_gbuffer_d0[cur], cam.prim_gbuffer_d1[cur], cam, p.x, p.y);
     gi_resolving_px(cam, hit, gi_load(cam.gi_reservoirs[0], screen_idx(cam, p.x, p.y)), in, p);
 }
 __global__ void ST_LB_GI_PREVIEW k_gi_preview_resolve(KPARAMS, int cur, u32 seed, const float4* __restrict__ in, const float4* __restrict__ source) {
+    ST_GRID_DEP();
     Px p = pixel_full(cam);
     if (!p.in) return;
     Hit chit = load_hit_lut(sc, cam.curr, cam.prim_gbuffer_d0[cur], cam.prim_gbuffer_d1[cur], cam, p.x, p.y);
@@ -807,6 +842,7 @@
 #if ST_EXACT_ONLY
 __global__ void __launch_bounds__(ST_BLOCK) k_denoise_reproject(KPARAMS, int cur, const float4* __restrict__ prev_colors, const float4* __restrict__ prev_moments,
                                                                 const float4* __restrict__ samples, float4* __restrict__ colors, float4* __restrict__ moments) {
+    ST_GRID_DEP();
     Px p = pixel_full(cam);
     if (!p.in) return;
     size_t i = pix(cam, p.x, p.y);
@@ -843,6 +879,7 @@
     store4m(cam, g.moments + i, f4(moment, 0.0f), y, ST_REACH_SVGF);
 }
 __global__ void __launch_bounds__(ST_BLOCK) k_denoise_reproject_pair(KPARAMS, int cur, const __grid_constant__ ReprojectSignal di, const __grid_constant__ ReprojectSignal gi) {
+    ST_GRID_DEP();
     Px p = pixel_full(cam);
     if (!p.in) return;
     size_t i = pix(cam, p.x, p.y);
@@ -876,6 +913,7 @@
 
 template <bool FAST>
 __global__ void __launch_bounds__(ST_BLOCK) k_denoise_variance(KPARAMS, int cur) {
+    ST_GRID_DEP();
     Px p = pixel_full(cam);
     if (!p.in) return;
     size_t i = pix(cam, p.x, p.y);
@@ -927,6 +965,7 @@
                                                               const float4* __restrict__ di_in, float4* __restrict__ di_out,
                                                               const float4* __restrict__ gi_in, float4* __restrict__ gi_out,
                                                               const float4* __restrict__ pair_in, float4* __restrict__ pair_out) {
+    ST_GRID_DEP();
     Px p = pixel_full(cam);
     if (!p.in) return;
     size_t i = pix(cam, p.x, p.y);
@@ -1066,6 +1105,7 @@
                                                                    const __grid_constant__ CUtensorMap tm_gi,
                                                                    float4* __restrict__ di_out, float4* __restrict__ gi_out, float4* __restrict__ pair_out,
                                                                    u32* __restrict__ errors) {
+    ST_GRID_DEP();
     typedef WaveletTile<S, J, TW, TH> T;
     extern __shared__ unsigned char s_raw[];
     __shared__ __align__(8) unsigned long long s_bar;
@@ -1140,6 +1180,7 @@
     return color;
 }
 __global__ void __launch_bounds__(ST_BLOCK) k_composition(KPARAMS, int cur, u32 mode, const float4* __restrict__ di_diff, const float4* __restrict__ gi_diff) {
+    ST_GRID_DEP();
     Px p = pixel_full(cam);
     if (!p.in) return;
     size_t i = pix(cam, p.x, p.y);
@@ -1163,6 +1204,7 @@
 }
 __global__ void __launch_bounds__(TAA_TW * TAA_TH) k_taa_resolve(KPARAMS, int cur, u32 mode, const float4* __restrict__ di_diff, const float4* __restrict__ gi_diff,
                                                                  const float4* __restrict__ hist_in, float4* __restrict__ hist_out, float4 jit) {
+    ST_GRID_DEP();
     const int HW = TAA_TW + 2, HH = TAA_TH + 2;
     __shared__ float4 s_t[HW * HH];
     const int bx = (int)blockIdx.x * TAA_TW - 1, by = (int)blockIdx.y * TAA_TH - 1;
@@ -1228,6 +1270,7 @@
 
 
 __global__ void __launch_bounds__(ST_BLOCK) k_output_rgba8(KPARAMS, uchar4* __restrict__ out) {
+    ST_GRID_DEP();
     Px p = pixel_full(cam);
     if (!p.in) return;
     size_t i = pix(cam, p.x, p.y);
@@ -1614,19 +1657,27 @@
     out[i] = r;
 }
 
+template <typename... P, typename... A>
+static void launch_pdl(void (*k)(P...), dim3 grid, dim3 block, size_t smem, cudaStream_t st, A&&... args) {
+    cudaLaunchAttribute at[1];
+    at[0].id = cudaLaunchAttributeProgrammaticStreamSerialization; at[0].val.programmaticStreamSerializationAllowed = 1;
+    cudaLaunchConfig_t cfg = {};
+    cfg.gridDim = grid; cfg.blockDim = block; cfg.dynamicSmemBytes = smem; cfg.stream = st; cfg.attrs = at; cfg.numAttrs = 1;
+    cudaLaunchKernelEx(&cfg, k, std::forward<A>(args)...);
+}
 static dim3 grid_full(const CameraDev& cam) { return dim3((cam.w + TILE_W - 1) / TILE_W, (cam.y1 - cam.y0 + TILE_H - 1) / TILE_H); }
 static dim3 grid_half(const CameraDev& cam) { int hw = 8 * (((cam.w + 7) / 8) / 2); return dim3((hw + TILE_W - 1) / TILE_W, (cam.y1 - cam.y0 + TILE_H - 1) / TILE_H); }
-#define HALF_LAUNCH(kernel, c, st, ...) do { dim3 g_ = grid_half(c); if (g_.x > 0 && g_.y > 0) kernel<<<g_, ST_BLOCK, 0, st>>>(__VA_ARGS__); } while (0)
+#define HALF_LAUNCH(kernel, c, st, ...) do { dim3 g_ = grid_half(c); if (g_.x > 0 && g_.y > 0) launch_pdl(kernel, g_, ST_BLOCK, 0, st, __VA_ARGS__); } while (0)
 
 void launch_di_sampling(const CameraDev& c, const SceneDev& s, int cur, u32 seed, u32 frame, const LightGridDev* lg, cudaStream_t st) {
-    if (lg) k_di_sampling<true><<<grid_full(c), ST_BLOCK, 0, st>>>(c, s, cur, seed, frame, *lg); else k_di_sampling<false><<<grid_full(c), ST_BLOCK, 0, st>>>(c, s, cur, seed, frame, LightGridDev{});
-}
-void launch_di_temporal(const CameraDev& c, const SceneDev& s, int cur, u32 seed, cudaStream_t st) { k_di_temporal<<<grid_full(c), ST_BLOCK, 0, st>>>(c, s, cur, seed); }
+    if (lg) launch_pdl(k_di_sampling<true>, grid_full(c), ST_BLOCK, 0, st, c, s, cur, seed, frame, *lg); else launch_pdl(k_di_sampling<false>, grid_full(c), ST_BLOCK, 0, st, c, s, cur, seed, frame, LightGridDev{});
+}
+void launch_di_temporal(const CameraDev& c, const SceneDev& s, int cur, u32 seed, cudaStream_t st) { launch_pdl(k_di_temporal, grid_full(c), ST_BLOCK, 0, st, c, s, cur, seed); }
 void launch_di_spatial_pick(const CameraDev& c, const SceneDev& s, int cur, u32 seed, u32 frame, cudaStream_t st) { HALF_LAUNCH(k_di_spatial_pick, c, st, c, s, cur, seed, frame); }
-void launch_spatial_trace(const CameraDev& c, const SceneDev& s, const float4* d0, const float4* d1, float4* d2, cudaStream_t st) { k_spatial_trace<<<grid_full(c), ST_BLOCK, 0, st>>>(c, s, d0, d1, d2); }
+void launch_spatial_trace(const CameraDev& c, const SceneDev& s, const float4* d0, const float4* d1, float4* d2, cudaStream_t st) { launch_pdl(k_spatial_trace, grid_full(c), ST_BLOCK, 0, st, c, s, d0, d1, d2); }
 void launch_di_spatial_sample(const CameraDev& c, const SceneDev& s, u32 seed, u32 frame, cudaStream_t st) { HALF_LAUNCH(k_di_spatial_sample, c, st, c, s, seed, frame); }
-void launch_di_resolving(const CameraDev& c, const SceneDev& s, int cur, cudaStream_t st) { k_di_resolving<<<grid_full(c), ST_BLOCK, 0, st>>>(c, s, cur); }
-void launch_gi_reprojection(const CameraDev& c, const SceneDev& s, int cur, cudaStream_t st) { k_gi_reprojection<<<grid_full(c), ST_BLOCK, 0, st>>>(c, s, cur); }
+void launch_di_resolving(const CameraDev& c, const SceneDev& s, int cur, cudaStream_t st) { launch_pdl(k_di_resolving, grid_full(c), ST_BLOCK, 0, st, c, s, cur); }
+void launch_gi_reprojection(const CameraDev& c, const SceneDev& s, int cur, cudaStream_t st) { launch_pdl(k_gi_reprojection, grid_full(c), ST_BLOCK, 0, st, c, s, cur); }
 void launch_gi_sampling_a(const CameraDev& c, const SceneDev& s, int cur, u32 seed, u32 frame, bool nmap, const TexFilterDev* tf, cudaStream_t st) {
     if (tf) {
         if (nmap) HALF_LAUNCH((k_gi_sampling_a<true, true>), c, st, c, s, cur, seed, frame, *tf); else HALF_LAUNCH((k_gi_sampling_a<false, true>), c, st, c, s, cur, seed, frame, *tf);
@@ -1638,23 +1689,23 @@
 void launch_gi_sampling_b(const CameraDev& c, const SceneDev& s, int cur, u32 seed, u32 frame, const LightGridDev* lg, cudaStream_t st) {
     if (lg) HALF_LAUNCH(k_gi_sampling_b<true>, c, st, c, s, cur, seed, frame, *lg); else HALF_LAUNCH(k_gi_sampling_b<false>, c, st, c, s, cur, seed, frame, LightGridDev{});
 }
-void launch_gi_temporal(const CameraDev& c, const SceneDev& s, int cur, u32 seed, u32 frame, int inline_reprojection, cudaStream_t st) { k_gi_temporal<<<grid_full(c), ST_BLOCK, 0, st>>>(c, s, cur, seed, frame, inline_reprojection); }
+void launch_gi_temporal(const CameraDev& c, const SceneDev& s, int cur, u32 seed, u32 frame, int inline_reprojection, cudaStream_t st) { launch_pdl(k_gi_temporal, grid_full(c), ST_BLOCK, 0, st, c, s, cur, seed, frame, inline_reprojection); }
 void launch_gi_spatial_pick(const CameraDev& c, const SceneDev& s, int cur, u32 seed, u32 frame, cudaStream_t st) { HALF_LAUNCH(k_gi_spatial_pick, c, st, c, s, cur, seed, frame); }
 void launch_gi_spatial_sample(const CameraDev& c, const SceneDev& s, u32 seed, u32 frame, cudaStream_t st) { HALF_LAUNCH(k_gi_spatial_sample, c, st, c, s, seed, frame); }
-void launch_gi_preview(const CameraDev& c, const SceneDev& s, int cur, u32 seed, u32 nth, const float4* in, float4* out, int mirror_reach, cudaStream_t st) { k_gi_preview<<<grid_full(c), ST_BLOCK, 0, st>>>(c, s, cur, seed, nth, in, out, mirror_reach); }
-void launch_gi_resolving(const CameraDev& c, const SceneDev& s, int cur, const float4* in, cudaStream_t st) { k_gi_resolving<<<grid_full(c), ST_BLOCK, 0, st>>>(c, s, cur, in); }
+void launch_gi_preview(const CameraDev& c, const SceneDev& s, int cur, u32 seed, u32 nth, const float4* in, float4* out, int mirror_reach, cudaStream_t st) { launch_pdl(k_gi_preview, grid_full(c), ST_BLOCK, 0, st, c, s, cur, seed, nth, in, out, mirror_reach); }
+void launch_gi_resolving(const CameraDev& c, const SceneDev& s, int cur, const float4* in, cudaStream_t st) { launch_pdl(k_gi_resolving, grid_full(c), ST_BLOCK, 0, st, c, s, cur, in); }
 void launch_di_sample_temporal(const CameraDev& c, const SceneDev& s, int cur, u32 seed_sampling, u32 seed_temporal, u32 frame, const LightGridDev* lg, cudaStream_t st) {
-    if (lg) k_di_sample_temporal<true><<<grid_full(c), ST_BLOCK, 0, st>>>(c, s, cur, seed_sampling, seed_temporal, frame, *lg);
-    else k_di_sample_temporal<false><<<grid_full(c), ST_BLOCK, 0, st>>>(c, s, cur, seed_sampling, seed_temporal, frame, LightGridDev{});
+    if (lg) launch_pdl(k_di_sample_temporal<true>, grid_full(c), ST_BLOCK, 0, st, c, s, cur, seed_sampling, seed_temporal, frame, *lg);
+    else launch_pdl(k_di_sample_temporal<false>, grid_full(c), ST_BLOCK, 0, st, c, s, cur, seed_sampling, seed_temporal, frame, LightGridDev{});
 }
 void launch_di_spatial_fused(const CameraDev& c, const SceneDev& s, int cur, u32 seed_pick, u32 seed_sample, u32 frame, cudaStream_t st) { HALF_LAUNCH(k_di_spatial_fused, c, st, c, s, cur, seed_pick, seed_sample, frame); }
 void launch_gi_sampling_fused(const CameraDev& c, const SceneDev& s, int cur, u32 seed_a, u32 seed_b, u32 frame, bool nmap, const LightGridDev* lg, const TexFilterDev* tf,
-                              cudaStream_t st) {
+                              int k11_here, cudaStream_t st) {
     const LightGridDev none{};
     const LightGridDev& g = lg ? *lg : none;
     const TexFilterDev tnone{};
     const TexFilterDev& t = tf ? *tf : tnone;
-#define ST_GSF(N_, L_, T_) HALF_LAUNCH((k_gi_sampling_fused<N_, L_, T_>), c, st, c, s, cur, seed_a, seed_b, frame, g, t)
+#define ST_GSF(N_, L_, T_) HALF_LAUNCH((k_gi_sampling_fused<N_, L_, T_>), c, st, c, s, cur, seed_a, seed_b, frame, g, t, k11_here)
     if (tf) {
         if (lg) { if (nmap) ST_GSF(true, true, true); else ST_GSF(false, true, true); }
         else { if (nmap) ST_GSF(true, false, true); else ST_GSF(false, false, true); }
@@ -1665,30 +1716,30 @@
 #undef ST_GSF
 }
 void launch_gi_spatial_fused(const CameraDev& c, const SceneDev& s, int cur, u32 seed_pick, u32 seed_sample, u32 frame, cudaStream_t st) { HALF_LAUNCH(k_gi_spatial_fused, c, st, c, s, cur, seed_pick, seed_sample, frame); }
-void launch_gi_preview_resolve(const CameraDev& c, const SceneDev& s, int cur, u32 seed, const float4* in, const float4* source, cudaStream_t st) { k_gi_preview_resolve<<<grid_full(c), ST_BLOCK, 0, st>>>(c, s, cur, seed, in, source); }
+void launch_gi_preview_resolve(const CameraDev& c, const SceneDev& s, int cur, u32 seed, const float4* in, const float4* source, cudaStream_t st) { launch_pdl(k_gi_preview_resolve, grid_full(c), ST_BLOCK, 0, st, c, s, cur, seed, in, source); }
 void launch_math_shading(int op, const float* a, const float* b, float* out, long n, cudaStream_t st) { k_math_shading<<<(unsigned)((n + 255) / 256), 256, 0, st>>>(op, a, b, out, n); }
 #if ST_EXACT_ONLY
 void launch_prim_gbuffer(const CameraDev& c, const SceneDev& s, int cur, int with_reprojection, bool nmap, const TexFilterDev* tf, cudaStream_t st) {
     const TexFilterDev none{};
     const TexFilterDev& t = tf ? *tf : none;
-#define ST_PG(N_, T_) k_prim_gbuffer<N_, T_><<<grid_full(c), ST_BLOCK, 0, st>>>(c, s, cur, with_reprojection, t)
+#define ST_PG(N_, T_) launch_pdl(k_prim_gbuffer<N_, T_>, grid_full(c), ST_BLOCK, 0, st, c, s, cur, with_reprojection, t)
     if (tf) { if (nmap) ST_PG(true, true); else ST_PG(false, true); }
     else { if (nmap) ST_PG(true, false); else ST_PG(false, false); }
 #undef ST_PG
 }
-void launch_frame_reprojection(const CameraDev& c, const SceneDev& s, int cur, cudaStream_t st) { k_frame_reprojection<<<grid_full(c), ST_BLOCK, 0, st>>>(c, s, cur); }
-void launch_denoise_reproject(const CameraDev& c, const SceneDev& s, int cur, const float4* pc, const float4* pm, const float4* smp, float4* col, float4* mom, cudaStream_t st) { k_denoise_reproject<<<grid_full(c), ST_BLOCK, 0, st>>>(c, s, cur, pc, pm, smp, col, mom); }
+void launch_frame_reprojection(const CameraDev& c, const SceneDev& s, int cur, cudaStream_t st) { launch_pdl(k_frame_reprojection, grid_full(c), ST_BLOCK, 0, st, c, s, cur); }
+void launch_denoise_reproject(const CameraDev& c, const SceneDev& s, int cur, const float4* pc, const float4* pm, const float4* smp, float4* col, float4* mom, cudaStream_t st) { launch_pdl(k_denoise_reproject, grid_full(c), ST_BLOCK, 0, st, c, s, cur, pc, pm, smp, col, mom); }
 void launch_denoise_reproject_pair(const CameraDev& c, const SceneDev& s, int cur, cudaStream_t st) {
     ReprojectSignal di{c.di_diff_prev_colors, c.di_diff_moments[cur ^ 1], c.di_diff_samples, c.di_diff_curr_colors, c.di_diff_moments[cur]};
     ReprojectSignal gi{c.gi_diff_prev_colors, c.gi_diff_moments[cur ^ 1], c.gi_diff_samples, c.gi_diff_curr_colors, c.gi_diff_moments[cur]};
-    k_denoise_reproject_pair<<<grid_full(c), ST_BLOCK, 0, st>>>(c, s, cur, di, gi);
+    launch_pdl(k_denoise_reproject_pair, grid_full(c), ST_BLOCK, 0, st, c, s, cur, di, gi);
 }
 void launch_denoise_variance(const CameraDev& c, const SceneDev& s, int cur, bool fast, cudaStream_t st) {
-    if (fast) k_denoise_variance<true><<<grid_full(c), ST_BLOCK, 0, st>>>(c, s, cur); else k_denoise_variance<false><<<grid_full(c), ST_BLOCK, 0, st>>>(c, s, cur);
+    if (fast) launch_pdl(k_denoise_variance<true>, grid_full(c), ST_BLOCK, 0, st, c, s, cur); else launch_pdl(k_denoise_variance<false>, grid_full(c), ST_BLOCK, 0, st, c, s, cur);
 }
 void launch_denoise_wavelet(const CameraDev& c, const SceneDev& s, int cur, u32 frame, u32 stride, float strength, const float4* di_in, float4* di_out, const float4* gi_in, float4* gi_out,
                             const float4* pair_in, float4* pair_out, bool fast, cudaStream_t st) {
-#define ST_WG(F_, P_) k_denoise_wavelet<F_, P_><<<grid_full(c), ST_BLOCK, 0, st>>>(c, s, cur, frame, stride, strength, di_in, di_out, gi_in, gi_out, pair_in, pair_out)
+#define ST_WG(F_, P_) launch_pdl(k_denoise_wavelet<F_, P_>, grid_full(c), ST_BLOCK, 0, st, c, s, cur, frame, stride, strength, di_in, di_out, gi_in, gi_out, pair_in, pair_out)
     if (pair_in) { if (fast) ST_WG(true, true); else ST_WG(false, true); }
     else { if (fast) ST_WG(true, false); else ST_WG(false, false); }
 #undef ST_WG
@@ -1702,6 +1753,7 @@
 template <bool FAST, int TW, int TH>
 __global__ void __launch_bounds__(TW * TH) k_denoise_variance_tiled(KPARAMS, int cur, const __grid_constant__ CUtensorMap tm_nd, const __grid_constant__ CUtensorMap tm_di,
                                                                     const __grid_constant__ CUtensorMap tm_gi, u32* __restrict__ errors) {
+    ST_GRID_DEP();
     typedef VarianceTile<TW, TH> T;
     extern __shared__ unsigned char s_raw[];
     __shared__ __align__(8) unsigned long long s_bar;
@@ -1863,13 +1915,13 @@
     if (c.curr.screen.x != (float)c.w || c.curr.screen.y != (float)c.h) return false;
     return fast ? variance_tiled_go<true>(c, s, cur, errors, st) : variance_tiled_go<false>(c, s, cur, errors, st);
 }
-void launch_composition(const CameraDev& c, const SceneDev& s, int cur, u32 mode, const float4* di_diff, const float4* gi_diff, cudaStream_t st) { k_composition<<<grid_full(c), ST_BLOCK, 0, st>>>(c, s, cur, mode, di_diff, gi_diff); }
+void launch_composition(const CameraDev& c, const SceneDev& s, int cur, u32 mode, const float4* di_diff, const float4* gi_diff, cudaStream_t st) { launch_pdl(k_composition, grid_full(c), ST_BLOCK, 0, st, c, s, cur, mode, di_diff, gi_diff); }
 void launch_taa_resolve(const CameraDev& c, const SceneDev& s, int cur, u32 mode, const float4* di_diff, const float4* gi_diff, const float4* hist_in, float4* hist_out,
                         float4 jit, cudaStream_t st) {
     const dim3 grid((c.w + TAA_TW - 1) / TAA_TW, (c.h + TAA_TH - 1) / TAA_TH);
-    k_taa_resolve<<<grid, TAA_TW * TAA_TH, 0, st>>>(c, s, cur, mode, di_diff, gi_diff, hist_in, hist_out, jit);
-}
-void launch_output_rgba8(const CameraDev& c, const SceneDev& s, uchar4* out, cudaStream_t st) { k_output_rgba8<<<grid_full(c), ST_BLOCK, 0, st>>>(c, s, out); }
+    launch_pdl(k_taa_resolve, grid, TAA_TW * TAA_TH, 0, st, c, s, cur, mode, di_diff, gi_diff, hist_in, hist_out, jit);
+}
+void launch_output_rgba8(const CameraDev& c, const SceneDev& s, uchar4* out, cudaStream_t st) { launch_pdl(k_output_rgba8, grid_full(c), ST_BLOCK, 0, st, c, s, out); }
 void launch_ref_tracing(const CameraDev& c, const SceneDev& s, u32 depth, bool nmap, cudaStream_t st) {
     if (nmap) k_ref_tracing<true><<<grid_full(c), ST_BLOCK, 0, st>>>(c, s, depth); else k_ref_tracing<false><<<grid_full(c), ST_BLOCK, 0, st>>>(c, s, depth);
 }
diff --git a/strolle_b200/csrc/kernels.h b/strolle_b200/csrc/kernels.h
--- a/strolle_b200/csrc/kernels.h
+++ b/strolle_b200/csrc/kernels.h
@@ -23,7 +23,7 @@
 void launch_gi_resolving(const CameraDev& c, const SceneDev& s, int cur, const float4* in, cudaStream_t st);
 void launch_di_sample_temporal(const CameraDev& c, const SceneDev& s, int cur, u32 seed_sampling, u32 seed_temporal, u32 frame, const LightGridDev* lg, cudaStream_t st);
 void launch_di_spatial_fused(const CameraDev& c, const SceneDev& s, int cur, u32 seed_pick, u32 seed_sample, u32 frame, cudaStream_t st);
-void launch_gi_sampling_fused(const CameraDev& c, const SceneDev& s, int cur, u32 seed_a, u32 seed_b, u32 frame, bool nmap, const LightGridDev* lg, const TexFilterDev* tf, cudaStream_t st);
+void launch_gi_sampling_fused(const CameraDev& c, const SceneDev& s, int cur, u32 seed_a, u32 seed_b, u32 frame, bool nmap, const LightGridDev* lg, const TexFilterDev* tf, int k11_here, cudaStream_t st);
 void launch_gi_spatial_fused(const CameraDev& c, const SceneDev& s, int cur, u32 seed_pick, u32 seed_sample, u32 frame, cudaStream_t st);
 void launch_gi_preview_resolve(const CameraDev& c, const SceneDev& s, int cur, u32 seed, const float4* in, const float4* source, cudaStream_t st);
 void launch_denoise_reproject(const CameraDev& c, const SceneDev& s, int cur, const float4* pc, const float4* pm, const float4* smp, float4* col, float4* mom, cudaStream_t st);
@@ -109,7 +109,7 @@
 void launch_gi_resolving(const CameraDev& c, const SceneDev& s, int cur, const float4* in, cudaStream_t st);
 void launch_di_sample_temporal(const CameraDev& c, const SceneDev& s, int cur, u32 seed_sampling, u32 seed_temporal, u32 frame, const LightGridDev* lg, cudaStream_t st);
 void launch_di_spatial_fused(const CameraDev& c, const SceneDev& s, int cur, u32 seed_pick, u32 seed_sample, u32 frame, cudaStream_t st);
-void launch_gi_sampling_fused(const CameraDev& c, const SceneDev& s, int cur, u32 seed_a, u32 seed_b, u32 frame, bool nmap, const LightGridDev* lg, const TexFilterDev* tf, cudaStream_t st);
+void launch_gi_sampling_fused(const CameraDev& c, const SceneDev& s, int cur, u32 seed_a, u32 seed_b, u32 frame, bool nmap, const LightGridDev* lg, const TexFilterDev* tf, int k11_here, cudaStream_t st);
 void launch_gi_spatial_fused(const CameraDev& c, const SceneDev& s, int cur, u32 seed_pick, u32 seed_sample, u32 frame, cudaStream_t st);
 void launch_gi_preview_resolve(const CameraDev& c, const SceneDev& s, int cur, u32 seed, const float4* in, const float4* source, cudaStream_t st);
 void launch_math_shading(int op, const float* a, const float* b, float* out, long n, cudaStream_t st);
```

Result: no change. 3745, median of 6 (+0.4%).
